# david-knigge/enf-pde

Measured on AMD Instinct MI355X. Metric: query-points/sec (ENF fit+decode) at 64 latents x 64^2 grid, higher is better.
Workload: dtype bf16

## Files before the change

enf-pde_amd/_lib.py:

```python
import ctypes
import os

_HERE = os.path.dirname(os.path.abspath(__file__))
LIB_PATH = os.environ.get("ENF_HIP_LIB") or os.path.join(_HERE, "libenf_hip.so")
TEST_LIB_PATH = os.environ.get("ENF_HIP_TEST_LIB") or os.path.join(_HERE, "libenf_hip_test.so")

ENF_NUM_TENSORS = 46
PREC = {"f32": 0, "fp32": 0, "float32": 0, "bf16": 1, "bfloat16": 1}
INVARIANT_IDS = {"rel_pos_periodic": 0, "latitude_periodic": 1, "polar_periodic": 2, "ponita": 3,
                 "abs_pos": 4, "rel_pos": 5, "norm_rel_pos": 6, "ball": 7, "ball_lat": 8, "ponita_full": 9}

EXPORTS = ["enf_abi_version", "enf_strerror", "enf_invariant_dim", "enf_invariant_pose_dim", "enf_check_desc",
           "enf_packed_weight_bytes", "enf_pack_weights", "enf_workspace_bytes", "enf_forward",
           "enf_backward_latents", "enf_backward_latents_ex", "enf_forward_stages", "enf_lt_layout", "enf_lt_layout_ext", "enf_pack_pair", "enf_pair_forward",
           "enf_pair_backward", "enf_pair_backward_ex", "enf_pair_scratch_bytes", "enf_pair_variant", "enf_pair_partition", "enf_backward_weights", "enf_backward_weights_scratch_bytes",
           "enf_backward_all", "enf_backward_all_scratch_bytes", "enf_fit_step", "enf_fit_inputs",
           "enf_mse_value_grad",
           "enf_ode_conv_forward", "enf_ode_conv_backward_basis", "enf_ode_conv_backward_weight", "enf_ode_conv_backward_weight_scratch_bytes", "enf_ode_poly_num_features", "enf_ode_poly_forward",
           "enf_ode_poly_backward", "enf_ode_vec_readout_forward", "enf_ode_vec_readout_backward", "enf_ode_block_supported", "enf_ode_block_scratch_bytes", "enf_ode_block_forward", "enf_ode_block_backward",
           "enf_ode_basis_supported", "enf_ode_basis_scratch_bytes", "enf_ode_basis_forward",
           "enf_ode_basis_backward", "enf_relu_mask_bytes", "enf_meta_sgd_update"]
ENF_NUM_PAIR_TENSORS = 12
(ENF_S_EQ, ENF_S_EV, ENF_S_G1, ENF_S_NH, ENF_S_DA1, ENF_S_DA2, ENF_S_DA3, ENF_S_HEAD0) = range(8)


def num_store(H):
    return 7 + 4 * H


class EnfDesc(ctypes.Structure):
    _fields_ = [(n, ctypes.c_int32) for n in
                ("B", "N", "Z", "H", "D", "C", "O", "dx", "invariant_id", "use_window", "precision")] + \
               [("h_true", ctypes.c_int32), ("d_true", ctypes.c_int32),
                ("pair_fwd_variant", ctypes.c_int32), ("pair_bwd_variant", ctypes.c_int32), ("mask_mode", ctypes.c_int32),
                ("mask_signals", ctypes.c_int32), ("embedding", ctypes.c_int32), ("relu_masks", ctypes.c_void_p)]


VARIANT = {"auto": 0, "latent_split": 1, "z_fold": 2, "z_fold_zsplit": 3}
MASK_MODE = {"off": 0, "write": 1, "read": 2}
EMB = {"rff": 0, "ffn": 1}


class EnfSgdSegment(ctypes.Structure):
    _fields_ = [("x", ctypes.c_void_p), ("g", ctypes.c_void_p), ("lr", ctypes.c_void_p), ("out", ctypes.c_void_p),
                ("n", ctypes.c_int64), ("width", ctypes.c_int32), ("g_stride", ctypes.c_int32), ("lr_len", ctypes.c_int32),
                ("reserved", ctypes.c_int32)]


ENF_SGD_MAX_SEGMENTS = 4


class EnfFitComponent(ctypes.Structure):
    _fields_ = [("src", ctypes.c_void_p), ("dst", ctypes.c_void_p), ("width", ctypes.c_int32), ("reserved", ctypes.c_int32)]


class EnfError(RuntimeError):
    pass


_lib = None
_test_lib = None


def load():
    global _lib
    if _lib is not None:
        return _lib
    _lib = _bind(LIB_PATH, test_hooks=False)
    return _lib


def load_test():
    global _test_lib
    if _test_lib is None:
        _test_lib = _bind(TEST_LIB_PATH, test_hooks=True)
    return _test_lib


class using:

    def __init__(self, lib):
        self.lib = lib

    def __enter__(self):
        global _lib
        self.prev, _lib = _lib, self.lib
        return self.lib

    def __exit__(self, *exc):
        global _lib
        _lib = self.prev


def _bind(path, test_hooks):
    if not os.path.exists(path):
        raise EnfError(f"{path} not found: build it with `make -C enf-pde_amd/csrc` "
                       "(or python -c 'import __graft_entry__ as g; g.build()'). There is no fallback path.")
    lib = ctypes.CDLL(path)
    vp, i64, sz, ci = ctypes.c_void_p, ctypes.c_int64, ctypes.c_size_t, ctypes.c_int
    dp = ctypes.POINTER(EnfDesc)
    lib.enf_abi_version.restype = ci
    lib.enf_strerror.restype = ctypes.c_char_p
    lib.enf_strerror.argtypes = [ci]
    lib.enf_invariant_dim.argtypes = [ci, ci]
    lib.enf_invariant_pose_dim.argtypes = [ci, ci]
    lib.enf_check_desc.argtypes = [dp]
    lib.enf_packed_weight_bytes.restype = sz
    lib.enf_packed_weight_bytes.argtypes = [dp]
    lib.enf_workspace_bytes.restype = sz
    lib.enf_workspace_bytes.argtypes = [dp]
    lib.enf_pack_weights.argtypes = [dp, ctypes.POINTER(vp), vp, vp]
    lib.enf_forward.argtypes = [dp, vp, i64, vp, vp, vp, vp, vp, vp, vp, vp, sz, vp]
    lib.enf_forward_stages.argtypes = [dp, vp, i64, vp, vp, vp, vp, vp, vp, vp, vp, sz, ctypes.c_uint, vp]
    lib.enf_backward_latents.argtypes = [dp, vp, i64, vp, vp, vp, vp, vp, vp, vp, vp, vp, vp, vp, sz, vp]
    lib.enf_backward_latents_ex.argtypes = [dp, vp, i64, vp, vp, vp, vp, vp, vp, vp, vp, vp, vp, vp, sz, ctypes.c_uint, vp]
    ip = ctypes.POINTER(ci)
    lib.enf_lt_layout.argtypes = [dp, ip, ip, ip, ip, ip, ip]
    lib.enf_pack_pair.argtypes = [dp, ctypes.POINTER(vp), vp, vp]
    lib.enf_mse_value_grad.argtypes = [vp, vp, sz, ctypes.c_float, vp, vp, vp]
    lib.enf_meta_sgd_update.argtypes = [ctypes.c_int, ctypes.POINTER(EnfSgdSegment), ctypes.c_float, vp]
    lib.enf_fit_inputs.argtypes = [ctypes.c_int, ctypes.POINTER(EnfFitComponent)] + [ctypes.c_int32] * 7 + [vp] * 7
    lib.enf_ode_conv_forward.argtypes = [ci, ci, ci, ci, vp, vp, i64, i64, vp, vp, vp, vp]
    lib.enf_ode_conv_backward_basis.argtypes = [ci, ci, ci, ci, vp, vp, vp, vp, vp]
    lib.enf_ode_conv_backward_weight_scratch_bytes.restype = sz
    lib.enf_ode_conv_backward_weight_scratch_bytes.argtypes = [ci, ci, ci, ci]
    lib.enf_ode_conv_backward_weight.argtypes = [ci, ci, ci, ci, vp, vp, vp, vp, vp, sz, vp]
    lib.enf_ode_poly_num_features.argtypes = [ci, ci]
    lib.enf_ode_poly_forward.argtypes = [i64, ci, ci, vp, vp, vp]
    lib.enf_ode_poly_backward.argtypes = [i64, ci, ci, vp, vp, vp, vp]
    lib.enf_ode_basis_supported.argtypes = [ci, ci, ci, ci, ci]
    cf = ctypes.c_float
    lib.enf_ode_vec_readout_forward.argtypes = [ci, ci, ci, ci, vp, vp, vp, vp, cf, cf, vp, vp, vp]
    lib.enf_ode_vec_readout_backward.argtypes = [ci, ci, ci, ci, vp, vp, vp, vp, cf, cf, vp, vp, vp, vp, vp, vp, vp, vp]
    lib.enf_ode_block_supported.argtypes = [ci, ci]
    lib.enf_ode_block_scratch_bytes.restype = sz
    lib.enf_ode_block_scratch_bytes.argtypes = [i64, ci, ci]
    lib.enf_ode_block_forward.argtypes = [i64, ci, ci, vp, vp, vp, vp, vp, vp, vp, ctypes.c_float, vp, vp, vp]
    lib.enf_ode_block_backward.argtypes = [i64, ci, ci, vp, vp, vp, vp, vp, vp, vp, ctypes.c_float, vp, vp, vp, sz, vp]
    lib.enf_ode_basis_scratch_bytes.restype = sz
    lib.enf_ode_basis_scratch_bytes.argtypes = [i64, ci, ci, ci, ci]
    lib.enf_ode_basis_forward.argtypes = [i64, ci, ci, ci, ci, vp, vp, vp, vp, vp, vp, vp, sz, vp]
    lib.enf_ode_basis_backward.argtypes = [i64, ci, ci, ci, ci, vp, vp, vp, vp, vp, vp, vp, vp, vp, vp, vp, vp, sz, vp]
    lib.enf_relu_mask_bytes.restype = sz
    lib.enf_relu_mask_bytes.argtypes = [dp]
    lib.enf_pair_variant.argtypes = [dp, ci]
    lib.enf_pair_partition.argtypes = [dp] + [ctypes.POINTER(ctypes.c_int32)] * 3
    lib.enf_backward_weights_scratch_bytes.restype = sz
    lib.enf_backward_weights_scratch_bytes.argtypes = [dp, ci]
    lib.enf_backward_weights.argtypes = [dp, vp, i64, vp, vp, vp, vp, vp, vp, ctypes.POINTER(vp), vp, vp, sz, vp]
    lib.enf_fit_step.argtypes = [dp, vp, i64, vp, vp, vp, vp, vp, ctypes.c_float, vp, vp, vp, vp, vp, sz, vp]
    lib.enf_backward_all_scratch_bytes.restype = sz
    lib.enf_backward_all_scratch_bytes.argtypes = [dp, ci]
    lib.enf_backward_all.argtypes = [dp, vp, i64, vp, vp, vp, ctypes.POINTER(vp), vp, vp, vp, vp, vp, vp, vp, ctypes.POINTER(vp), vp,
                                     vp, sz, vp, sz, ctypes.c_uint, vp]
    lib.enf_pair_scratch_bytes.restype = sz
    lib.enf_pair_scratch_bytes.argtypes = [dp]
    lib.enf_pair_forward.argtypes = [dp, vp, i64, vp, vp, vp, vp, vp, sz, vp]
    lib.enf_pair_backward.argtypes = [dp, vp, i64, vp, vp, vp, vp, vp, vp, ctypes.POINTER(vp), vp]
    lib.enf_pair_backward_ex.argtypes = [dp, vp, i64, vp, vp, vp, vp, vp, vp, ctypes.POINTER(vp), vp, vp]
    if test_hooks:
        for name in ("enf_debug_gemm", "enf_debug_pack", "enf_test_read_wave_sums"):
            getattr(lib, name).restype = ci
        lib.enf_debug_gemm.argtypes = [vp, vp, vp, ci, ci, ci, vp]
        lib.enf_debug_pack.argtypes = [vp, vp, ci, ci, ci, vp]
        lib.enf_test_read_wave_sums.argtypes = [vp]
    if lib.enf_abi_version() != 2:
        raise EnfError(f"{path}: ABI version mismatch")
    return lib


def check(rc):
    if rc == 0:
        return
    msg = load().enf_strerror(rc).decode()
    if rc == -2:
        raise ValueError(msg)
    if rc == -6:
        raise AssertionError(msg)
    if rc == -3:
        raise NotImplementedError(msg)
    raise EnfError(f"libenf_hip error {rc}: {msg}")


def launch(dev, fn, *args):
    import torch
    idx = dev.index if dev.index is not None else torch.cuda.current_device()
    if idx == torch.cuda.current_device():
        return check(fn(*args))
    with torch.cuda.device(idx):
        return check(fn(*args))


def make_desc(B, N, Z, H, D, C, O, dx, invariant_id, use_window, precision, d_true=0, h_true=0, variants=(0, 0),
              masks=None, embedding=0):
    d = EnfDesc()
    d.B, d.N, d.Z, d.H, d.D, d.C, d.O, d.dx = int(B), int(N), int(Z), int(H), int(D), int(C), int(O), int(dx)
    d.invariant_id, d.use_window, d.precision = int(invariant_id), int(bool(use_window)), int(precision)
    d.d_true, d.h_true = int(d_true), int(h_true)
    d.pair_fwd_variant, d.pair_bwd_variant = int(variants[0]), int(variants[1])
    d.embedding = int(embedding)
    if masks is not None:
        buf, mode, signals = masks
        d.relu_masks, d.mask_mode, d.mask_signals = buf.data_ptr(), MASK_MODE[mode], int(signals)
    return d
```

enf-pde_amd/csrc/enf_api.hip:

```cpp
#include <hip/hip_runtime.h>
#include <mutex>
#include <unordered_map>
#include "enf_launch.h"

extern "C" int enf_abi_version(void) { return ENF_ABI_VERSION; }

extern "C" const char* enf_strerror(int code) {
  switch (code) {
    case ENF_OK: return "ok";
    case ENF_EINVAL: return "invalid argument (null pointer or non-positive size)";
    case ENF_EINVARIANT: return "Unknown invariant type";
    case ENF_EUNSUPPORTED: return "shape not in the compiled kernel set (num_hidden 64 or 128 after padding; num_heads 1, 2, or 4 at num_hidden 64; "
                                  "num_out <= 32; ball / ball_lat at num_hidden 64 only)";
    case ENF_EWORKSPACE: return "workspace too small";
    case ENF_ELAUNCH: return "HIP launch failed";
    case ENF_EDIM: return "coordinate / pose width inconsistent with the invariant";
    default: return "unknown error";
  }
}

extern "C" int enf_invariant_dim(int inv, int dx) {
  const int i = enf_inv_dim(inv, dx);
  return i < 0 ? ENF_EINVARIANT : i;
}
extern "C" int enf_invariant_pose_dim(int inv, int dx) {
  const int i = enf_inv_pose_dim(inv, dx);
  return i < 0 ? ENF_EINVARIANT : i;
}

extern "C" int enf_check_desc(const EnfDesc* d) {
  if (!d) return ENF_EINVAL;
  if (d->B <= 0 || d->N <= 0 || d->Z <= 0 || d->C <= 0 || d->O <= 0 || d->H <= 0 || d->D <= 0) return ENF_EINVAL;
  if (d->invariant_id < 0 || d->invariant_id >= ENF_INV_COUNT) return ENF_EINVARIANT;
  if (d->dx < 1 || d->dx > 3) return ENF_EDIM;
  const bool two_d = d->invariant_id == ENF_INV_REL_POS_PERIODIC || d->invariant_id == ENF_INV_PONITA ||
                     d->invariant_id == ENF_INV_LATITUDE_PERIODIC || d->invariant_id == ENF_INV_POLAR_PERIODIC;
  if (two_d && d->dx != 2) return ENF_EDIM;
  if (d->invariant_id == ENF_INV_PONITA_FULL && d->dx != 3) return ENF_EDIM;
  if (enf_inv_has_phase(d->invariant_id) && d->D != 64) return ENF_EUNSUPPORTED;
  if (enf_inv_has_phase(d->invariant_id) && d->dx != 3) return ENF_EDIM;
  if (!(d->D == 64 || d->D == 128)) return ENF_EUNSUPPORTED;
  if (d->d_true < 0 || d->d_true > d->D || (d->d_true & 1)) return ENF_EINVAL;
  if (!(d->H == 1 || d->H == 2 || (d->H == 4 && d->D == 64))) return ENF_EUNSUPPORTED;
  if (d->h_true < 0 || d->h_true > d->H) return ENF_EINVAL;
  if (d->O > 32) return ENF_EUNSUPPORTED;
  if (d->precision != ENF_PREC_F32 && d->precision != ENF_PREC_BF16) return ENF_EINVAL;
  if (d->pair_fwd_variant < ENF_VARIANT_AUTO || d->pair_fwd_variant > ENF_VARIANT_ZFOLD_ZSPLIT) return ENF_EINVAL;
  if (d->pair_bwd_variant < ENF_VARIANT_AUTO || d->pair_bwd_variant > ENF_VARIANT_ZFOLD) return ENF_EINVAL;
  if (d->mask_mode < ENF_MASK_OFF || d->mask_mode > ENF_MASK_READ || d->mask_signals < 0) return ENF_EINVAL;
  if (d->mask_mode != ENF_MASK_OFF && !d->relu_masks) return ENF_EINVAL;
  if (d->embedding != ENF_EMB_RFF && d->embedding != ENF_EMB_FFN) return ENF_EINVAL;
  if (d->embedding == ENF_EMB_FFN && enf_inv_has_phase(d->invariant_id)) return ENF_EUNSUPPORTED;
  return ENF_OK;
}

extern "C" size_t enf_packed_weight_bytes(const EnfDesc* d) {
  if (enf_check_desc(d) != ENF_OK) return 0;
  return enf_layout(enf_dims(d)).total;
}

extern "C" size_t enf_workspace_bytes(const EnfDesc* d) {
  if (enf_check_desc(d) != ENF_OK) return 0;
  return enf_workspace(enf_dims(d)).total;
}

struct SidePending { hipEvent_t join = nullptr; bool pending = false; };
struct SideStream {
  hipStream_t s = nullptr;
  hipEvent_t fork = nullptr;
  std::mutex mu;
  std::unordered_map<const void*, SidePending> ws;
  SidePending* entry(const void* workspace) {
    auto it = ws.find(workspace);
    if (it != ws.end()) return &it->second;
    if (ws.size() >= 64)
      for (auto j = ws.begin(); j != ws.end();) {
        if (!j->second.pending) { (void)hipEventDestroy(j->second.join); j = ws.erase(j); } else ++j;
      }
    SidePending e;
    if (hipEventCreateWithFlags(&e.join, hipEventDisableTiming) != hipSuccess) return nullptr;
    return &ws.emplace(workspace, e).first->second;
  }
};
static constexpr int ENF_MAX_DEVICES = 64;
static SideStream* side_stream() {
  static std::mutex table_mu;
  static SideStream* table[ENF_MAX_DEVICES] = {};
  static bool tried[ENF_MAX_DEVICES] = {};
  int dev = 0;
  if (hipGetDevice(&dev) != hipSuccess || dev < 0 || dev >= ENF_MAX_DEVICES) return nullptr;
  std::lock_guard<std::mutex> lk(table_mu);
  if (!tried[dev]) {
    tried[dev] = true;
    SideStream* t = new SideStream();
    if (hipStreamCreateWithFlags(&t->s, hipStreamNonBlocking) == hipSuccess &&
        hipEventCreateWithFlags(&t->fork, hipEventDisableTiming) == hipSuccess)
      table[dev] = t;
    else
      delete t;
  }
  return table[dev];
}

int enf_side_join_pending(hipStream_t st, const void* workspace) {
  SideStream* side = side_stream();
  if (!side) return 0;
  std::lock_guard<std::mutex> lk(side->mu);
  auto it = side->ws.find(workspace);
  if (it != side->ws.end() && it->second.pending) {
    if (hipStreamWaitEvent(st, it->second.join, 0) != hipSuccess) return ENF_ELAUNCH;
    it->second.pending = false;
  }
  return 0;
}

static int side_prepare_bwd(SideStream* side, const EnfCall& c, bool zero_dlt) {
  if (!side) return 0;
  std::lock_guard<std::mutex> lk(side->mu);
  SidePending* e = side->entry(c.ws);
  if (!e) return 0;
  if (hipEventRecord(side->fork, c.st) != hipSuccess || hipStreamWaitEvent(side->s, side->fork, 0) != hipSuccess) return ENF_ELAUNCH;
  if (int rc = enf_launch_wz(c.m, c.L, c.blob, c.F(c.W.lt), nullptr, c.F(c.W.wzb), nullptr, c.ws + c.W.wzt, side->s)) return rc;
  if (zero_dlt && hipMemsetAsync(c.F(c.W.dlt), 0, enf_lt_bytes(c.m), side->s) != hipSuccess) return ENF_ELAUNCH;
  if (hipEventRecord(e->join, side->s) != hipSuccess) return ENF_ELAUNCH;
  e->pending = true;
  return 1;
}

extern "C" int enf_forward_stages(const EnfDesc* d, const float* x, int64_t x_bstride, const float* p, const float* a,
                                  const float* sigma, const void* packed, float* out, float* ybar, float* lse,
                                  void* workspace, size_t workspace_bytes, unsigned stages, void* stream) {
  EnfCall c;
  int rc = enf_call(c, d, x && p && a && out, sigma, packed, workspace, workspace_bytes, stream);
  if (rc) return rc;
  const EnfDims& m = c.m;
  const EnfWorkspace& W = c.W;
  float* yb = ybar ? ybar : c.F(W.ybar);
  const bool zf = enf_use_zfold(m);
  float* ls = lse ? lse : c.F(W.lse);
  const bool yhalf = (stages & ENF_STAGE_YBAR_HALF) && m.bf16 && !ybar && (stages & ENF_STAGE_PAIR) && (stages & ENF_STAGE_TAIL) &&
                     !(stages & ENF_STAGE_TAIL_SAVE) && enf_zfold_split(m) <= 1;
  if ((rc = enf_side_join_pending(c.st, workspace))) return rc;
  if ((stages & ENF_STAGE_PROLOGUE) && (rc = enf_launch_prologue(m, c.L, c.blob, p, a, sigma, c.F(W.lt), c.F(W.an), c.F(W.kv), c.st))) return rc;
  if ((stages & (ENF_STAGE_PAIR | ENF_STAGE_FOLD)) &&
      (rc = enf_launch_pair_fwd(m, c.L, c.blob, x, x_bstride, c.F(W.lt), yb, ls, zf ? c.ws + W.wz : nullptr, zf ? c.F(W.wzb) : nullptr,
                                zf ? c.ws + W.wzu : nullptr, enf_zfold_split(m) > 1 ? c.F(W.ysplit) : nullptr, (stages & ENF_STAGE_FOLD) != 0,
                                ((stages & ENF_STAGE_PAIR) != 0 ? 1 : 0) | (yhalf ? 2 : 0), c.st)))
    return rc;
  if ((stages & ENF_STAGE_PREPARE_BWD) && enf_use_zfold_bwd(m) && (rc = side_prepare_bwd(side_stream(), c, true)) < 0) return rc;
  const bool tsave = (stages & ENF_STAGE_TAIL_SAVE) != 0;
  if ((stages & ENF_STAGE_TAIL) &&
      (rc = enf_launch_tail(m, c.L, c.blob, yb, out, nullptr, nullptr, nullptr, tsave ? c.F(W.tail_act) : nullptr, 0, (tsave ? 1 : 0) | (yhalf ? 2 : 0), c.st)))
    return rc;
  return ENF_OK;
}

extern "C" int enf_forward(const EnfDesc* d, const float* x, int64_t x_bstride, const float* p, const float* a,
                           const float* sigma, const void* packed, float* out, float* ybar, float* lse, void* workspace,
                           size_t workspace_bytes, void* stream) {
  return enf_forward_stages(d, x, x_bstride, p, a, sigma, packed, out, ybar, lse, workspace, workspace_bytes,
                            ENF_STAGE_PROLOGUE | ENF_STAGE_FOLD | ENF_STAGE_PAIR | ENF_STAGE_TAIL, stream);
}

extern "C" int enf_backward_latents(const EnfDesc* d, const float* x, int64_t x_bstride, const float* p, const float* a,
                                    const float* sigma, const void* packed, const float* ybar, const float* lse,
                                    const float* dout, float* dp, float* da, float* dsigma, void* workspace,
                                    size_t workspace_bytes, void* stream) {
  return enf_backward_latents_ex(d, x, x_bstride, p, a, sigma, packed, ybar, lse, dout, dp, da, dsigma, workspace,
                                 workspace_bytes, 0u, stream);
}

static int pair_bwd_on_workspace(const EnfCall& c, const float* x, int64_t x_bstride, const float* lse) {
  const bool zb = enf_use_zfold_bwd(c.m);
  return enf_launch_pair_bwd(c.m, c.L, c.blob, x, x_bstride, c.F(c.W.lt), lse, c.F(c.W.dybar), c.F(c.W.delta), c.F(c.W.dlt), nullptr,
                             zb ? c.ws + c.W.wzt : nullptr, zb ? c.F(c.W.wzb) : nullptr, nullptr, c.st);
}

extern "C" int enf_backward_latents_ex(const EnfDesc* d, const float* x, int64_t x_bstride, const float* p, const float* a,
                                       const float* sigma, const void* packed, const float* ybar, const float* lse,
                                       const float* dout, float* dp, float* da, float* dsigma, void* workspace,
                                       size_t workspace_bytes, unsigned flags, void* stream) {
  EnfCall c;
  int rc = enf_call(c, d, x && p && a && ybar && lse && dout && dp && da && dsigma, sigma, packed, workspace, workspace_bytes, stream);
  if (rc) return rc;
  const EnfDims& m = c.m;
  const EnfWorkspace& W = c.W;
  hipStream_t st = c.st;
  const bool zb = enf_use_zfold_bwd(m);
  if (flags & ENF_BWD_ONLY_PAIR) {
    if ((rc = enf_side_join_pending(st, workspace))) return rc;
    if (hipMemsetAsync(c.F(W.dlt), 0, enf_lt_bytes(m), st) != hipSuccess) return ENF_ELAUNCH;
    return pair_bwd_on_workspace(c, x, x_bstride, lse);
  }
  if (!(flags & ENF_BWD_REUSE_PROLOGUE) && (rc = enf_launch_prologue(m, c.L, c.blob, p, a, sigma, c.F(W.lt), c.F(W.an), c.F(W.kv), st)))
    return rc;
  SideStream* side = zb ? side_stream() : nullptr;
  bool prepared = false;
  if (zb && side && (flags & ENF_BWD_REUSE_PREPARED) && (flags & ENF_BWD_REUSE_PROLOGUE)) {
    std::lock_guard<std::mutex> lk(side->mu);
    auto it = side->ws.find(workspace);
    prepared = it != side->ws.end() && it->second.pending;
  }
  if (!prepared && (rc = enf_side_join_pending(st, workspace))) return rc;
  if (zb && !prepared) {
    if ((rc = side_prepare_bwd(side, c, false)) < 0) return rc;
    if (!rc && (rc = enf_launch_wz(m, c.L, c.blob, c.F(W.lt), nullptr, c.F(W.wzb), nullptr, c.ws + W.wzt, st))) return rc;
  }
  const bool treuse = (flags & ENF_BWD_REUSE_TAIL) && (flags & ENF_BWD_REUSE_PROLOGUE);
  if ((rc = enf_launch_tail(m, c.L, c.blob, ybar, nullptr, dout, c.F(W.dybar), c.F(W.delta), c.F(W.tail_act), 1, treuse ? 1 : 0, st))) return rc;
  if (!prepared && hipMemsetAsync(c.F(W.dlt), 0, enf_lt_bytes(m), st) != hipSuccess) return ENF_ELAUNCH;
  if ((rc = enf_side_join_pending(st, workspace))) return rc;
  if ((rc = pair_bwd_on_workspace(c, x, x_bstride, lse))) return rc;
  return enf_launch_prologue_bwd(m, c.L, c.blob, p, sigma, c.F(W.an), c.F(W.kv), c.F(W.dlt), dp, da, dsigma, st);
}


extern "C" int enf_fit_step(const EnfDesc* d, const float* x, int64_t x_bstride, const float* p, const float* a, const float* sigma,
                            const void* packed, const float* target, float grad_scale, float* loss, float* dp, float* da,
                            float* dsigma, void* workspace, size_t workspace_bytes, void* stream) {
  EnfCall c;
  int rc = enf_call(c, d, x && p && a && target && loss && dp && da && dsigma, sigma, packed, workspace, workspace_bytes, stream);
  if (rc) return rc;
  const EnfDims& m = c.m;
  const EnfWorkspace& W = c.W;
  hipStream_t st = c.st;
  const bool zf = enf_use_zfold(m), zb = enf_use_zfold_bwd(m);
  if ((rc = enf_side_join_pending(st, workspace))) return rc;
  if ((rc = enf_launch_prologue(m, c.L, c.blob, p, a, sigma, c.F(W.lt), c.F(W.an), c.F(W.kv), st))) return rc;
  if ((rc = enf_launch_pair_fwd(m, c.L, c.blob, x, x_bstride, c.F(W.lt), c.F(W.ybar), c.F(W.lse), zf ? c.ws + W.wz : nullptr,
                                zf ? c.F(W.wzb) : nullptr, zf ? c.ws + W.wzu : nullptr, enf_zfold_split(m) > 1 ? c.F(W.ysplit) : nullptr, 1, 1, st)))
    return rc;
  if ((rc = side_prepare_bwd(zb ? side_stream() : nullptr, c, true)) < 0) return rc;
  if (!rc) {
    if (zb && (rc = enf_launch_wz(m, c.L, c.blob, c.F(W.lt), nullptr, c.F(W.wzb), nullptr, c.ws + W.wzt, st))) return rc;
    if (hipMemsetAsync(c.F(W.dlt), 0, enf_lt_bytes(m), st) != hipSuccess) return ENF_ELAUNCH;
  }
  if ((rc = enf_launch_tail_loss(m, c.L, c.blob, c.F(W.ybar), target, grad_scale, loss, c.F(W.dybar), c.F(W.delta), c.F(W.tail_act), st))) return rc;
  if ((rc = enf_side_join_pending(st, workspace))) return rc;
  if ((rc = pair_bwd_on_workspace(c, x, x_bstride, c.F(W.lse)))) return rc;
  return enf_launch_prologue_bwd(m, c.L, c.blob, p, sigma, c.F(W.an), c.F(W.kv), c.F(W.dlt), dp, da, dsigma, st);
}

extern "C" int enf_lt_layout(const EnfDesc* d, int* stride, int* off_u, int* off_v0, int* off_pose, int* off_wcoef, int* off_c) {
  int rc = enf_check_desc(d);
  if (rc) return rc;
  if (stride) *stride = enf_lt_stride(d->H, d->D);
  if (off_u) *off_u = enf_lt_off_u(d->H, d->D);
  if (off_v0) *off_v0 = enf_lt_off_v0(d->H, d->D);
  if (off_pose) *off_pose = enf_lt_off_pose(d->H, d->D);
  if (off_wcoef) *off_wcoef = enf_lt_off_wcoef(d->H, d->D);
  if (off_c) *off_c = enf_lt_off_c(d->H, d->D);
  return ENF_OK;
}

extern "C" int enf_lt_layout_ext(const EnfDesc* d, int* off_ext, int* off_phase_q, int* off_phase_v) {
  int rc = enf_check_desc(d);
  if (rc) return rc;
  if (off_ext) *off_ext = enf_lt_off_ext(d->H, d->D);
  if (off_phase_q) *off_phase_q = enf_lt_off_phq(d->H, d->D);
  if (off_phase_v) *off_phase_v = enf_lt_off_phv(d->H, d->D);
  return ENF_OK;
}

extern "C" int enf_pair_variant(const EnfDesc* d, int backward) {
  const int rc = enf_check_desc(d);
  if (rc) return rc;
  const EnfDims m = enf_dims(d);
  if (backward) return enf_use_zfold_bwd(m) ? ENF_VARIANT_ZFOLD : ENF_VARIANT_LATENT_SPLIT;
  const int sp = enf_zfold_split(m);
  return sp > 1 ? ENF_VARIANT_ZFOLD_ZSPLIT : (sp == 1 ? ENF_VARIANT_ZFOLD : ENF_VARIANT_LATENT_SPLIT);
}

extern "C" int enf_pair_partition(const EnfDesc* d, int32_t* run, int32_t* workgroups, int32_t* parts) {
  const int rc = enf_check_desc(d);
  if (rc) return rc;
  if (!run || !workgroups || !parts) return ENF_EINVAL;
  const EnfDims m = enf_dims(d);
  if (enf_zfold_split(m) < 2) return 0;
  const EnfStreamK k = enf_zfold_streamk(m);
  *run = k.len; *workgroups = k.wgs; *parts = k.parts;
  return 1;
}

struct PairScratch { size_t wz, wzb, wzu, ysplit, total; };
static PairScratch pair_scratch(const EnfDims& m) {
  PairScratch s{0, 0, 0, 0, 0};
  if (!enf_use_zfold(m)) return s;
  const size_t BZ = (size_t)m.B * m.Z, BN = (size_t)m.B * m.N;
  const int split = enf_zfold_split(m);
  s.wzb = s.wz + enf_align(BZ * m.H * enf_panel_bytes(m.D, m.D, m.bf16));
  s.wzu = s.wzb + enf_align(sizeof(float) * BZ * m.HD);
  s.ysplit = s.wzu + enf_align(BZ * enf_wzu_bytes(m.H, m.D));
  s.total = s.ysplit + (split > 1 ? sizeof(float) * split * (BN * m.HD + BN * m.H * 3) : 0);
  return s;
}

extern "C" size_t enf_pair_scratch_bytes(const EnfDesc* d) {
  if (enf_check_desc(d)) return 0;
  return pair_scratch(enf_dims(d)).total;
}

extern "C" int enf_pair_forward(const EnfDesc* d, const float* x, int64_t x_bstride, const float* lt, const void* packed,
                                float* ybar, float* lse, void* scratch, size_t scratch_bytes, void* stream) {
  int rc = enf_check_desc(d);
  if (rc) return rc;
  if (!x || !lt || !packed || !ybar || !lse) return ENF_EINVAL;
  const EnfDims m = enf_dims(d);
  const PairScratch S = pair_scratch(m);
  const bool zf = S.total != 0;
  if (zf && (!scratch || scratch_bytes < S.total)) return ENF_EWORKSPACE;
  char* sc = (char*)scratch;
  return enf_launch_pair_fwd(m, enf_layout(m), (const char*)packed, x, x_bstride, lt, ybar, lse, zf ? sc + S.wz : nullptr,
                             zf ? reinterpret_cast<float*>(sc + S.wzb) : nullptr, zf ? sc + S.wzu : nullptr,
                             zf && enf_zfold_split(m) > 1 ? reinterpret_cast<float*>(sc + S.ysplit) : nullptr, 1, 1, (hipStream_t)stream);
}

extern "C" size_t enf_relu_mask_bytes(const EnfDesc* d) {
  if (enf_check_desc(d) != ENF_OK) return 0;
  const size_t signals = d->mask_signals > 0 ? d->mask_signals : d->B;
  return signals * d->Z * ((d->N + 15) / 16) * 2 * 64 * sizeof(unsigned);
}

extern "C" int enf_pair_backward(const EnfDesc* d, const float* x, int64_t x_bstride, const float* lt, const void* packed,
                                 const float* lse, const float* dybar, const float* delta, float* dlt, void* const* store,
                                 void* stream) {
  return enf_pair_backward_ex(d, x, x_bstride, lt, packed, lse, dybar, delta, dlt, store, nullptr, stream);
}

extern "C" int enf_pair_backward_ex(const EnfDesc* d, const float* x, int64_t x_bstride, const float* lt, const void* packed,
                                    const float* lse, const float* dybar, const float* delta, float* dlt, void* const* store,
                                    float* dx, void* stream) {
  int rc = enf_check_desc(d);
  if (rc) return rc;
  if (!x || !lt || !packed || !lse || !dybar || !delta || !dlt) return ENF_EINVAL;
  const EnfDims m = enf_dims(d);
  if (store)
    for (int i = 0; i < ENF_NUM_STORE(m.H); ++i)
      if (!store[i]) return ENF_EINVAL;
  hipStream_t st = (hipStream_t)stream;
  if (hipMemsetAsync(dlt, 0, enf_lt_bytes(m), st) != hipSuccess) return ENF_ELAUNCH;
  return enf_launch_pair_bwd(m, enf_layout(m), (const char*)packed, x, x_bstride, lt, lse, dybar, delta, dlt, store, nullptr, nullptr, dx, st);
}

extern "C" size_t enf_backward_weights_scratch_bytes(const EnfDesc* d, int chunk_signals) {
  if (enf_check_desc(d) != ENF_OK || chunk_signals < 1 || chunk_signals > d->B) return 0;
  return enf_wgrad_scratch_bytes(enf_dims(d), chunk_signals);
}

extern "C" int enf_backward_weights(const EnfDesc* d, const float* x, int64_t x_bstride, const float* lt, const void* packed,
                                    const float* lse, const float* dybar, const float* delta, float* dlt,
                                    float* const* dpair, float* dx, void* scratch, size_t scratch_bytes, void* stream) {
  int rc = enf_check_desc(d);
  if (rc) return rc;
  if (d->embedding == ENF_EMB_FFN) return ENF_EUNSUPPORTED;
  if (!x || !lt || !packed || !lse || !dybar || !delta || !dlt || !dpair || !scratch) return ENF_EINVAL;
  for (int i = 0; i < ENF_NUM_PAIR_TENSORS; ++i)
    if (i != ENF_P_COEFQ && i != ENF_P_COEFV && !dpair[i]) return ENF_EINVAL;
  const EnfDims m = enf_dims(d);
  const int cb = enf_wgrad_chunk(m, scratch_bytes, [&](int n) { return enf_wgrad_scratch_bytes(m, n); });
  if (!cb) return ENF_EWORKSPACE;
  return enf_launch_wgrad_chunks(m, enf_layout(m), (const char*)packed, cb, x, x_bstride, lt, lse, dybar, delta, dlt, dx, (char*)scratch,
                                 dpair, (hipStream_t)stream);
}
```

enf-pde_amd/csrc/enf_debug.hip:

```cpp
#include <hip/hip_runtime.h>
#include "enf_launch.h"
#include "enf_device.h"

template <int KBIN, int MTOUT, bool BF16>
__global__ __launch_bounds__(64) void enf_debug_gemm_kernel(const char* panel, const float* X, float* Y) {
  extern __shared__ __attribute__((aligned(16))) char smem[];
  const int lane = threadIdx.x, col = lane & 15, quad = lane >> 4;
  constexpr int BYTES = PanelCfg<KBIN, MTOUT, BF16>::BYTES;
  for (int i = lane; i < BYTES / 16; i += 64)
    reinterpret_cast<f32x4*>(smem)[i] = reinterpret_cast<const f32x4*>(panel)[i];
  __syncthreads();
  f32x4 x[2 * KBIN];
#pragma unroll
  for (int t = 0; t < 2 * KBIN; ++t)
#pragma unroll
    for (int i = 0; i < 4; ++i) x[t][i] = X[(16 * t + 4 * quad + i) * 16 + col];
  Frags<BF16, KBIN> F;
  make_frags<BF16, KBIN>(F, x);
  f32x4 acc[MTOUT];
#pragma unroll
  for (int m = 0; m < MTOUT; ++m) acc[m] = f32x4{0.f, 0.f, 0.f, 0.f};
  gemm_stage<BF16, KBIN, MTOUT>(acc, F, smem, lane);
#pragma unroll
  for (int m = 0; m < MTOUT; ++m)
#pragma unroll
    for (int i = 0; i < 4; ++i) Y[(16 * m + 4 * quad + i) * 16 + col] = acc[m][i];
}

extern "C" int enf_debug_gemm(const void* panel, const float* X, float* Y, int M, int K, int bf16, void* stream) {
  hipStream_t st = (hipStream_t)stream;
  const size_t bytes = (size_t)M * K * (bf16 ? 2 : 4);
#define C(KB, MT)                                                                                                   \
  if (K == 32 * KB && M == 16 * MT) {                                                                               \
    if (bf16) hipLaunchKernelGGL((enf_debug_gemm_kernel<KB, MT, true>), dim3(1), dim3(64), bytes, st, (const char*)panel, X, Y);  \
    else hipLaunchKernelGGL((enf_debug_gemm_kernel<KB, MT, false>), dim3(1), dim3(64), bytes, st, (const char*)panel, X, Y);      \
    return hipGetLastError() == hipSuccess ? 0 : ENF_ELAUNCH;                                                        \
  }
  C(2, 4) C(4, 4) C(1, 4) C(2, 1)
#undef C
  return ENF_EUNSUPPORTED;
}
```

enf-pde_amd/csrc/enf_launch.h:

```cpp
#pragma once
#include <hip/hip_runtime.h>
#include <atomic>
#include "enf_layout.h"

typedef std::atomic<unsigned long long> EnfAttrBits;
inline bool enf_lds_attr(const void* kern, int bytes, EnfAttrBits& done) {
  int dev = 0;
  if (hipGetDevice(&dev) != hipSuccess) return false;
  if (dev >= 0 && dev < 64 && ((done.load(std::memory_order_acquire) >> dev) & 1ull)) return true;
  if (hipFuncSetAttribute(kern, hipFuncAttributeMaxDynamicSharedMemorySize, bytes) != hipSuccess) return false;
  if (dev >= 0 && dev < 64) done.fetch_or(1ull << dev, std::memory_order_release);
  return true;
}

struct EnfCall {
  EnfDims m;
  EnfLayout L;
  EnfWorkspace W;
  hipStream_t st;
  char* ws;
  const char* blob;
  float* F(size_t off) const { return reinterpret_cast<float*>(ws + off); }
};
inline int enf_call(EnfCall& c, const EnfDesc* d, bool pointers_ok, const float* sigma, const void* packed, void* workspace,
                    size_t workspace_bytes, void* stream) {
  const int rc = enf_check_desc(d);
  if (rc) return rc;
  if (!pointers_ok || !packed || !workspace) return ENF_EINVAL;
  if (d->use_window && !sigma) return ENF_EINVAL;
  c.m = enf_dims(d);
  c.L = enf_layout(c.m);
  c.W = enf_workspace(c.m);
  if (workspace_bytes < c.W.total) return ENF_EWORKSPACE;
  c.st = (hipStream_t)stream;
  c.ws = (char*)workspace;
  c.blob = (const char*)packed;
  return ENF_OK;
}

int enf_side_join_pending(hipStream_t st, const void* workspace);

int enf_launch_prologue(const EnfDims& m, const EnfLayout& L, const char* blob, const float* p, const float* a, const float* sigma,
                        float* lt, float* an, float* kv, hipStream_t st);
int enf_launch_prologue_bwd(const EnfDims& m, const EnfLayout& L, const char* blob, const float* p, const float* sigma,
                            const float* an, const float* kv, const float* dlt, float* dp, float* da, float* dsigma, hipStream_t st);
int enf_launch_prologue_bwd_wg(const EnfDims& m, const EnfLayout& L, const char* blob, const float* p, const float* sigma,
                               const float* an, const float* kv, const float* dlt, float* dp, float* da, float* dsigma, float* pg,
                               hipStream_t st);

int enf_launch_wz(const EnfDims& m, const EnfLayout& L, const char* blob, const float* lt, char* wz, float* wzb, char* wzu,
                  char* wzt, hipStream_t st);

int enf_launch_pair_fwd(const EnfDims& m, const EnfLayout& L, const char* blob, const float* x, long long x_bstride, const float* lt,
                        float* ybar, float* lse, char* wz, float* wzb, char* wzu, float* ysplit, int run_fold, int run_pair,
                        hipStream_t st);

int enf_launch_pair_bwd(const EnfDims& m, const EnfLayout& L, const char* blob, const float* x, long long x_bstride, const float* lt,
                        const float* lse, const float* dybar, const float* delta, float* dlt, void* const* store, const char* wzt,
                        const float* wzb, float* dxq, hipStream_t st);

size_t enf_xtd_part_bytes(const EnfDims& m, long long P);
int enf_launch_xtd(const EnfDims& m, void* const* store, long long P, float* const* dpair, float* part, int accumulate,
                   hipStream_t st);

size_t enf_wgrad_scratch_bytes(const EnfDims& m, int cb);
int enf_launch_wgrad_chunks(const EnfDims& m, const EnfLayout& L, const char* blob, int cb, const float* x, long long x_bstride,
                            const float* lt, const float* lse, const float* dybar, const float* delta, float* dlt, float* dx,
                            char* scratch, float* const* dpair, hipStream_t st);
template <class Bytes>
inline int enf_wgrad_chunk(const EnfDims& m, size_t avail, Bytes bytes) {
  const int step = m.mask_mode == ENF_MASK_READ && m.mask_B < m.B ? m.mask_B : 1;
  int cb = m.B;
  while (cb > step && bytes(cb) > avail) cb = (cb - 1) / step * step;
  return cb >= 1 && bytes(cb) <= avail ? cb : 0;
}

int enf_launch_tail(const EnfDims& m, const EnfLayout& L, const char* blob, const float* ybar, float* out, const float* dout,
                    float* dybar, float* delta, float* act, int bwd, int opt, hipStream_t st);
int enf_launch_tail_wg(const EnfDims& m, const EnfLayout& L, const char* blob, const float* ybar, float* out, const float* dout,
                       float* dybar, float* delta, float* act, float* tdel, int bwd, int opt, hipStream_t st);
int enf_launch_tail_loss(const EnfDims& m, const EnfLayout& L, const char* blob, const float* ybar, const float* target, float gscale,
                         float* loss, float* dybar, float* delta, float* act, hipStream_t st);
```

enf-pde_amd/csrc/enf_prologue.hip:

```cpp
#include <hip/hip_runtime.h>
#include <math.h>
#include <type_traits>
#include "enf_launch.h"

typedef float pf4 __attribute__((ext_vector_type(4)));

#ifndef ENF_PROLOGUE_ZT
#define ENF_PROLOGUE_ZT 4
#endif
constexpr int ZT = ENF_PROLOGUE_ZT;
#ifndef ENF_PROLOGUE_UNROLL
#define ENF_PROLOGUE_UNROLL 16
#endif
#define PRO_UNROLL ENF_PROLOGUE_UNROLL

static __device__ __forceinline__ float wave_sum(float v) {
  for (int o = 32; o > 0; o >>= 1) v += __shfl_xor(v, o, 64);
  return v;
}

struct PrologueArgs {
  const float* p; const float* a; const float* sigma;
  const char* blob; EnfLayout L;
  float* lt; float* an; float* kv;
  int BZ, H, D, C, dp, inv;
  int Dt;
};

__global__ __launch_bounds__(256) void enf_prologue_kernel(PrologueArgs A) {
  extern __shared__ __attribute__((aligned(16))) float sm[];
  const int D = A.D, H = A.H, HD = H * D, C = A.C;
  float* s_a = sm;
  float* s_an = s_a + ZT * C;
  float* s_k = s_an + ZT * D;
  const int tid = threadIdx.x, lane = tid & 63, wave = tid >> 6;
  const int row0 = blockIdx.x * ZT;
  auto W = [&](size_t off) { return reinterpret_cast<const float*>(A.blob + off); };
  const int stride = enf_lt_stride(H, D);
  for (int i = tid; i < ZT * C; i += 256) {
    const int zz = i / C, c = i % C, r = row0 + zz;
    s_a[c * ZT + zz] = r < A.BZ ? A.a[(size_t)r * C + c] : 0.f;
  }
  __syncthreads();
  for (int d = tid; d < D; d += 256) {
    float acc[ZT];
    const float bs = W(A.L.stem_b)[d];
#pragma unroll
    for (int zz = 0; zz < ZT; ++zz) acc[zz] = bs;
#pragma unroll PRO_UNROLL
    for (int c = 0; c < C; ++c) {
      const float w = W(A.L.stem_w)[(size_t)c * D + d];
#pragma unroll
      for (int q = 0; q < ZT / 4; ++q) {
        const pf4 x = *reinterpret_cast<const pf4*>(s_a + c * ZT + 4 * q);
#pragma unroll
        for (int zz = 0; zz < 4; ++zz) acc[4 * q + zz] = fmaf(x[zz], w, acc[4 * q + zz]);
      }
    }
#pragma unroll
    for (int zz = 0; zz < ZT; ++zz) s_an[d * ZT + zz] = acc[zz];
  }
  __syncthreads();
  for (int zz = wave; zz < ZT; zz += 4) {
    const int r = row0 + zz;
    float v = 0.f;
    for (int d = lane; d < A.Dt; d += 64) v += s_an[d * ZT + zz];
    const float mu = wave_sum(v) / A.Dt;
    float q = 0.f;
    for (int d = lane; d < A.Dt; d += 64) { const float t = s_an[d * ZT + zz] - mu; q += t * t; }
    const float rstd = rsqrtf(wave_sum(q) / A.Dt + 1e-6f);
    for (int d = lane; d < D; d += 64) {
      const float sv = s_an[d * ZT + zz];
      const float xn = (sv - mu) * rstd;
      if (r < A.BZ) {
        A.an[(size_t)r * (2 * D + 2) + d] = sv;
        A.an[(size_t)r * (2 * D + 2) + D + d] = xn;
      }
      s_an[d * ZT + zz] = xn * W(A.L.lna_g)[d] + W(A.L.lna_b)[d];
    }
    if (lane == 0 && r < A.BZ) { A.an[(size_t)r * (2 * D + 2) + 2 * D] = mu; A.an[(size_t)r * (2 * D + 2) + 2 * D + 1] = rstd; }
  }
  __syncthreads();
  for (int j = tid; j < 2 * HD; j += 256) {
    const bool isv = j >= HD;
    const int jj = isv ? j - HD : j;
    const float* Wm = W(isv ? A.L.wv : A.L.wk);
    float acc[ZT];
    const float bb = W(isv ? A.L.bv : A.L.bk)[jj];
#pragma unroll
    for (int zz = 0; zz < ZT; ++zz) acc[zz] = bb;
#pragma unroll PRO_UNROLL
    for (int d = 0; d < D; ++d) {
      const float w = Wm[(size_t)d * HD + jj];
#pragma unroll
      for (int q = 0; q < ZT / 4; ++q) {
        const pf4 x = *reinterpret_cast<const pf4*>(s_an + d * ZT + 4 * q);
#pragma unroll
        for (int zz = 0; zz < 4; ++zz) acc[4 * q + zz] = fmaf(x[zz], w, acc[4 * q + zz]);
      }
    }
#pragma unroll
    for (int zz = 0; zz < ZT; ++zz) {
      const int r = row0 + zz;
      if (!isv) s_k[jj * ZT + zz] = acc[zz];
      if (r < A.BZ) {
        A.kv[(size_t)r * 2 * HD + j] = acc[zz];
        if (isv) A.lt[(size_t)r * stride + enf_lt_off_v0(H, D) + jj] = acc[zz];
      }
    }
  }
  __syncthreads();
  for (int j = tid; j < HD; j += 256) {
    const int h = j / D, i = j % D;
    const float* mut = W(A.L.mut) + (size_t)h * D * D + i;
    float acc[ZT];
#pragma unroll
    for (int zz = 0; zz < ZT; ++zz) acc[zz] = 0.f;
#pragma unroll PRO_UNROLL
    for (int dd = 0; dd < D; ++dd) {
      const float w = mut[(size_t)dd * D];
      const float* kp = s_k + (h * D + dd) * ZT;
#pragma unroll
      for (int q = 0; q < ZT / 4; ++q) {
        const pf4 x = *reinterpret_cast<const pf4*>(kp + 4 * q);
#pragma unroll
        for (int zz = 0; zz < 4; ++zz) acc[4 * q + zz] = fmaf(x[zz], w, acc[4 * q + zz]);
      }
    }
#pragma unroll
    for (int zz = 0; zz < ZT; ++zz) {
      const int r = row0 + zz;
      if (r < A.BZ) A.lt[(size_t)r * stride + enf_lt_off_u(H, D) + j] = acc[zz];
    }
  }
  for (int t = wave; t < ZT * H; t += 4) {
    const int zz = t / H, h = t % H, r = row0 + zz;
    float sacc = 0.f;
    for (int dd = lane; dd < D; dd += 64) sacc = fmaf(W(A.L.cvec)[h * D + dd], s_k[(h * D + dd) * ZT + zz], sacc);
    sacc = wave_sum(sacc);
    if (lane == 0 && r < A.BZ) A.lt[(size_t)r * stride + enf_lt_off_c(H, D) + h] = sacc;
  }
  if (tid < ZT) {
    const int r = row0 + tid;
    if (r < A.BZ) {
      const float* pp = A.p + (size_t)r * A.dp;
      float q[4] = {0.f, 0.f, 0.f, 0.f};
      float wc;
      const float sg = A.sigma ? A.sigma[r] : 1.f;
      const bool sphere = A.inv == ENF_INV_LATITUDE_PERIODIC || A.inv == ENF_INV_POLAR_PERIODIC || enf_inv_has_phase(A.inv);
      if (A.inv == ENF_INV_PONITA || A.inv == ENF_INV_PONITA_FULL) { q[0] = pp[0]; q[1] = pp[1]; q[2] = cosf(pp[2]); q[3] = sinf(pp[2]); }
      else if (sphere) { q[0] = pp[0]; q[1] = pp[1]; q[2] = sinf(pp[1]); q[3] = cosf(pp[1]); }
      else { for (int i = 0; i < A.dp && i < 3; ++i) q[i] = pp[i]; }
      wc = sphere ? 1.f / (2.f * sg * sg) : 1.f / (sg * sg);
      float* o = A.lt + (size_t)r * stride;
      for (int i = 0; i < 4; ++i) o[enf_lt_off_pose(H, D) + i] = q[i];
      o[enf_lt_off_wcoef(H, D)] = wc;
      if (enf_inv_has_phase(A.inv)) {
        float lat[2] = {0.f, 0.f};
        if (A.inv == ENF_INV_BALL) {
          const float ca = cosf(pp[0]), sa = sinf(pp[0]), cb = cosf(pp[1]), sb = sinf(pp[1]), cg = cosf(pp[2]), sg2 = sinf(pp[2]);
          float* R = o + enf_lt_off_ext(H, D);
          R[0] = ca * cb; R[1] = ca * sb * sg2 - sa * cg; R[2] = ca * sb * cg + sa * sg2;
          R[3] = sa * cb; R[4] = sa * sb * sg2 + ca * cg; R[5] = sa * sb * cg - ca * sg2;
          R[6] = -sb;     R[7] = cb * sg2;                R[8] = cb * cg;
          lat[0] = pp[3];
        } else { lat[0] = pp[1]; lat[1] = pp[3]; }
        const float* cq = W(A.L.cphq), *cv = W(A.L.cphv);
        for (int j = 0; j < D / 2; ++j) {
          o[enf_lt_off_phq(H, D) + j] = lat[0] * cq[j] + lat[1] * cq[D / 2 + j];
          o[enf_lt_off_phv(H, D) + j] = lat[0] * cv[j] + lat[1] * cv[D / 2 + j];
        }
      }
    }
  }
}

int enf_launch_prologue(const EnfDims& m, const EnfLayout& L, const char* blob, const float* p, const float* a,
                        const float* sigma, float* lt, float* an, float* kv, hipStream_t st) {
  PrologueArgs A;
  A.p = p; A.a = a; A.sigma = sigma; A.blob = blob; A.L = L; A.lt = lt; A.an = an; A.kv = kv;
  A.BZ = m.B * m.Z; A.H = m.H; A.D = m.D; A.C = m.C; A.dp = m.dp; A.inv = m.inv; A.Dt = m.Dt;
  const size_t smem = sizeof(float) * (ZT * m.C + ZT * m.D + ZT * m.HD);
  hipLaunchKernelGGL(enf_prologue_kernel, dim3((A.BZ + ZT - 1) / ZT), dim3(256), smem, st, A);
  return hipGetLastError() == hipSuccess ? 0 : ENF_ELAUNCH;
}

struct PrologueBwdArgs {
  const float* p; const float* sigma; const char* blob; EnfLayout L;
  const float* an; const float* kv; const float* dlt;
  float* dp; float* da; float* dsigma;
  int BZ, H, D, C, dp_dim, inv;
  int Dt;
  float* pg;
};

__global__ __launch_bounds__(256) void enf_prologue_bwd_kernel(PrologueBwdArgs A) {
  extern __shared__ __attribute__((aligned(16))) float sm[];
  const int D = A.D, H = A.H, HD = H * D, C = A.C;
  float* s_du = sm;
  float* s_dk = s_du + ZT * HD;
  float* s_dan = s_dk + ZT * 2 * HD;
  float* s_dc = s_dan + ZT * D;
  float* s_part = s_dc + ZT * H;
  const int tid = threadIdx.x, lane = tid & 63, wave = tid >> 6, row0 = blockIdx.x * ZT;
  const int stride = enf_lt_stride(H, D);
  auto W = [&](size_t off) { return reinterpret_cast<const float*>(A.blob + off); };
  for (int t = tid; t < ZT * HD; t += 256) {
    const int zz = t / HD, j = t % HD, r = row0 + zz;
    const float* g = A.dlt + (size_t)(r < A.BZ ? r : 0) * stride;
    s_du[j * ZT + zz] = r < A.BZ ? g[enf_lt_off_u(H, D) + j] : 0.f;
    s_dk[(HD + j) * ZT + zz] = r < A.BZ ? g[enf_lt_off_v0(H, D) + j] : 0.f;
  }
  if (tid < ZT * H) {
    const int zz = tid / H, h = tid % H, r = row0 + zz;
    s_dc[h * ZT + zz] = r < A.BZ ? A.dlt[(size_t)r * stride + enf_lt_off_c(H, D) + h] : 0.f;
  }
  __syncthreads();
  for (int j = tid; j < HD; j += 256) {
    const int h = j / D, dd = j % D;
    const float cv = W(A.L.cvec)[h * D + dd];
    const float* mu = W(A.L.mu) + (size_t)h * D * D + dd;
    float acc[ZT];
#pragma unroll
    for (int zz = 0; zz < ZT; ++zz) acc[zz] = cv * s_dc[h * ZT + zz];
#pragma unroll PRO_UNROLL
    for (int i = 0; i < D; ++i) {
      const float w = mu[(size_t)i * D];
      const float* gp = s_du + (h * D + i) * ZT;
#pragma unroll
      for (int q = 0; q < ZT / 4; ++q) {
        const pf4 x = *reinterpret_cast<const pf4*>(gp + 4 * q);
#pragma unroll
        for (int zz = 0; zz < 4; ++zz) acc[4 * q + zz] = fmaf(x[zz], w, acc[4 * q + zz]);
      }
    }
#pragma unroll
    for (int zz = 0; zz < ZT; ++zz) {
      s_dk[j * ZT + zz] = acc[zz];
      if (A.pg && row0 + zz < A.BZ) {
        float* pr = A.pg + (size_t)(row0 + zz) * (2 * HD + 4 * D);
        pr[j] = acc[zz];
        pr[HD + 4 * D + j] = s_dc[h * ZT + zz] * A.kv[(size_t)(row0 + zz) * 2 * HD + j];
      }
    }
  }
  __syncthreads();
  {
    const int nsplit = 256 / D, d = tid % D, part = tid / D, jper = HD / nsplit;
    float acc[ZT];
#pragma unroll
    for (int zz = 0; zz < ZT; ++zz) acc[zz] = 0.f;
    const float* wkt = W(A.L.wkt) + d;
    const float* wvt = W(A.L.wvt) + d;
#pragma unroll PRO_UNROLL
    for (int j = part * jper; j < (part + 1) * jper; ++j) {
      const float wk = wkt[(size_t)j * D], wv = wvt[(size_t)j * D];
#pragma unroll
      for (int q = 0; q < ZT / 4; ++q) {
        const pf4 kq = *reinterpret_cast<const pf4*>(s_dk + j * ZT + 4 * q), vq = *reinterpret_cast<const pf4*>(s_dk + (HD + j) * ZT + 4 * q);
#pragma unroll
        for (int zz = 0; zz < 4; ++zz) acc[4 * q + zz] = fmaf(wk, kq[zz], fmaf(wv, vq[zz], acc[4 * q + zz]));
      }
    }
#pragma unroll
    for (int zz = 0; zz < ZT; ++zz) s_part[tid * ZT + zz] = acc[zz];
    __syncthreads();
    if (tid < D) {
      const float g = W(A.L.lna_g)[tid];
#pragma unroll
      for (int zz = 0; zz < ZT; ++zz) {
        float v = 0.f;
        for (int q = 0; q < nsplit; ++q) v += s_part[(q * D + tid) * ZT + zz];
        s_dan[tid * ZT + zz] = v * g;
        if (A.pg && row0 + zz < A.BZ) {
          float* pr = A.pg + (size_t)(row0 + zz) * (2 * HD + 4 * D) + HD;
          const float xn = A.an[(size_t)(row0 + zz) * (2 * D + 2) + D + tid];
          pr[tid] = v;
          pr[2 * D + tid] = xn * g + W(A.L.lna_b)[tid];
          pr[3 * D + tid] = v * xn;
        }
      }
    }
  }
  __syncthreads();
  for (int zz = wave; zz < ZT; zz += 4) {
    const int r = row0 + zz;
    const int rr = r < A.BZ ? r : A.BZ - 1;
    const float* anr = A.an + (size_t)rr * (2 * D + 2);
    float v1 = 0.f, v2 = 0.f;
    for (int d = lane; d < D; d += 64) { const float g = s_dan[d * ZT + zz]; v1 += g; v2 += g * anr[D + d]; }
    const float m1 = wave_sum(v1) / A.Dt, m2 = wave_sum(v2) / A.Dt;
    const float rstd = anr[2 * D + 1];
    for (int d = lane; d < D; d += 64) {
      const float ds = rstd * (s_dan[d * ZT + zz] - m1 - anr[D + d] * m2);
      s_dan[d * ZT + zz] = ds;
      if (A.pg && r < A.BZ) A.pg[(size_t)r * (2 * HD + 4 * D) + HD + D + d] = ds;
    }
  }
  __syncthreads();
  for (int t = tid; t < ZT * C; t += 256) {
    const int zz = t / C, c = t % C, r = row0 + zz;
    float sacc = 0.f;
#pragma unroll PRO_UNROLL
    for (int d = 0; d < D; ++d) sacc = fmaf(W(A.L.stem_w)[(size_t)c * D + d], s_dan[d * ZT + zz], sacc);
    if (r < A.BZ) A.da[(size_t)r * C + c] = sacc;
  }
  if (tid < ZT) {
    const int r = row0 + tid;
    if (r < A.BZ) {
      const float* g = A.dlt + (size_t)r * stride + enf_lt_off_pose(H, D);
      const float* pp = A.p + (size_t)r * A.dp_dim;
      float* o = A.dp + (size_t)r * A.dp_dim;
      const bool sph = A.inv == ENF_INV_LATITUDE_PERIODIC || A.inv == ENF_INV_POLAR_PERIODIC || enf_inv_has_phase(A.inv);
      if (A.inv == ENF_INV_PONITA || A.inv == ENF_INV_PONITA_FULL) { o[0] = g[0]; o[1] = g[1]; o[2] = -sinf(pp[2]) * g[2] + cosf(pp[2]) * g[3]; }
      else if (sph) { o[0] = g[0]; o[1] = g[1] + cosf(pp[1]) * g[2] - sinf(pp[1]) * g[3]; }
      else { for (int i = 0; i < A.dp_dim && i < 3; ++i) o[i] = g[i]; }
      if (enf_inv_has_phase(A.inv)) {
        const float* e = A.dlt + (size_t)r * stride + enf_lt_off_ext(H, D);
        if (A.inv == ENF_INV_BALL) {
          const float ca = cosf(pp[0]), sa = sinf(pp[0]), cb = cosf(pp[1]), sb = sinf(pp[1]), cg = cosf(pp[2]), sg2 = sinf(pp[2]);
          o[0] += e[0] * (-sa * cb) + e[1] * (-sa * sb * sg2 - ca * cg) + e[2] * (-sa * sb * cg + ca * sg2) +
                  e[3] * (ca * cb) + e[4] * (ca * sb * sg2 - sa * cg) + e[5] * (ca * sb * cg + sa * sg2);
          o[1] += e[0] * (-ca * sb) + e[1] * (ca * cb * sg2) + e[2] * (ca * cb * cg) + e[3] * (-sa * sb) + e[4] * (sa * cb * sg2) +
                  e[5] * (sa * cb * cg) + e[6] * (-cb) + e[7] * (-sb * sg2) + e[8] * (-sb * cg);
          o[2] = e[1] * (ca * sb * cg + sa * sg2) + e[2] * (-ca * sb * sg2 + sa * cg) + e[4] * (sa * sb * cg - ca * sg2) +
                 e[5] * (-sa * sb * sg2 - ca * cg) + e[7] * (cb * cg) + e[8] * (-cb * sg2);
          o[3] = e[9];
        } else { o[1] += e[9]; o[2] = 0.f; o[3] = e[10]; }
      }
      const float sg = A.sigma ? A.sigma[r] : 1.f;
      const float dwc = A.dlt[(size_t)r * stride + enf_lt_off_wcoef(H, D)];
      A.dsigma[r] = (sph ? -1.f : -2.f) / (sg * sg * sg) * dwc;
    }
  }
}

namespace {
constexpr int LT = 16;
constexpr int PW = 8;

__device__ __forceinline__ void mm_tile(pf4& acc, const float* __restrict__ A, int lda, int i0, int K, const float* sB, int lane) {
  const int i = lane & 15, kk = lane >> 4;
  const float* ap = A + (size_t)kk * lda + i0 + i;
  const float* bp = sB + kk * LT + i;
  int k0 = 0;
  for (; k0 + 32 <= K; k0 += 32) {
    float a[8], b[8];
#pragma unroll
    for (int u = 0; u < 8; ++u) { a[u] = ap[(size_t)(k0 + 4 * u) * lda]; b[u] = bp[(k0 + 4 * u) * LT]; }
    __builtin_amdgcn_sched_barrier(0);
#pragma unroll
    for (int u = 0; u < 8; ++u) acc = __builtin_amdgcn_mfma_f32_16x16x4f32(a[u], b[u], acc, 0, 0, 0);
  }
  for (; k0 < K; k0 += 4) {
    const bool ok = k0 + kk < K;
    const float a = ok ? ap[(size_t)k0 * lda] : 0.f, b = ok ? bp[k0 * LT] : 0.f;
    acc = __builtin_amdgcn_mfma_f32_16x16x4f32(a, b, acc, 0, 0, 0);
  }
}
__device__ __forceinline__ void mm_tile_rows(pf4& acc, const float* __restrict__ M, int ldm, int i0, int imax, int K, const float* sB, int lane) {
  const int i = lane & 15, kk = lane >> 4;
  const bool iok = i0 + i < imax;
  for (int k0 = 0; k0 < K; k0 += 4) {
    const bool ok = iok && k0 + kk < K;
    const float a = ok ? M[(size_t)(i0 + i) * ldm + k0 + kk] : 0.f, b = k0 + kk < K ? sB[(k0 + kk) * LT + i] : 0.f;
    acc = __builtin_amdgcn_mfma_f32_16x16x4f32(a, b, acc, 0, 0, 0);
  }
}
template <int NT>
__device__ __forceinline__ void mm_tiles(pf4 (&acc)[NT], const float* const (&ap)[NT], const float* const (&bp)[NT], int lda, int K) {
  for (int k0 = 0; k0 < K; k0 += 32) {
    float a[NT][8], b[NT][8];
#pragma unroll
    for (int t = 0; t < NT; ++t)
#pragma unroll
      for (int u = 0; u < 8; ++u) { a[t][u] = ap[t][(size_t)(k0 + 4 * u) * lda]; b[t][u] = bp[t][(k0 + 4 * u) * LT]; }
    __builtin_amdgcn_sched_barrier(0);
#pragma unroll
    for (int u = 0; u < 8; ++u) {
#pragma unroll
      for (int t = 0; t < NT; ++t) acc[t] = __builtin_amdgcn_mfma_f32_16x16x4f32(a[t][u], b[t][u], acc[t], 0, 0, 0);
      __builtin_amdgcn_sched_barrier(0);
    }
  }
}
__device__ __forceinline__ float half_sum(float v) {
  for (int o = 16; o > 0; o >>= 1) v += __shfl_xor(v, o, 64);
  return v;
}

struct ProBwdArgs {
  const float* p; const float* sigma; const char* blob; EnfLayout L;
  const float* an; const float* kv; const float* dlt;
  float* dp; float* da; float* dsigma; float* pg;
  int BZ, H, D, C, dp_dim, inv, Dt;
};

__global__ __launch_bounds__(64 * PW) void enf_prologue_bwd_mfma_kernel(ProBwdArgs A) {
  extern __shared__ __attribute__((aligned(16))) float sm[];
  const int D = A.D, H = A.H, HD = H * D, C = A.C, PGW = 2 * HD + 4 * D;
  float* s_du = sm;
  float* s_dk = s_du + HD * LT;
  float* s_dan = s_dk + 2 * HD * LT;
  float* s_dc = s_dan + D * LT;
  const int tid = threadIdx.x, lane = tid & 63, wave = tid >> 6, j = lane & 15, q = lane >> 4, row0 = blockIdx.x * LT;
  const int stride = enf_lt_stride(H, D);
  auto W = [&](size_t off) { return reinterpret_cast<const float*>(A.blob + off); };
  for (int t = tid; t < LT * HD; t += 64 * PW) {
    const int zz = t / HD, f = t % HD, r = row0 + zz;
    const float* g = A.dlt + (size_t)(r < A.BZ ? r : 0) * stride;
    s_du[f * LT + zz] = r < A.BZ ? g[enf_lt_off_u(H, D) + f] : 0.f;
    s_dk[(HD + f) * LT + zz] = r < A.BZ ? g[enf_lt_off_v0(H, D) + f] : 0.f;
  }
  if (tid < LT * H) {
    const int zz = tid / H, h = tid % H, r = row0 + zz;
    s_dc[h * LT + zz] = r < A.BZ ? A.dlt[(size_t)r * stride + enf_lt_off_c(H, D) + h] : 0.f;
  }
  __syncthreads();
  const int r_mine = row0 + j;
  const bool rok = r_mine < A.BZ;
  {
    const int T = HD / 16;
    auto dk_tiles = [&](auto nt_c) {
      constexpr int NT = decltype(nt_c)::value;
      pf4 acc[NT];
      const float* ap[NT];
      const float* bp[NT];
      int f0[NT];
#pragma unroll
      for (int t = 0; t < NT; ++t) {
        f0[t] = 16 * (wave + PW * t);
        const int h = f0[t] / D, d0 = f0[t] % D;
        acc[t] = pf4{0.f, 0.f, 0.f, 0.f};
        ap[t] = W(A.L.mu) + (size_t)h * D * D + (size_t)q * D + d0 + j;
        bp[t] = s_du + (h * D + q) * LT + j;
      }
      mm_tiles<NT>(acc, ap, bp, D, D);
#pragma unroll
      for (int t = 0; t < NT; ++t) {
        const int h = f0[t] / D;
        const float dc = s_dc[h * LT + j];
        const pf4 cv = *reinterpret_cast<const pf4*>(W(A.L.cvec) + f0[t] + 4 * q);
#pragma unroll
        for (int e = 0; e < 4; ++e) { acc[t][e] = fmaf(cv[e], dc, acc[t][e]); s_dk[(f0[t] + 4 * q + e) * LT + j] = acc[t][e]; }
        if (A.pg && rok) {
          float* pr = A.pg + (size_t)r_mine * PGW;
          const pf4 kq = *reinterpret_cast<const pf4*>(A.kv + (size_t)r_mine * 2 * HD + f0[t] + 4 * q);
          *reinterpret_cast<pf4*>(pr + f0[t] + 4 * q) = acc[t];
          *reinterpret_cast<pf4*>(pr + HD + 4 * D + f0[t] + 4 * q) = pf4{dc * kq[0], dc * kq[1], dc * kq[2], dc * kq[3]};
        }
      }
    };
    if (T == 16) dk_tiles(std::integral_constant<int, 2>{});
    else if (T == 8 || wave < T) dk_tiles(std::integral_constant<int, 1>{});
  }
  __syncthreads();
  if (wave < D / 16) {
    const int t = wave, hk = HD / 2;
    pf4 acc[4];
    const float* ap[4];
    const float* bp[4];
#pragma unroll
    for (int v = 0; v < 4; ++v) {
      acc[v] = pf4{0.f, 0.f, 0.f, 0.f};
      ap[v] = W(v < 2 ? A.L.wkt : A.L.wvt) + (size_t)((v & 1) * hk + q) * D + 16 * t + j;
      bp[v] = s_dk + ((v < 2 ? 0 : HD) + (v & 1) * hk + q) * LT + j;
    }
    mm_tiles<4>(acc, ap, bp, D, hk);
    pf4 sum;
#pragma unroll
    for (int e = 0; e < 4; ++e) sum[e] = (acc[0][e] + acc[1][e]) + (acc[2][e] + acc[3][e]);
    const pf4 g = *reinterpret_cast<const pf4*>(W(A.L.lna_g) + 16 * t + 4 * q);
#pragma unroll
    for (int e = 0; e < 4; ++e) s_dan[(16 * t + 4 * q + e) * LT + j] = sum[e] * g[e];
    if (A.pg && rok) {
      float* pr = A.pg + (size_t)r_mine * PGW + HD;
      const pf4 xn = *reinterpret_cast<const pf4*>(A.an + (size_t)r_mine * (2 * D + 2) + D + 16 * t + 4 * q);
      const pf4 b = *reinterpret_cast<const pf4*>(W(A.L.lna_b) + 16 * t + 4 * q);
      *reinterpret_cast<pf4*>(pr + 16 * t + 4 * q) = sum;
      *reinterpret_cast<pf4*>(pr + 2 * D + 16 * t + 4 * q) = pf4{xn[0] * g[0] + b[0], xn[1] * g[1] + b[1], xn[2] * g[2] + b[2], xn[3] * g[3] + b[3]};
      *reinterpret_cast<pf4*>(pr + 3 * D + 16 * t + 4 * q) = pf4{sum[0] * xn[0], sum[1] * xn[1], sum[2] * xn[2], sum[3] * xn[3]};
    }
  }
  __syncthreads();
  {
    const int zz = 2 * wave + (lane >> 5), l32 = lane & 31, r = row0 + zz;
    const int rr = r < A.BZ ? r : A.BZ - 1;
    const float* anr = A.an + (size_t)rr * (2 * D + 2);
    float v1 = 0.f, v2 = 0.f;
    for (int d = l32; d < D; d += 32) { const float g = s_dan[d * LT + zz]; v1 += g; v2 += g * anr[D + d]; }
    const float m1 = half_sum(v1) / A.Dt, m2 = half_sum(v2) / A.Dt;
    const float rstd = anr[2 * D + 1];
    for (int d = l32; d < D; d += 32) {
      const float ds = rstd * (s_dan[d * LT + zz] - m1 - anr[D + d] * m2);
      s_dan[d * LT + zz] = ds;
      if (A.pg && r < A.BZ) A.pg[(size_t)r * PGW + HD + D + d] = ds;
    }
  }
  __syncthreads();
  for (int t = wave; t < (C + 15) / 16; t += PW) {
    pf4 acc = {0.f, 0.f, 0.f, 0.f};
    mm_tile_rows(acc, W(A.L.stem_w), D, 16 * t, C, D, s_dan, lane);
    if (rok) {
#pragma unroll
      for (int e = 0; e < 4; ++e)
        if (16 * t + 4 * q + e < C) A.da[(size_t)r_mine * C + 16 * t + 4 * q + e] = acc[e];
    }
  }
  if (tid < LT) {
    const int r = row0 + tid;
    if (r < A.BZ) {
      const float* g = A.dlt + (size_t)r * stride + enf_lt_off_pose(H, D);
      const float* pp = A.p + (size_t)r * A.dp_dim;
      float* o = A.dp + (size_t)r * A.dp_dim;
      const bool sph = A.inv == ENF_INV_LATITUDE_PERIODIC || A.inv == ENF_INV_POLAR_PERIODIC || enf_inv_has_phase(A.inv);
      if (A.inv == ENF_INV_PONITA || A.inv == ENF_INV_PONITA_FULL) { o[0] = g[0]; o[1] = g[1]; o[2] = -sinf(pp[2]) * g[2] + cosf(pp[2]) * g[3]; }
      else if (sph) { o[0] = g[0]; o[1] = g[1] + cosf(pp[1]) * g[2] - sinf(pp[1]) * g[3]; }
      else { for (int i = 0; i < A.dp_dim && i < 3; ++i) o[i] = g[i]; }
      if (enf_inv_has_phase(A.inv)) {
        const float* e = A.dlt + (size_t)r * stride + enf_lt_off_ext(H, D);
        if (A.inv == ENF_INV_BALL) {
          const float ca = cosf(pp[0]), sa = sinf(pp[0]), cb = cosf(pp[1]), sb = sinf(pp[1]), cg = cosf(pp[2]), sg2 = sinf(pp[2]);
          o[0] += e[0] * (-sa * cb) + e[1] * (-sa * sb * sg2 - ca * cg) + e[2] * (-sa * sb * cg + ca * sg2) +
                  e[3] * (ca * cb) + e[4] * (ca * sb * sg2 - sa * cg) + e[5] * (ca * sb * cg + sa * sg2);
          o[1] += e[0] * (-ca * sb) + e[1] * (ca * cb * sg2) + e[2] * (ca * cb * cg) + e[3] * (-sa * sb) + e[4] * (sa * cb * sg2) +
                  e[5] * (sa * cb * cg) + e[6] * (-cb) + e[7] * (-sb * sg2) + e[8] * (-sb * cg);
          o[2] = e[1] * (ca * sb * cg + sa * sg2) + e[2] * (-ca * sb * sg2 + sa * cg) + e[4] * (sa * sb * cg - ca * sg2) +
                 e[5] * (-sa * sb * sg2 - ca * cg) + e[7] * (cb * cg) + e[8] * (-cb * sg2);
          o[3] = e[9];
        } else { o[1] += e[9]; o[2] = 0.f; o[3] = e[10]; }
      }
      const float sg = A.sigma ? A.sigma[r] : 1.f;
      const float dwc = A.dlt[(size_t)r * stride + enf_lt_off_wcoef(H, D)];
      A.dsigma[r] = (sph ? -1.f : -2.f) / (sg * sg * sg) * dwc;
    }
  }
}
}

static int enf_launch_prologue_bwd_mfma(const EnfDims& m, const EnfLayout& L, const char* blob, const float* p, const float* sigma,
                                        const float* an, const float* kv, const float* dlt, float* dp, float* da, float* dsigma,
                                        float* pg, hipStream_t st) {
  ProBwdArgs A;
  A.p = p; A.sigma = sigma; A.blob = blob; A.L = L; A.an = an; A.kv = kv; A.dlt = dlt;
  A.dp = dp; A.da = da; A.dsigma = dsigma; A.pg = pg;
  A.BZ = m.B * m.Z; A.H = m.H; A.D = m.D; A.C = m.C; A.dp_dim = m.dp; A.inv = m.inv; A.Dt = m.Dt;
  const size_t smem = sizeof(float) * LT * (3 * m.HD + m.D + m.H);
  static EnfAttrBits attr{0};
  if (!enf_lds_attr(reinterpret_cast<const void*>(enf_prologue_bwd_mfma_kernel), 160 * 1024, attr)) return ENF_ELAUNCH;
  hipLaunchKernelGGL(enf_prologue_bwd_mfma_kernel, dim3((A.BZ + LT - 1) / LT), dim3(64 * PW), smem, st, A);
  return hipGetLastError() == hipSuccess ? 0 : ENF_ELAUNCH;
}

int enf_launch_prologue_bwd(const EnfDims& m, const EnfLayout& L, const char* blob, const float* p,
                            const float* sigma, const float* an, const float* kv, const float* dlt, float* dp,
                            float* da, float* dsigma, hipStream_t st) {
  return enf_launch_prologue_bwd_wg(m, L, blob, p, sigma, an, kv, dlt, dp, da, dsigma, nullptr, st);
}
int enf_launch_prologue_bwd_wg(const EnfDims& m, const EnfLayout& L, const char* blob, const float* p,
                               const float* sigma, const float* an, const float* kv, const float* dlt, float* dp,
                               float* da, float* dsigma, float* pg, hipStream_t st) {
  if (m.D % 32 == 0) return enf_launch_prologue_bwd_mfma(m, L, blob, p, sigma, an, kv, dlt, dp, da, dsigma, pg, st);
  PrologueBwdArgs A;
  A.pg = pg;
  A.p = p; A.sigma = sigma; A.blob = blob; A.L = L; A.an = an; A.kv = kv; A.dlt = dlt;
  A.dp = dp; A.da = da; A.dsigma = dsigma;
  A.BZ = m.B * m.Z; A.H = m.H; A.D = m.D; A.C = m.C; A.dp_dim = m.dp; A.inv = m.inv; A.Dt = m.Dt;
  const size_t smem = sizeof(float) * (ZT * 3 * m.HD + ZT * m.D + ZT * m.H + ZT * 256);
  hipLaunchKernelGGL(enf_prologue_bwd_kernel, dim3((A.BZ + ZT - 1) / ZT), dim3(256), smem, st, A);
  return hipGetLastError() == hipSuccess ? 0 : ENF_ELAUNCH;
}
```

enf-pde_amd/csrc/enf_tail.hip:

```cpp
#include <hip/hip_runtime.h>
#include <cstdlib>
#include "enf_launch.h"
#define ENF_PIPE_ONE_RS 1
#include "enf_device.h"

struct TailArgs {
  const float* ybar; const char* blob; EnfLayout L;
  float* out;
  const float* dout;
  float* dybar; float* delta; float* act;
  const float* target; float* loss; float gscale, inv_n;
  float* tdel;
  int ybar_half;
  int NQ, O;
  float inv_hd;
};

template <int NT> DEV void load_rows(f32x4 (&X)[NT], const float* row, int quad) {
#pragma unroll
  for (int t = 0; t < NT; ++t) X[t] = *reinterpret_cast<const f32x4*>(row + 16 * t + 4 * quad);
}
template <int NT> DEV void load_rows_half(f32x4 (&X)[NT], const unsigned short* row, int quad) {
#pragma unroll
  for (int t = 0; t < NT; ++t) {
    const uint2 w = *reinterpret_cast<const uint2*>(row + 16 * t + 4 * quad);
    X[t] = f32x4{__builtin_bit_cast(float, w.x << 16), __builtin_bit_cast(float, w.x & 0xffff0000u),
                 __builtin_bit_cast(float, w.y << 16), __builtin_bit_cast(float, w.y & 0xffff0000u)};
  }
}
template <int NT> DEV void store_rows(const f32x4 (&X)[NT], float* row, int quad) {
#pragma unroll
  for (int t = 0; t < NT; ++t) *reinterpret_cast<f32x4*>(row + 16 * t + 4 * quad) = X[t];
}
template <int NT> DEV void zero_tiles(f32x4 (&X)[NT]) {
#pragma unroll
  for (int t = 0; t < NT; ++t) X[t] = f32x4{0.f, 0.f, 0.f, 0.f};
}

template <int D, int H, bool BF16> struct TailCfg {
  static constexpr int KB = D / 32, KBH = H * D / 32, NT = D / 16, NTH = H * D / 16, HD = H * D;
  static constexpr int ACT = 2 * HD + 2 * D + 2;
  static constexpr int ST_TB = PanelCfg<KBH, NTH, BF16>::STAGE;
  static constexpr int ST_O0 = PanelCfg<KBH, NT, BF16>::STAGE;
  static constexpr int ST_O2 = PanelCfg<KB, NT, BF16>::STAGE;
  static constexpr int ST_O4 = PanelCfg<KB, 2, BF16>::STAGE;
  static constexpr int ST_G4 = PanelCfg<1, NT, BF16>::STAGE;
  static constexpr int ST_G0 = PanelCfg<KB, NTH, BF16>::STAGE;
  static constexpr int SMEM = 2 * STAGE_MAX + 4 * (2 * HD + 2 * D + 32);
  static constexpr int SMEM3 = 3 * STAGE_MAX + 4 * (2 * HD + 2 * D + 32);
};

template <int BYTES> struct La2Cnt { static constexpr int K = BYTES > 0 ? (BYTES / 1024) / NWAVES : 0; };
template <int K> DEV void wait_vm() { asm volatile("s_waitcnt vmcnt(%0)" ::"n"(K) : "memory"); }
template <int BYTES> DEV void la2_issue(const Pipe& P, unsigned off, char* ring, int slot, int lane) {
  stage_issue<BYTES>(P.rs, off, ring + slot * STAGE_MAX, P.wave, lane);
}
template <int KBIN, int MTOUT, bool BF16> struct Pan {
  using C = PanelCfg<KBIN, MTOUT, BF16>;
  static constexpr int SPP = C::SPP, STAGE = C::STAGE;
};
struct NoPan { static constexpr int SPP = 0, STAGE = 0; };

template <int SP, int KBIN, int MTOUT, bool BF16, typename N1, typename N2, int INIT>
DEV void la2_step(f32x4 (&acc)[MTOUT], const Frags<BF16, KBIN>& F, Pipe& P, char* ring, unsigned panel, unsigned n1, unsigned n2,
                  int lane, const float* bias) {
  using C = PanelCfg<KBIN, MTOUT, BF16>;
  constexpr int AHEAD = SP + 2 - C::SPP;
  const int slot2 = (P.cur + 2) % 3;
  constexpr int ISSUED = AHEAD < 0 ? C::STAGE : (AHEAD < N1::SPP ? N1::STAGE : (AHEAD == N1::SPP && N1::SPP <= 1 ? N2::STAGE : 0));
  if constexpr (AHEAD < 0) la2_issue<C::STAGE>(P, panel + (SP + 2) * C::STAGE, ring, slot2, lane);
  else if constexpr (AHEAD < N1::SPP) la2_issue<N1::STAGE>(P, n1 + AHEAD * N1::STAGE, ring, slot2, lane);
  else if constexpr (AHEAD == N1::SPP && N1::SPP <= 1 && N2::STAGE > 0) la2_issue<N2::STAGE>(P, n2, ring, slot2, lane);
  gemm_stage<BF16, KBIN, C::MTS, INIT>(&acc[SP * C::MTS], F, ring + P.cur * STAGE_MAX, lane, bias + 16 * SP * C::MTS);
  wait_vm<La2Cnt<ISSUED>::K>();
  __syncthreads();
  P.cur = (P.cur + 1) % 3;
}
template <int KBIN, int MTOUT, bool BF16, typename N1, typename N2, int INIT = INIT_ACC>
DEV void panel_gemm_la2(f32x4 (&acc)[MTOUT], const Frags<BF16, KBIN>& F, Pipe& P, char* ring, unsigned panel, unsigned n1,
                        unsigned n2, int lane, const float* bias = nullptr) {
  using C = PanelCfg<KBIN, MTOUT, BF16>;
  static_assert(C::SPP <= 8, "unrolled by hand");
#define LA2_STEP(SP_) if constexpr (C::SPP > SP_) la2_step<SP_, KBIN, MTOUT, BF16, N1, N2, INIT>(acc, F, P, ring, panel, n1, n2, lane, bias);
  LA2_STEP(0) LA2_STEP(1) LA2_STEP(2) LA2_STEP(3) LA2_STEP(4) LA2_STEP(5) LA2_STEP(6) LA2_STEP(7)
#undef LA2_STEP
}
template <typename A0, typename B0>
DEV void la2_first(Pipe& P, char* ring, unsigned a, unsigned b, int wave, int lane) {
  P.cur = 0;
  P.wave = __builtin_amdgcn_readfirstlane(wave);
  P.early = false;
  la2_issue<A0::STAGE>(P, a, ring, 0, lane);
  constexpr int S1 = A0::SPP > 1 ? A0::STAGE : B0::STAGE;
  if constexpr (A0::SPP > 1) la2_issue<A0::STAGE>(P, a + A0::STAGE, ring, 1, lane);
  else if constexpr (B0::STAGE > 0) la2_issue<B0::STAGE>(P, b, ring, 1, lane);
  wait_vm<La2Cnt<S1>::K>();
  __syncthreads();
}
template <bool LA2, int KBIN, int MTOUT, bool BF16, typename N1, typename N2, int NEXT_BYTES>
DEV void tail_gemm(f32x4 (&acc)[MTOUT], const Frags<BF16, KBIN>& F, Pipe& P, char* ring, unsigned panel, unsigned n1, unsigned n2,
                   int lane) {
  if constexpr (LA2) panel_gemm_la2<KBIN, MTOUT, BF16, N1, N2>(acc, F, P, ring, panel, n1, n2, lane);
  else panel_gemm<KBIN, MTOUT, BF16, NEXT_BYTES>(acc, F, P, ring, panel, n1, true, lane);
}

template <int D, int H, bool BF16, bool SAVE, bool LA2, typename NX1, typename NX2>
DEV void tail_forward(f32x4 (&o4)[2], const float* yrow, float* act, const EnfLayout& L, const float* cst, Pipe& P,
                      char* ring, unsigned next, unsigned next2, int lane, int quad, float inv_hd, bool save_ok = true, bool y_half = false) {
  using T = TailCfg<D, H, BF16>;
  constexpr int KB = T::KB, KBH = T::KBH, NT = T::NT, NTH = T::NTH, HD = T::HD;
  using PTB = Pan<KBH, NTH, BF16>; using PO0 = Pan<KBH, NT, BF16>; using PO2 = Pan<KB, NT, BF16>; using PO4 = Pan<KB, 2, BF16>;
  constexpr int NEXT_BYTES = NX1::STAGE > 0 ? NX1::STAGE : 1024;
  const float* c_bB = cst, *c_bF1 = cst + HD, *c_bO0 = cst + 2 * HD, *c_bO2 = cst + 2 * HD + D, *c_bO4 = cst + 2 * HD + 2 * D;
  Frags<BF16, KBH> FH;
  f32x4 a[NTH];
  if (y_half) load_rows_half<NTH>(a, reinterpret_cast<const unsigned short*>(yrow), quad);
  else load_rows<NTH>(a, yrow, quad);
  make_frags<BF16, KBH>(FH, a);
#pragma unroll
  for (int t = 0; t < NTH; ++t) a[t] = rowvec(c_bB, t, quad);
  tail_gemm<LA2, KBH, NTH, BF16, PTB, PO0, T::ST_TB>(a, FH, P, ring, (unsigned)L.atb, (unsigned)L.atf1, (unsigned)L.ato0, lane);
  if (SAVE && save_ok) store_rows<NTH>(a, act, quad);
#pragma unroll
  for (int t = 0; t < NTH; ++t)
#pragma unroll
    for (int i = 0; i < 4; ++i) a[t][i] = gelu_f(a[t][i]);
  float mu, rstd;
  ln_stats<NTH>(a, mu, rstd, inv_hd);
  if (SAVE && save_ok && quad == 0) { act[T::ACT - 2] = mu; act[T::ACT - 1] = rstd; }
  ln_apply<NTH>(a, mu, rstd);
  make_frags<BF16, KBH>(FH, a);
#pragma unroll
  for (int t = 0; t < NTH; ++t) a[t] = rowvec(c_bF1, t, quad);
  tail_gemm<LA2, KBH, NTH, BF16, PO0, PO2, T::ST_O0>(a, FH, P, ring, (unsigned)L.atf1, (unsigned)L.ato0, (unsigned)L.ato2, lane);
  if (SAVE && save_ok) store_rows<NTH>(a, act + HD, quad);
#pragma unroll
  for (int t = 0; t < NTH; ++t)
#pragma unroll
    for (int i = 0; i < 4; ++i) a[t][i] = gelu_f(a[t][i]);
  make_frags<BF16, KBH>(FH, a);
  f32x4 c[NT];
#pragma unroll
  for (int t = 0; t < NT; ++t) c[t] = rowvec(c_bO0, t, quad);
  tail_gemm<LA2, KBH, NT, BF16, PO2, PO4, T::ST_O2>(c, FH, P, ring, (unsigned)L.ato0, (unsigned)L.ato2, (unsigned)L.ato4, lane);
  if (SAVE && save_ok) store_rows<NT>(c, act + 2 * HD, quad);
#pragma unroll
  for (int t = 0; t < NT; ++t)
#pragma unroll
    for (int i = 0; i < 4; ++i) c[t][i] = gelu_f(c[t][i]);
  Frags<BF16, KB> FD;
  make_frags<BF16, KB>(FD, c);
#pragma unroll
  for (int t = 0; t < NT; ++t) c[t] = rowvec(c_bO2, t, quad);
  tail_gemm<LA2, KB, NT, BF16, PO4, NX1, T::ST_O4>(c, FD, P, ring, (unsigned)L.ato2, (unsigned)L.ato4, next, lane);
  if (SAVE && save_ok) store_rows<NT>(c, act + 2 * HD + D, quad);
#pragma unroll
  for (int t = 0; t < NT; ++t)
#pragma unroll
    for (int i = 0; i < 4; ++i) c[t][i] = gelu_f(c[t][i]);
  make_frags<BF16, KB>(FD, c);
  o4[0] = rowvec(c_bO4, 0, quad);
  o4[1] = rowvec(c_bO4, 1, quad);
  tail_gemm<LA2, KB, 2, BF16, NX1, NX2, NEXT_BYTES>(o4, FD, P, ring, (unsigned)L.ato4, next, next2, lane);
}

template <int D, int H, bool BF16>
DEV void tail_consts(float* cst, const char* blob, const EnfLayout& L, int tid) {
  constexpr int HD = H * D;
  auto G = [&](size_t off) { return reinterpret_cast<const float*>(blob + off); };
  for (int i = tid; i < HD; i += NTHREADS) { cst[i] = G(L.bB)[i]; cst[HD + i] = G(L.bF1)[i]; }
  for (int i = tid; i < D; i += NTHREADS) { cst[2 * HD + i] = G(L.bO0)[i]; cst[2 * HD + D + i] = G(L.bO2)[i]; }
  for (int i = tid; i < 32; i += NTHREADS) cst[2 * HD + 2 * D + i] = G(L.bO4)[i];
}

template <int D, int H, bool BF16, bool LA2, bool SAVE>
__global__ __launch_bounds__(NTHREADS, 2) void enf_tail_fwd_kernel(TailArgs A) {
  using T = TailCfg<D, H, BF16>;
  extern __shared__ __attribute__((aligned(16))) char smem[];
  char* ring = smem;
  float* cst = reinterpret_cast<float*>(smem + (LA2 ? 3 : 2) * STAGE_MAX);
  const int tid = threadIdx.x, lane = tid & 63, wave = tid >> 6, col = lane & 15, quad = lane >> 4;
  const int q0 = blockIdx.x * (16 * NWAVES) + wave * 16;
  const int qi = min(q0 + col, A.NQ - 1);
  tail_consts<D, H, BF16>(cst, A.blob, A.L, tid);
  Pipe P;
  P.rs = make_blob_rsrc(A.blob, (unsigned)A.L.total);
  P.rs2 = P.rs;
  if constexpr (LA2) {
    __syncthreads();
    la2_first<Pan<T::KBH, T::NTH, BF16>, Pan<T::KBH, T::NTH, BF16>>(P, ring, (unsigned)A.L.atb, (unsigned)A.L.atf1, wave, lane);
  } else first_stage<T::ST_TB>(P, ring, (unsigned)A.L.atb, wave, lane);
  f32x4 o4[2];
  const bool yh = !SAVE && A.ybar_half;
  const float* yrow = yh ? reinterpret_cast<const float*>(reinterpret_cast<const unsigned short*>(A.ybar) + (size_t)qi * T::HD)
                         : A.ybar + (size_t)qi * T::HD;
  tail_forward<D, H, BF16, SAVE, LA2, NoPan, NoPan>(o4, yrow, SAVE ? A.act + (size_t)qi * T::ACT : nullptr, A.L,
                                                    cst, P, ring, NO_STAGE, NO_STAGE, lane, quad, A.inv_hd, true, yh);
  if (q0 + col < A.NQ) {
#pragma unroll
    for (int t = 0; t < 2; ++t)
#pragma unroll
      for (int i = 0; i < 4; ++i) {
        const int o = 16 * t + 4 * quad + i;
        if (o < A.O) A.out[(size_t)(q0 + col) * A.O + o] = o4[t][i];
      }
  }
}

template <int D, int H, bool BF16, bool LA2, bool RECOMP, bool WG = false, bool LOSS = false>
__global__ __launch_bounds__(NTHREADS, 2) void enf_tail_bwd_kernel(TailArgs A) {
  static_assert(!LOSS || RECOMP, "the fused loss needs the forward chain's outputs");
  using T = TailCfg<D, H, BF16>;
  constexpr int KB = T::KB, KBH = T::KBH, NT = T::NT, NTH = T::NTH, HD = T::HD;
  using PG4 = Pan<1, NT, BF16>; using PG2 = Pan<KB, NT, BF16>; using PG0 = Pan<KB, NTH, BF16>; using PGH = Pan<KBH, NTH, BF16>;
  extern __shared__ __attribute__((aligned(16))) char smem[];
  char* ring = smem;
  float* cst = reinterpret_cast<float*>(smem + (LA2 ? 3 : 2) * STAGE_MAX);
  const int tid = threadIdx.x, lane = tid & 63, wave = tid >> 6, col = lane & 15, quad = lane >> 4;
  const int q0 = blockIdx.x * (16 * NWAVES) + wave * 16;
  const bool qvalid = q0 + col < A.NQ;
  const int qi = min(q0 + col, A.NQ - 1);
  float* act = A.act + (size_t)qi * T::ACT;
  float* tdel = WG ? A.tdel + (size_t)qi * (2 * HD + 2 * D) : nullptr;
  const float* yrow = A.ybar + (size_t)qi * HD;
  tail_consts<D, H, BF16>(cst, A.blob, A.L, tid);
  Pipe P;
  P.rs = make_blob_rsrc(A.blob, (unsigned)A.L.total);
  P.rs2 = P.rs;
  f32x4 o4[2] = {f32x4{0.f, 0.f, 0.f, 0.f}, f32x4{0.f, 0.f, 0.f, 0.f}};
  if constexpr (RECOMP) {
    if constexpr (LA2) {
      __syncthreads();
      la2_first<PGH, PGH>(P, ring, (unsigned)A.L.atb, (unsigned)A.L.atf1, wave, lane);
    } else first_stage<T::ST_TB>(P, ring, (unsigned)A.L.atb, wave, lane);
    tail_forward<D, H, BF16, true, LA2, PG4, PG2>(o4, yrow, act, A.L, cst, P, ring, (unsigned)A.L.gto4, (unsigned)A.L.gto2, lane, quad,
                                                  A.inv_hd, !WG || qvalid);
  } else {
    if constexpr (LA2) {
      __syncthreads();
      la2_first<PG4, PG2>(P, ring, (unsigned)A.L.gto4, (unsigned)A.L.gto2, wave, lane);
    } else first_stage<T::ST_G4>(P, ring, (unsigned)A.L.gto4, wave, lane);
  }

  f32x4 g0[2];
  if constexpr (LOSS) {
    float se = 0.f;
    const float gs = 2.0f * A.inv_n * A.gscale;
#pragma unroll
    for (int t = 0; t < 2; ++t)
#pragma unroll
      for (int i = 0; i < 4; ++i) {
        const int o = 16 * t + 4 * quad + i;
        const float dd = (o < A.O && qvalid) ? o4[t][i] - A.target[(size_t)qi * A.O + o] : 0.f;
        se = fmaf(dd, dd, se);
        g0[t][i] = dd * gs;
      }
#pragma unroll
    for (int o = 32; o > 0; o >>= 1) se += __shfl_xor(se, o, 64);
    if (lane == 0) atomicAdd(A.loss, se * A.inv_n);
  } else {
#pragma unroll
  for (int t = 0; t < 2; ++t)
#pragma unroll
    for (int i = 0; i < 4; ++i) {
      const int o = 16 * t + 4 * quad + i;
      g0[t][i] = (o < A.O && qvalid) ? A.dout[(size_t)qi * A.O + o] : 0.f;
    }
  }
  Frags<BF16, 1> F1;
  make_frags<BF16, 1>(F1, g0);
  f32x4 c[NT];
  zero_tiles<NT>(c);
  tail_gemm<LA2, 1, NT, BF16, PG2, PG0, T::ST_O2>(c, F1, P, ring, (unsigned)A.L.gto4, (unsigned)A.L.gto2, (unsigned)A.L.gto0, lane);
  {
    f32x4 pre[NT];
    load_rows<NT>(pre, act + 2 * HD + D, quad);
#pragma unroll
    for (int t = 0; t < NT; ++t)
#pragma unroll
      for (int i = 0; i < 4; ++i) c[t][i] *= gelu_grad_f(pre[t][i]);
    if constexpr (WG) {
      if (qvalid) store_rows<NT>(c, tdel + 2 * HD + D, quad);
#pragma unroll
      for (int t = 0; t < NT; ++t)
#pragma unroll
        for (int i = 0; i < 4; ++i) pre[t][i] = gelu_f(pre[t][i]);
      if (qvalid) store_rows<NT>(pre, act + 2 * HD + D, quad);
    }
  }
  Frags<BF16, KB> FD;
  make_frags<BF16, KB>(FD, c);
  zero_tiles<NT>(c);
  tail_gemm<LA2, KB, NT, BF16, PG0, PGH, T::ST_G0>(c, FD, P, ring, (unsigned)A.L.gto2, (unsigned)A.L.gto0, (unsigned)A.L.gtf1, lane);
  {
    f32x4 pre[NT];
    load_rows<NT>(pre, act + 2 * HD, quad);
#pragma unroll
    for (int t = 0; t < NT; ++t)
#pragma unroll
      for (int i = 0; i < 4; ++i) c[t][i] *= gelu_grad_f(pre[t][i]);
    if constexpr (WG) {
      if (qvalid) store_rows<NT>(c, tdel + 2 * HD, quad);
#pragma unroll
      for (int t = 0; t < NT; ++t)
#pragma unroll
        for (int i = 0; i < 4; ++i) pre[t][i] = gelu_f(pre[t][i]);
      if (qvalid) store_rows<NT>(pre, act + 2 * HD, quad);
    }
  }
  make_frags<BF16, KB>(FD, c);
  f32x4 a[NTH];
  zero_tiles<NTH>(a);
  tail_gemm<LA2, KB, NTH, BF16, PGH, PGH, T::ST_TB>(a, FD, P, ring, (unsigned)A.L.gto0, (unsigned)A.L.gtf1, (unsigned)A.L.gtb, lane);
  {
    f32x4 pre[NTH];
    load_rows<NTH>(pre, act + HD, quad);
#pragma unroll
    for (int t = 0; t < NTH; ++t)
#pragma unroll
      for (int i = 0; i < 4; ++i) a[t][i] *= gelu_grad_f(pre[t][i]);
    if constexpr (WG) {
      if (qvalid) store_rows<NTH>(a, tdel + HD, quad);
#pragma unroll
      for (int t = 0; t < NTH; ++t)
#pragma unroll
        for (int i = 0; i < 4; ++i) pre[t][i] = gelu_f(pre[t][i]);
      if (qvalid) store_rows<NTH>(pre, act + HD, quad);
    }
  }
  Frags<BF16, KBH> FH;
  make_frags<BF16, KBH>(FH, a);
  zero_tiles<NTH>(a);
  tail_gemm<LA2, KBH, NTH, BF16, PGH, NoPan, T::ST_TB>(a, FH, P, ring, (unsigned)A.L.gtf1, (unsigned)A.L.gtb, NO_STAGE, lane);
  {
    f32x4 pre[NTH];
    load_rows<NTH>(pre, act, quad);
    const float mu = act[T::ACT - 2], rstd = act[T::ACT - 1];
    float s1 = 0.f, s2 = 0.f;
#pragma unroll
    for (int t = 0; t < NTH; ++t)
#pragma unroll
      for (int i = 0; i < 4; ++i) {
        const float nh = (gelu_f(pre[t][i]) - mu) * rstd;
        s1 += a[t][i]; s2 = fmaf(a[t][i], nh, s2);
      }
    const float m1 = xquad_sum(s1) * A.inv_hd, m2 = xquad_sum(s2) * A.inv_hd;
#pragma unroll
    for (int t = 0; t < NTH; ++t)
#pragma unroll
      for (int i = 0; i < 4; ++i) {
        const float nh = (gelu_f(pre[t][i]) - mu) * rstd;
        a[t][i] = rstd * (a[t][i] - m1 - nh * m2) * gelu_grad_f(pre[t][i]);
        if constexpr (WG) pre[t][i] = nh;
      }
    if constexpr (WG) {
      if (qvalid) store_rows<NTH>(a, tdel, quad);
      if (qvalid) store_rows<NTH>(pre, act, quad);
    }
  }
  make_frags<BF16, KBH>(FH, a);
  zero_tiles<NTH>(a);
  tail_gemm<LA2, KBH, NTH, BF16, NoPan, NoPan, 1024>(a, FH, P, ring, (unsigned)A.L.gtb, NO_STAGE, NO_STAGE, lane);
  f32x4 y[NTH];
  load_rows<NTH>(y, yrow, quad);
#pragma unroll
  for (int h = 0; h < H; ++h) {
    float s = 0.f;
#pragma unroll
    for (int t = 0; t < NT; ++t)
#pragma unroll
      for (int i = 0; i < 4; ++i) s = fmaf(a[h * NT + t][i], y[h * NT + t][i], s);
    s = xquad_sum(s);
    if (quad == 0 && qvalid) A.delta[(size_t)qi * H + h] = s;
  }
  if (qvalid) store_rows<NTH>(a, A.dybar + (size_t)qi * HD, quad);
}

template <int D, int H, bool BF16>
static int launch_tail(const TailArgs& A, bool bwd, bool opt, hipStream_t st) {
  const bool wg = bwd && A.tdel != nullptr;
  const bool fused_loss = bwd && A.target != nullptr;
  using T = TailCfg<D, H, BF16>;
  dim3 grid((A.NQ + 16 * NWAVES - 1) / (16 * NWAVES));
  const bool la2 = grid.x <= 256;
  static EnfAttrBits attr_done[4][2][2];
  auto go = [&](void (*kern_ptr)(TailArgs)) -> int {
    const int smem = la2 ? T::SMEM3 : T::SMEM;
    if (!enf_lds_attr(reinterpret_cast<const void*>(kern_ptr), smem, attr_done[fused_loss ? 3 : (wg ? 2 : bwd)][la2][opt])) return ENF_ELAUNCH;
    hipLaunchKernelGGL(kern_ptr, grid, dim3(NTHREADS), smem, st, A);
    return hipGetLastError() == hipSuccess ? 0 : ENF_ELAUNCH;
  };
  if (fused_loss) {
    if (wg || opt) return ENF_EINVAL;
    return la2 ? go(enf_tail_bwd_kernel<D, H, BF16, true, true, false, true>) : go(enf_tail_bwd_kernel<D, H, BF16, false, true, false, true>);
  }
  if (wg) {
    if (la2) return opt ? go(enf_tail_bwd_kernel<D, H, BF16, true, false, true>) : go(enf_tail_bwd_kernel<D, H, BF16, true, true, true>);
    return opt ? go(enf_tail_bwd_kernel<D, H, BF16, false, false, true>) : go(enf_tail_bwd_kernel<D, H, BF16, false, true, true>);
  }
  if (bwd) {
    if (la2) return opt ? go(enf_tail_bwd_kernel<D, H, BF16, true, false>) : go(enf_tail_bwd_kernel<D, H, BF16, true, true>);
    return opt ? go(enf_tail_bwd_kernel<D, H, BF16, false, false>) : go(enf_tail_bwd_kernel<D, H, BF16, false, true>);
  }
  if (la2) return opt ? go(enf_tail_fwd_kernel<D, H, BF16, true, true>) : go(enf_tail_fwd_kernel<D, H, BF16, true, false>);
  return opt ? go(enf_tail_fwd_kernel<D, H, BF16, false, true>) : go(enf_tail_fwd_kernel<D, H, BF16, false, false>);
}

int enf_launch_tail(const EnfDims& m, const EnfLayout& L, const char* blob, const float* ybar, float* out,
                    const float* dout, float* dybar, float* delta, float* act, int bwd, int opt, hipStream_t st) {
  return enf_launch_tail_wg(m, L, blob, ybar, out, dout, dybar, delta, act, nullptr, bwd, opt, st);
}
int enf_launch_tail_wg(const EnfDims& m, const EnfLayout& L, const char* blob, const float* ybar, float* out,
                       const float* dout, float* dybar, float* delta, float* act, float* tdel, int bwd, int opt, hipStream_t st) {
  if (m.OB != 1) return ENF_EUNSUPPORTED;
  TailArgs A;
  A.target = nullptr; A.loss = nullptr; A.gscale = 0.f; A.inv_n = 0.f;
  A.tdel = tdel;
  A.ybar_half = (!bwd && (opt & 2) && m.bf16) ? 1 : 0;
  opt &= 1;
  A.ybar = ybar; A.blob = blob; A.L = L; A.out = out; A.dout = dout; A.dybar = dybar; A.delta = delta; A.act = act;
  A.NQ = m.B * m.N; A.O = m.O; A.inv_hd = 1.0f / (float)(m.Ht * m.Dt);
#define ENF_CASE(DD, HH)                                                                   \
  if (m.D == DD && m.H == HH) return m.bf16 ? launch_tail<DD, HH, true>(A, bwd != 0, opt != 0, st) : launch_tail<DD, HH, false>(A, bwd != 0, opt != 0, st);
  ENF_CASE(128, 2)
  ENF_CASE(64, 2)
  ENF_CASE(128, 1)
  ENF_CASE(64, 1)
  ENF_CASE(64, 4)
#undef ENF_CASE
  return ENF_EUNSUPPORTED;
}

int enf_launch_tail_loss(const EnfDims& m, const EnfLayout& L, const char* blob, const float* ybar, const float* target,
                         float gscale, float* loss, float* dybar, float* delta, float* act, hipStream_t st) {
  if (m.OB != 1) return ENF_EUNSUPPORTED;
  TailArgs A;
  A.ybar = ybar; A.blob = blob; A.L = L; A.out = nullptr; A.dout = nullptr; A.dybar = dybar; A.delta = delta; A.act = act; A.tdel = nullptr;
  A.ybar_half = 0;
  A.target = target; A.loss = loss; A.gscale = gscale; A.inv_n = 1.0f / ((float)m.B * (float)m.N * (float)m.O);
  A.NQ = m.B * m.N; A.O = m.O; A.inv_hd = 1.0f / (float)(m.Ht * m.Dt);
#define ENF_CASE(DD, HH)                                                                   \
  if (m.D == DD && m.H == HH) return m.bf16 ? launch_tail<DD, HH, true>(A, true, false, st) : launch_tail<DD, HH, false>(A, true, false, st);
  ENF_CASE(128, 2)
  ENF_CASE(64, 2)
  ENF_CASE(128, 1)
  ENF_CASE(64, 1)
  ENF_CASE(64, 4)
#undef ENF_CASE
  return ENF_EUNSUPPORTED;
}
```

enf-pde_amd/enf/models/__init__.py:

```python
import ctypes
import math

import torch

from .. import steerable_attention
from ..steerable_attention.invariant import BaseInvariant
from ... import _lib
from . import _pad

__all__ = ["EquivariantCrossAttentionNeF", "TENSOR_PATHS", "FFN_TENSOR_PATHS", "tensor_paths"]

_BLK = "cross_attention_blocks_0"
TENSOR_PATHS = [
    ("latent_stem", "kernel"), ("latent_stem", "bias"),
    (_BLK, "layer_norm_attn", "scale"), (_BLK, "layer_norm_attn", "bias"),
    (_BLK, "attn", "invariant_embedding_query", "encoding", "coefficients"),
    (_BLK, "attn", "invariant_embedding_query", "layers_0", "linear", "kernel"),
    (_BLK, "attn", "invariant_embedding_query", "layers_0", "linear", "bias"),
    (_BLK, "attn", "invariant_embedding_query", "linear_final", "kernel"),
    (_BLK, "attn", "invariant_embedding_query", "linear_final", "bias"),
    (_BLK, "attn", "invariant_embedding_value", "encoding", "coefficients"),
    (_BLK, "attn", "invariant_embedding_value", "layers_0", "linear", "kernel"),
    (_BLK, "attn", "invariant_embedding_value", "layers_0", "linear", "bias"),
    (_BLK, "attn", "invariant_embedding_value", "linear_final", "kernel"),
    (_BLK, "attn", "invariant_embedding_value", "linear_final", "bias"),
    (_BLK, "attn", "inv_emb_to_q", "kernel"), (_BLK, "attn", "inv_emb_to_q", "bias"),
    (_BLK, "attn", "a_to_k", "kernel"), (_BLK, "attn", "a_to_k", "bias"),
    (_BLK, "attn", "a_to_v", "kernel"), (_BLK, "attn", "a_to_v", "bias"),
    (_BLK, "attn", "inv_emb_to_v", "Dense_0", "kernel"), (_BLK, "attn", "inv_emb_to_v", "Dense_0", "bias"),
    (_BLK, "attn", "inv_emb_to_v", "LayerNorm_0", "scale"), (_BLK, "attn", "inv_emb_to_v", "LayerNorm_0", "bias"),
    (_BLK, "attn", "inv_emb_to_v", "Dense_1", "kernel"), (_BLK, "attn", "inv_emb_to_v", "Dense_1", "bias"),
    (_BLK, "attn", "inv_emb_cond_mixer", "Dense_0", "kernel"), (_BLK, "attn", "inv_emb_cond_mixer", "Dense_0", "bias"),
    (_BLK, "attn", "inv_emb_cond_mixer", "LayerNorm_0", "scale"), (_BLK, "attn", "inv_emb_cond_mixer", "LayerNorm_0", "bias"),
    (_BLK, "attn", "inv_emb_cond_mixer", "Dense_1", "kernel"), (_BLK, "attn", "inv_emb_cond_mixer", "Dense_1", "bias"),
    (_BLK, "attn", "out_proj", "kernel"), (_BLK, "attn", "out_proj", "bias"),
    (_BLK, "pointwise_ffn", "Dense_0", "kernel"), (_BLK, "pointwise_ffn", "Dense_0", "bias"),
    (_BLK, "pointwise_ffn", "LayerNorm_0", "scale"), (_BLK, "pointwise_ffn", "LayerNorm_0", "bias"),
    (_BLK, "pointwise_ffn", "Dense_1", "kernel"), (_BLK, "pointwise_ffn", "Dense_1", "bias"),
    ("out_proj", "layers_0", "kernel"), ("out_proj", "layers_0", "bias"),
    ("out_proj", "layers_2", "kernel"), ("out_proj", "layers_2", "bias"),
    ("out_proj", "layers_4", "kernel"), ("out_proj", "layers_4", "bias"),
]
assert len(TENSOR_PATHS) == _lib.ENF_NUM_TENSORS
BLOCK_PATHS = [t[1:] for t in TENSOR_PATHS if t[0] == _BLK]


def _ffn_paths(branch):
    e = (_BLK, "attn", f"invariant_embedding_{branch}")
    return [e + ("Dense_0", "kernel"), None, e + ("Dense_0", "bias"), e + ("Dense_1", "kernel"), e + ("Dense_1", "bias")]


FFN_TENSOR_PATHS = TENSOR_PATHS[:4] + _ffn_paths("query") + _ffn_paths("value") + TENSOR_PATHS[14:]
assert len(FFN_TENSOR_PATHS) == _lib.ENF_NUM_TENSORS


def tensor_paths(num_layers=0):
    return TENSOR_PATHS + [(f"self_attention_blocks_{i}",) + t for i in range(num_layers) for t in BLOCK_PATHS]


def _get(tree, path):
    for k in path:
        tree = tree[k]
    return tree


def _set(tree, path, value):
    for k in path[:-1]:
        tree = tree.setdefault(k, {})
    tree[path[-1]] = value


def _ptr(t):
    return ctypes.c_void_p(t.data_ptr()) if t is not None else ctypes.c_void_p(0)


FUSED_FIT_STEP = __import__("os").environ.get("ENF_FIT_STEP") != "0"


class _EnfFunction(torch.autograd.Function):

    @staticmethod
    def forward(ctx, x, p, a, sigma, model, packed):
        lib = _lib.load()
        B, Z = p.shape[0], p.shape[1]
        N = x.shape[1]
        desc = model._desc(B, N, Z, masks=model._masks)
        xb, xstride = model._x_arg(x)
        p_, a_ = p.contiguous(), a.contiguous()
        s_ = sigma.contiguous() if sigma is not None else None
        dev = p.device
        out = torch.empty((B, N, model.num_out), device=dev, dtype=torch.float32)
        HD = model._Hp * model._Dp
        no_grad = not any(ctx.needs_input_grad[:4])
        ybar = None if no_grad else torch.empty((B, N, HD), device=dev, dtype=torch.float32)
        lse = None if no_grad else torch.empty((B, N, model._Hp), device=dev, dtype=torch.float32)
        ws = model._workspace(desc, dev)
        st = ctypes.c_void_p(torch.cuda.current_stream(dev).cuda_stream)
        ctx.tail_saved = any(ctx.needs_input_grad[1:4])
        lt_key = (ws.data_ptr(), packed.data_ptr(), B, Z) + tuple((t.data_ptr(), t._version) for t in (p_, a_) + ((s_,) if s_ is not None else ()))
        held = model._lt_held.get(ws.data_ptr())
        reuse_lt = held is not None and held[0] == lt_key and held[1] == model._ws_tags.get(ws.data_ptr())
        stages = (14 if reuse_lt else 15) | (16 if ctx.tail_saved else 0) | (64 if no_grad else 0)
        _lib.launch(dev, lib.enf_forward_stages, ctypes.byref(desc), _ptr(xb), xstride, _ptr(p_), _ptr(a_), _ptr(s_), _ptr(packed),
                                          _ptr(out), _ptr(ybar), _ptr(lse), _ptr(ws), ws.numel(), stages, st)
        ctx.ws_tag = model._ws_touch(ws)
        model._lt_held[ws.data_ptr()] = (lt_key, ctx.ws_tag[1], (p_, a_, s_, packed))
        ctx.model = model
        ctx.has_sigma = sigma is not None
        ctx.xstride = xstride
        if not no_grad:
            ctx.save_for_backward(xb, p_, a_, s_ if s_ is not None else p_.new_empty(0), packed, ybar, lse)
        return out

    @staticmethod
    @torch.autograd.function.once_differentiable
    def backward(ctx, dout):
        lib = _lib.load()
        model = ctx.model
        xb, p_, a_, s_, packed, ybar, lse = ctx.saved_tensors
        sigma = s_ if ctx.has_sigma else None
        B, Z = p_.shape[0], p_.shape[1]
        N = ybar.shape[1]
        desc = model._desc(B, N, Z)
        dev = p_.device
        dout = dout.contiguous().float()
        dp = torch.empty_like(p_)
        da = torch.empty_like(a_)
        dsig = torch.empty((B, Z, 1), device=dev, dtype=torch.float32)
        ws = model._workspace(desc, dev)
        st = ctypes.c_void_p(torch.cuda.current_stream(dev).cuda_stream)
        reuse = 1 if model._ws_tag(ws) == ctx.ws_tag else 0
        if reuse and ctx.tail_saved:
            reuse |= 2
        _lib.launch(dev, lib.enf_backward_latents_ex, ctypes.byref(desc), _ptr(xb), ctx.xstride, _ptr(p_), _ptr(a_), _ptr(sigma),
                                               _ptr(packed), _ptr(ybar), _ptr(lse), _ptr(dout), _ptr(dp), _ptr(da),
                                               _ptr(dsig), _ptr(ws), ws.numel(), reuse, st)
        model._ws_touch(ws)
        return None, dp, da, (dsig if ctx.has_sigma else None), None, None


class EquivariantCrossAttentionNeF:

    default_pair_variants = ("auto", "auto")

    def __init__(self, num_hidden, num_heads, num_layers, num_out, latent_dim, cross_attn_invariant,
                 self_attn_invariant=None, embedding_type="rff", embedding_freq_multiplier=(0.05, 0.1),
                 condition_value_transform=True, use_gaussian_window=True, precision="bf16"):
        if not isinstance(cross_attn_invariant, BaseInvariant):
            raise TypeError("cross_attn_invariant must come from enf.steerable_attention.invariant.get_ca_invariant")
        if embedding_type not in ("rff", "ffn"):
            if embedding_type == "polynomial":
                raise NotImplementedError(f"embedding type '{embedding_type}' is outside the accelerated path "
                                          "(no shipped config selects it; SURVEY.md 2, row 2)")
            raise ValueError(f"Unknown embedding type: {embedding_type}.")
        if embedding_type == "ffn":
            if int(num_layers) > 0:
                raise NotImplementedError("embedding type 'ffn' is built for num_layers = 0 only (no latent self-attention)")
            if cross_attn_invariant.name in ("ball", "ball_lat"):
                raise NotImplementedError(f"embedding type 'ffn' is not built for the '{cross_attn_invariant.name}' invariant")
        if not condition_value_transform:
            raise NotImplementedError("condition_value_transform=False is not on the accelerated path")
        if embedding_type == "rff":
            assert not num_hidden % 2, "For the Fourier Features hidden_dim should be even to calculate them correctly."
        elif num_hidden % 2:
            raise NotImplementedError(f"embedding type 'ffn' is built for an even num_hidden, not {num_hidden}")
        if precision not in _lib.PREC:
            raise ValueError(f"unknown precision {precision!r}")
        self.num_hidden, self.num_heads, self.num_layers = int(num_hidden), int(num_heads), int(num_layers)
        self._Dp = _pad.padded_width(self.num_hidden)
        self._Hp = _pad.padded_heads(self.num_heads)
        if self._Hp == 4 and self._Dp != 64:
            raise NotImplementedError("3 or 4 heads are built for num_hidden <= 64 only")
        self.num_out, self.latent_dim = int(num_out), int(latent_dim)
        self.cross_attn_invariant = cross_attn_invariant
        self.self_attn_invariant = self_attn_invariant if self_attn_invariant is not None else cross_attn_invariant
        if self.num_layers > 0:
            if self.self_attn_invariant.name not in _lib.INVARIANT_IDS:
                raise NotImplementedError(f"self-attention with the '{self.self_attn_invariant.name}' invariant is not built")
        self.embedding_type = embedding_type
        self.embedding_freq_multiplier = tuple(embedding_freq_multiplier)
        self.condition_value_transform = condition_value_transform
        self.use_gaussian_window = bool(use_gaussian_window)
        self.precision = precision
        self._pack_cache = {}
        self._ws_cache = {}
        self._ws_gen = 0
        self._ws_tags = {}
        self._lt_held = {}
        self.pair_variants = None
        self._masks = None

    def with_precision(self, precision):
        import copy
        if precision not in _lib.PREC:
            raise ValueError(f"unknown precision {precision!r}")
        m = copy.copy(self)
        m.precision = precision
        m._pack_cache, m._ws_cache, m._ws_gen, m._ws_tags, m._masks, m._lt_held = {}, {}, 0, {}, None, {}
        return m

    def _desc(self, B, N, Z, masks=None):
        inv = self.cross_attn_invariant
        return _lib.make_desc(B, N, Z, self._Hp, self._Dp, self.latent_dim, self.num_out,
                              inv.num_x_pos_dims, inv.kernel_id, self.use_gaussian_window, _lib.PREC[self.precision],
                              d_true=self.num_hidden if self._Dp != self.num_hidden else 0,
                              h_true=self.num_heads if self._Hp != self.num_heads else 0,
                              variants=tuple(_lib.VARIANT[v] for v in (self.pair_variants or self.default_pair_variants)),
                              masks=masks, embedding=_lib.EMB[self.embedding_type])

    def _workspace(self, desc, device):
        lib = _lib.load()
        nbytes = lib.enf_workspace_bytes(ctypes.byref(desc))
        if nbytes == 0:
            _lib.check(lib.enf_check_desc(ctypes.byref(desc)))
        key = (str(device), torch.cuda.current_stream(device).cuda_stream)
        ws = self._ws_cache.get(key)
        if ws is None or ws.numel() < nbytes:
            ws = torch.empty(int(nbytes), device=device, dtype=torch.uint8)
            self._ws_cache[key] = ws
        return ws

    def _ws_touch(self, ws):
        self._ws_gen += 1
        self._ws_tags[ws.data_ptr()] = self._ws_gen
        return (ws.data_ptr(), self._ws_gen)

    def _ws_tag(self, ws):
        return (ws.data_ptr(), self._ws_tags.get(ws.data_ptr()))

    @staticmethod
    def _x_arg(x):
        if x.dim() != 3:
            raise ValueError("x must be (batch, num_coords, coord_dim)")
        if x.stride(0) == 0:
            return x[0].contiguous(), 0
        xc = x.contiguous()
        return xc, xc.shape[1] * xc.shape[2]

    def init(self, key, x=None, p=None, a=None, gaussian_window_size=None, device=None):
        if device is None:
            device = p.device if p is not None else torch.device("cuda")
        g = key if isinstance(key, torch.Generator) else torch.Generator().manual_seed(int(key))
        D, H, C, O = self.num_hidden, self.num_heads, self.latent_dim, self.num_out
        I = self.cross_attn_invariant.dim
        HD = H * D

        def normal(shape, std):
            return torch.randn(shape, generator=g) * std

        def lecun(n_in, n_out):
            t = torch.empty(n_in, n_out)
            torch.nn.init.trunc_normal_(t, mean=0.0, std=1.0, a=-2.0, b=2.0, generator=g)
            return {"kernel": t * (math.sqrt(1.0 / n_in) / 0.87962566103423978), "bias": torch.zeros(n_out)}

        def ln(n):
            return {"scale": torch.ones(n), "bias": torch.zeros(n)}

        def ffn(n_in, n_hid, n_out):
            return {"Dense_0": lecun(n_in, n_hid), "LayerNorm_0": ln(n_hid), "Dense_1": lecun(n_hid, n_out)}

        def rff(std):
            lim = math.sqrt(3 * 2.0 / D)
            return {"encoding": {"coefficients": normal((I, D // 2), std)},
                    "layers_0": {"linear": {"kernel": normal((D, D), math.sqrt(2.0 / D)), "bias": normal((D,), 1e-6)}},
                    "linear_final": {"kernel": (torch.rand((D, D), generator=g) * 2 - 1) * lim, "bias": normal((D,), 1e-6)}}

        def ffn_emb():
            return {"Dense_0": lecun(I, D), "Dense_1": lecun(D, D)}

        fq, fv = self.embedding_freq_multiplier
        emb_q, emb_v = (ffn_emb(), ffn_emb()) if self.embedding_type == "ffn" else (rff(fq), rff(fv))
        attn = {"invariant_embedding_query": emb_q, "invariant_embedding_value": emb_v,
                "inv_emb_to_q": lecun(D, HD), "a_to_k": lecun(D, HD), "a_to_v": lecun(D, HD),
                "inv_emb_to_v": ffn(D, D, 2 * HD), "inv_emb_cond_mixer": ffn(D, D, D), "out_proj": lecun(HD, HD)}
        P = {"latent_stem": lecun(C, D),
             _BLK: {"layer_norm_attn": ln(D), "attn": attn, "pointwise_ffn": ffn(HD, HD, HD)},
             "out_proj": {"layers_0": lecun(HD, D), "layers_2": lecun(D, D), "layers_4": lecun(D, O)}}
        Is = self.self_attn_invariant.dim
        for i in range(self.num_layers):
            def rff_s(std):
                r = rff(std)
                r["encoding"]["coefficients"] = normal((Is, D // 2), std)
                return r
            P[f"self_attention_blocks_{i}"] = {
                "layer_norm_attn": ln(D),
                "attn": {"invariant_embedding_query": rff_s(fq), "invariant_embedding_value": rff_s(fv),
                         "inv_emb_to_q": lecun(D, HD), "a_to_k": lecun(D, HD), "a_to_v": lecun(D, HD),
                         "inv_emb_to_v": ffn(D, D, 2 * HD), "inv_emb_cond_mixer": ffn(D, D, D), "out_proj": lecun(HD, D)},
                "pointwise_ffn": ffn(D, D, D)}

        def to_dev(t):
            return {k: to_dev(v) for k, v in t.items()} if isinstance(t, dict) else t.to(device=device, dtype=torch.float32)
        return {"params": to_dev(P)}

    def tensor_paths(self):
        return FFN_TENSOR_PATHS if self.embedding_type == "ffn" else tensor_paths(self.num_layers)

    def param_tensors(self, params):
        P = params["params"] if "params" in params else params
        paths = self.tensor_paths()
        dev = _get(P, paths[0]).device
        return [torch.empty(0, device=dev) if path is None else _get(P, path) for path in paths]

    def invalidate_caches(self):
        self._pack_cache.clear()
        self._lt_held.clear()
        self._pair_key = None
        self._pair_blob = None
        self._train_blob = None

    def load_params(self, tree, device="cuda"):
        self.invalidate_caches()
        P = tree["params"] if "params" in tree else tree
        out = {}
        for path in self.tensor_paths():
            if path is not None:
                _set(out, path, torch.as_tensor(_get(P, path)).to(device=device, dtype=torch.float32).contiguous())
        return {"params": out}

    def pack(self, params):
        lib = _lib.load()
        ts = self.param_tensors(params)[:_lib.ENF_NUM_TENSORS]
        dev = ts[0].device
        if dev.type != "cuda":
            raise _lib.EnfError("parameters must live on the GPU: the decoder has no CPU path")
        key = (self.precision, tuple((t.data_ptr(), t._version) if t is not None else None for t in ts))
        hit = self._pack_cache.get("k")
        if hit is not None and hit[0] == key:
            return hit[1]
        desc = self._desc(1, 1, 1)
        _lib.check(lib.enf_check_desc(ctypes.byref(desc)))
        ts = [t.detach().to(torch.float32).contiguous() if t is not None else None for t in ts]
        self._check_shapes(ts)
        if self._Dp != self.num_hidden or self._Hp != self.num_heads:
            ts = [t.contiguous() if t is not None else None
                  for t in _pad.pad_tensors(ts, self.num_hidden, self._Dp, self.num_heads, self._Hp, ffn=self.embedding_type == "ffn")]
        nbytes = lib.enf_packed_weight_bytes(ctypes.byref(desc))
        blob = torch.empty(int(nbytes), device=dev, dtype=torch.uint8)
        arr = (ctypes.c_void_p * len(ts))(*[t.data_ptr() if t is not None else None for t in ts])
        st = ctypes.c_void_p(torch.cuda.current_stream(dev).cuda_stream)
        _lib.launch(dev, lib.enf_pack_weights, ctypes.byref(desc), arr, _ptr(blob), st)
        self._pack_cache["k"] = (key, blob, ts)
        return blob

    def _check_shapes(self, ts):
        shp_done = []
        for t, shp, path in zip(ts, self._expected_shapes(), self.tensor_paths()):
            if shp is None:
                if t is not None and t.numel():
                    raise ValueError(f"the ffn embedding has no tensor in ENF_W_* slot {len(shp_done)}")
                shp_done.append(None)
                continue
            shp_done.append(shp)
            if t is None:
                raise ValueError(f"parameter {'/'.join(path)} is missing")
            if tuple(t.shape) != shp:
                raise ValueError(f"parameter {'/'.join(path)} has shape {tuple(t.shape)}, expected {shp}")

    def _expected_shapes(self):
        D, H, C, O, I = self.num_hidden, self.num_heads, self.latent_dim, self.num_out, self.cross_attn_invariant.dim
        HD = H * D
        rff = [(I, D), None, (D,), (D, D), (D,)] if self.embedding_type == "ffn" else [(I, D // 2), (D, D), (D,), (D, D), (D,)]
        return ([(C, D), (D,), (D,), (D,)] + rff + rff + [(D, HD), (HD,)] * 3 +
                [(D, D), (D,), (D,), (D,), (D, 2 * HD), (2 * HD,)] + [(D, D), (D,), (D,), (D,), (D, D), (D,)] +
                [(HD, HD), (HD,)] + [(HD, HD), (HD,), (HD,), (HD,), (HD, HD), (HD,)] +
                [(HD, D), (D,), (D, D), (D,), (D, O), (O,)])

    def apply(self, params, x, p, a, gaussian_window_size=None):
        inv = self.cross_attn_invariant
        if not (x.is_cuda and p.is_cuda and a.is_cuda):
            raise _lib.EnfError("EquivariantCrossAttentionNeF.apply needs CUDA/HIP tensors: there is no CPU path")
        if x.shape[-1] != inv.num_x_pos_dims:
            raise AssertionError(f"x has coordinate width {x.shape[-1]}, invariant '{inv.name}' expects {inv.num_x_pos_dims}")
        if p.shape[-1] != inv.num_z_pos_dims + inv.num_z_ori_dims:
            raise AssertionError(f"p has width {p.shape[-1]}, expected {inv.num_z_pos_dims + inv.num_z_ori_dims}")
        if a.shape[-1] != self.latent_dim:
            raise AssertionError(f"a has width {a.shape[-1]}, expected latent_dim={self.latent_dim}")
        if x.shape[0] != p.shape[0] or a.shape[:2] != p.shape[:2]:
            raise AssertionError("batch / latent dimensions of x, p, a disagree")
        sigma = gaussian_window_size if self.use_gaussian_window else None
        if self.use_gaussian_window and sigma is None:
            raise AssertionError("gaussian_window_size is required when use_gaussian_window=True")
        if sigma is not None and not torch.is_tensor(sigma):
            sigma = torch.full((p.shape[0], p.shape[1], 1), float(sigma), device=p.device)
        x, p, a = x.float(), p.float(), a.float()
        if sigma is not None:
            sigma = sigma.float().reshape(p.shape[0], p.shape[1], 1)
        ts = self.param_tensors(params)
        if self.num_layers > 0:
            from . import _train
            self._check_shapes(ts)
            return _train.apply_layers(self, ts, x, p, a, sigma)
        if torch.is_grad_enabled() and (x.requires_grad or any(t is not None and t.requires_grad for t in ts)):
            from . import _train
            self._check_shapes(ts)
            return _train.apply_train(self, ts, x, p, a, sigma)
        packed = self.pack(params)
        return _EnfFunction.apply(x, p, a, sigma, self, packed)

    __call__ = apply

    def relu_mask_buffer(self, B, N, Z, device):
        desc = self._desc(B, N, Z)
        return torch.empty(int(_lib.load().enf_relu_mask_bytes(ctypes.byref(desc))) // 4, device=device, dtype=torch.int32)

    def relu_masks(self, buf, mode, signals):
        import contextlib
        if mode not in ("write", "read"):
            raise ValueError("mode must be 'write' or 'read'")

        @contextlib.contextmanager
        def cm():
            prev, self._masks = self._masks, (buf, mode, int(signals))
            try:
                yield buf
            finally:
                self._masks = prev
        return cm()

    @torch.no_grad()
    def mse_value_and_latent_grads(self, params, x, p, a, gaussian_window_size, target, grad_scale=1.0, loss_out=None):
        lib = _lib.load()
        sigma = gaussian_window_size if self.use_gaussian_window else None
        if self.num_layers > 0:
            with torch.enable_grad():
                leaves = [t.detach().float().requires_grad_(True) for t in (p, a)] + \
                         ([sigma.detach().float().requires_grad_(True)] if sigma is not None else [])
                out = self.apply(params, x, leaves[0], leaves[1], leaves[2] if sigma is not None else None)
                loss = ((out - target) ** 2).mean()
                g = torch.autograd.grad(loss * grad_scale, leaves, allow_unused=True)
            g = [torch.zeros_like(t) if gi is None else gi for t, gi in zip(leaves, g)]
            if loss_out is not None:
                loss_out.add_(loss.detach().reshape(1))
            return loss.detach().reshape(1), g[0], g[1], (g[2] if sigma is not None else None)
        packed = self.pack(params)
        x, p_, a_ = x.float(), p.float().contiguous(), a.float().contiguous()
        s_ = sigma.float().reshape(p_.shape[0], p_.shape[1], 1).contiguous() if sigma is not None else None
        B, Z, N, dev = p_.shape[0], p_.shape[1], x.shape[1], p_.device
        desc = self._desc(B, N, Z, masks=self._masks)
        xb, xstride = self._x_arg(x)
        ws = self._workspace(desc, dev)
        st = ctypes.c_void_p(torch.cuda.current_stream(dev).cuda_stream)
        tgt = target.float().contiguous()
        if tuple(tgt.shape) != (B, N, self.num_out):
            raise AssertionError(f"target has shape {tuple(tgt.shape)}, expected {(B, N, self.num_out)}")
        loss = loss_out if loss_out is not None else torch.zeros(1, device=dev, dtype=torch.float32)
        dp, da = torch.empty_like(p_), torch.empty_like(a_)
        dsig = torch.empty((B, Z, 1), device=dev, dtype=torch.float32)
        if not FUSED_FIT_STEP:
            HD = self._Hp * self._Dp
            out = torch.empty((B, N, self.num_out), device=dev, dtype=torch.float32)
            ybar = torch.empty((B, N, HD), device=dev, dtype=torch.float32)
            lse = torch.empty((B, N, self._Hp), device=dev, dtype=torch.float32)
            _lib.launch(dev, lib.enf_forward_stages, ctypes.byref(desc), _ptr(xb), xstride, _ptr(p_), _ptr(a_), _ptr(s_), _ptr(packed),
                        _ptr(out), _ptr(ybar), _ptr(lse), _ptr(ws), ws.numel(), 15 | 16 | 32, st)
            dout = torch.empty_like(out)
            _lib.launch(dev, lib.enf_mse_value_grad, _ptr(out), _ptr(tgt), out.numel(), float(grad_scale), _ptr(dout), _ptr(loss), st)
            _lib.launch(dev, lib.enf_backward_latents_ex, ctypes.byref(desc), _ptr(xb), xstride, _ptr(p_), _ptr(a_), _ptr(s_),
                        _ptr(packed), _ptr(ybar), _ptr(lse), _ptr(dout), _ptr(dp), _ptr(da), _ptr(dsig), _ptr(ws), ws.numel(), 1 | 2 | 4, st)
            self._ws_touch(ws)
            return loss, dp, da, (dsig if sigma is not None else None)
        _lib.launch(dev, lib.enf_fit_step, ctypes.byref(desc), _ptr(xb), xstride, _ptr(p_), _ptr(a_), _ptr(s_), _ptr(packed), _ptr(tgt),
                    float(grad_scale), _ptr(loss), _ptr(dp), _ptr(da), _ptr(dsig), _ptr(ws), ws.numel(), st)
        self._ws_touch(ws)
        return loss, dp, da, (dsig if sigma is not None else None)
```

enf-pde_amd/fitting/inner_loop.py:

```python
import ctypes

import torch

from .. import _lib


def default_meta_sgd_lrs(latent_dim, lr_p=1.0, lr_a=5.0, lr_window=0.0, with_ori=False, device="cuda"):
    lrs = {"p_pos": torch.full((1,), lr_p, device=device), "a": torch.full((latent_dim,), lr_a, device=device),
           "gaussian_window": torch.full((1,), lr_window, device=device)}
    if with_ori:
        lrs["p_ori"] = torch.full((1,), lr_p, device=device)
    return lrs


def make_masks(num_coords, num_sampled, num_inner_steps, generator=None, device="cuda"):
    cols = [torch.randperm(num_coords, generator=generator)[:num_sampled] for _ in range(num_inner_steps + 1)]
    return torch.stack(cols, dim=1).to(device)


FUSED_FIT_INPUTS = __import__("os").environ.get("ENF_FIT_INPUTS") != "0"


def _fit_inputs(latents0, coords, img, masks):
    ts = list(latents0.values()) + [coords, img]
    if not (img.is_cuda and masks.is_cuda and masks.dtype == torch.int64 and masks.dim() == 2 and masks.is_contiguous() and coords.dim() == 2
            and img.dim() == 3 and 1 <= len(latents0) <= _lib.ENF_SGD_MAX_SEGMENTS and masks.shape[0] > 0
            and all(t.dtype == torch.float32 and t.is_contiguous() and t.device == img.device for t in ts)
            and all(v.dim() == 3 and v.shape[0] == 1 for v in latents0.values())
            and len({v.shape[1] for v in latents0.values()}) == 1):
        return None
    B, N, O = img.shape
    Ns, S1 = masks.shape
    Z = next(iter(latents0.values())).shape[1]
    dev = img.device
    lat = {k: torch.empty((B, Z, v.shape[2]), device=dev, dtype=torch.float32) for k, v in latents0.items()}
    xs = torch.empty((S1, Ns, coords.shape[1]), device=dev, dtype=torch.float32)
    ys = torch.empty((S1, B, Ns, O), device=dev, dtype=torch.float32)
    losses = torch.empty(S1, device=dev, dtype=torch.float32)
    comps = (_lib.EnfFitComponent * _lib.ENF_SGD_MAX_SEGMENTS)()
    keep = []
    for i, (k, v) in enumerate(latents0.items()):
        src = v.detach()
        keep.append(src)
        comps[i] = _lib.EnfFitComponent(src.data_ptr(), lat[k].data_ptr(), v.shape[2], 0)
    st = ctypes.c_void_p(torch.cuda.current_stream(dev).cuda_stream)
    _lib.launch(dev, _lib.load().enf_fit_inputs, len(latents0), comps, B, Z, N, Ns, S1, coords.shape[1], O, coords.data_ptr(), img.data_ptr(),
                masks.data_ptr(), xs.data_ptr(), ys.data_ptr(), losses.data_ptr(), st)
    return lat, xs, ys, losses


def _pose(lat, num_ori_dims):
    return torch.cat((lat["p_pos"], lat["p_ori"]), dim=-1) if num_ori_dims > 0 else lat["p_pos"]


def meta_sgd_update(lat, grads, lrs, scale):
    lib = _lib.load()
    new = dict(lat)
    segs = (_lib.EnfSgdSegment * _lib.ENF_SGD_MAX_SEGMENTS)()
    keep = []
    for i, (k, g) in enumerate(grads.items()):
        x = lat[k].float().contiguous()
        w = x.shape[-1]
        if g.dtype != torch.float32 or g.shape != x.shape or g.stride(-1) != 1 or \
                any(g.stride(d) != g.stride(d + 1) * g.shape[d + 1] for d in range(g.dim() - 2)):
            g = g.float().contiguous()
        lr = lrs[k].detach().float().contiguous()
        out = torch.empty_like(x)
        keep += [x, g, lr]
        segs[i] = _lib.EnfSgdSegment(x.data_ptr(), g.data_ptr(), lr.data_ptr(), out.data_ptr(), x.numel(), w,
                                     g.stride(-2) if g.dim() > 1 else w, lr.numel(), 0)
        new[k] = out
    st = ctypes.c_void_p(torch.cuda.current_stream(out.device).cuda_stream)
    _lib.launch(out.device, lib.enf_meta_sgd_update, len(grads), segs, float(scale), st)
    return new


def inner_loop(nef, nef_params, latents0, lrs, coords, img, masks, optimize_gaussian_window=False,
               noise_pos=0.0, generator=None):
    B = img.shape[0]
    S = masks.shape[1] - 1
    n_ori = nef.cross_attn_invariant.num_z_ori_dims
    fused = _fit_inputs(latents0, coords, img, masks) if FUSED_FIT_INPUTS else None
    if fused is not None:
        lat, xs_all, ys_all, losses = fused
    else:
        lat = {k: v.detach().repeat_interleave(B, dim=0) for k, v in latents0.items()}
        masks_t = masks.t().contiguous()
        xs_all = coords[masks_t]
        ys_all = img[:, masks_t].transpose(0, 1).float().contiguous()
        losses = torch.zeros(S + 1, device=img.device, dtype=torch.float32)
    if noise_pos:
        lat["p_pos"] = lat["p_pos"] + torch.randn(lat["p_pos"].shape, generator=generator,
                                                  device="cpu").to(lat["p_pos"].device) * noise_pos
    n_pos = lat["p_pos"].shape[-1]
    for s in range(S):
        xs = xs_all[s][None].expand(B, -1, -1)
        _, dp, da, dsig = nef.mse_value_and_latent_grads(nef_params, xs, _pose(lat, n_ori), lat["a"],
                                                         lat.get("gaussian_window"), ys_all[s], loss_out=losses[s:s + 1])
        grads = {"p_pos": dp[..., :n_pos], "a": da}
        if n_ori > 0:
            grads["p_ori"] = dp[..., n_pos:]
        if optimize_gaussian_window and dsig is not None:
            grads["gaussian_window"] = dsig
        lat = meta_sgd_update(lat, grads, lrs, B)
    with torch.no_grad():
        xs = xs_all[S][None].expand(B, -1, -1)
        out = nef.apply(nef_params, xs, _pose(lat, n_ori), lat["a"], lat.get("gaussian_window")).float().contiguous()
        st = ctypes.c_void_p(torch.cuda.current_stream(out.device).cuda_stream)
        if out.shape != ys_all[S].shape:
            raise AssertionError(f"targets have shape {tuple(ys_all[S].shape)}, expected {tuple(out.shape)}")
        _lib.launch(out.device, _lib.load().enf_mse_value_grad, out.data_ptr(), ys_all[S].data_ptr(), out.numel(), 1.0, None,
                    losses[S:].data_ptr(), st)
    return losses[S], lat


@torch.no_grad()
def decode(nef, nef_params, coords, p, a, window, chunk=None):
    B = p.shape[0]
    x = coords[None].expand(B, -1, -1) if coords.dim() == 2 else coords
    if chunk is None:
        return nef.apply(nef_params, x, p, a, window)
    outs = [nef.apply(nef_params, x[:, i:i + chunk], p, a, window) for i in range(0, x.shape[1], chunk)]
    return torch.cat(outs, dim=1)
```

include/enf_hip.h:

```cpp
#ifndef ENF_HIP_H
#define ENF_HIP_H

#include <stddef.h>
#include <stdint.h>

#ifdef __cplusplus
extern "C" {
#endif

#define ENF_ABI_VERSION 2

enum {
  ENF_INV_REL_POS_PERIODIC = 0,
  ENF_INV_LATITUDE_PERIODIC = 1,
  ENF_INV_POLAR_PERIODIC = 2,
  ENF_INV_PONITA = 3,
  ENF_INV_ABS_POS = 4,
  ENF_INV_REL_POS = 5,
  ENF_INV_NORM_REL_POS = 6,
  ENF_INV_BALL = 7,
  ENF_INV_BALL_LAT = 8,
  ENF_INV_PONITA_FULL = 9,
  ENF_INV_COUNT = 10
};

enum {
  ENF_PREC_F32 = 0,
  ENF_PREC_BF16 = 1
};

enum {
  ENF_VARIANT_AUTO = 0,
  ENF_VARIANT_LATENT_SPLIT = 1,
  ENF_VARIANT_ZFOLD = 2,
  ENF_VARIANT_ZFOLD_ZSPLIT = 3
};

enum {
  ENF_EMB_RFF = 0,
  ENF_EMB_FFN = 1
};

#define ENF_MASK_OFF 0
#define ENF_MASK_WRITE 1
#define ENF_MASK_READ 2

enum {
  ENF_OK = 0,
  ENF_EINVAL = -1,
  ENF_EINVARIANT = -2,
  ENF_EUNSUPPORTED = -3,
  ENF_EWORKSPACE = -4,
  ENF_ELAUNCH = -5,
  ENF_EDIM = -6
};

typedef struct EnfDesc {
  int32_t B, N, Z;
  int32_t H, D, C, O;
  int32_t dx;
  int32_t invariant_id;
  int32_t use_window;
  int32_t precision;
  int32_t h_true;
  int32_t d_true;
  int32_t pair_fwd_variant;
  int32_t pair_bwd_variant;
  int32_t mask_mode;
  int32_t mask_signals;
  int32_t embedding;
  void* relu_masks;
} EnfDesc;

enum {
  ENF_W_STEM_W = 0, ENF_W_STEM_B,
  ENF_W_LNA_G, ENF_W_LNA_B,
  ENF_W_RQ_COEF, ENF_W_RQ_W1, ENF_W_RQ_B1, ENF_W_RQ_W2, ENF_W_RQ_B2,
  ENF_W_RV_COEF, ENF_W_RV_W1, ENF_W_RV_B1, ENF_W_RV_W2, ENF_W_RV_B2,
  ENF_W_Q_W, ENF_W_Q_B,
  ENF_W_K_W, ENF_W_K_B,
  ENF_W_V_W, ENF_W_V_B,
  ENF_W_F1_W0, ENF_W_F1_B0, ENF_W_F1_G, ENF_W_F1_BE, ENF_W_F1_W1, ENF_W_F1_B1,
  ENF_W_MX_W0, ENF_W_MX_B0, ENF_W_MX_G, ENF_W_MX_BE, ENF_W_MX_W1, ENF_W_MX_B1,
  ENF_W_AO_W, ENF_W_AO_B,
  ENF_W_FF_W0, ENF_W_FF_B0, ENF_W_FF_G, ENF_W_FF_BE, ENF_W_FF_W1, ENF_W_FF_B1,
  ENF_W_O0_W, ENF_W_O0_B, ENF_W_O2_W, ENF_W_O2_B, ENF_W_O4_W, ENF_W_O4_B,
  ENF_NUM_TENSORS
};

int enf_abi_version(void);
const char* enf_strerror(int code);

int enf_invariant_dim(int invariant_id, int dx);
int enf_invariant_pose_dim(int invariant_id, int dx);

int enf_check_desc(const EnfDesc* d);

size_t enf_packed_weight_bytes(const EnfDesc* d);
int enf_pack_weights(const EnfDesc* d, const float* const* tensors, void* packed, void* stream);

size_t enf_workspace_bytes(const EnfDesc* d);

int enf_forward(const EnfDesc* d, const float* x, int64_t x_bstride, const float* p, const float* a,
                const float* sigma, const void* packed, float* out, float* ybar, float* lse,
                void* workspace, size_t workspace_bytes, void* stream);

#define ENF_STAGE_PROLOGUE 1u
#define ENF_STAGE_PAIR 2u
#define ENF_STAGE_TAIL 4u
#define ENF_STAGE_FOLD 8u
#define ENF_STAGE_TAIL_SAVE 16u
#define ENF_STAGE_PREPARE_BWD 32u
#define ENF_STAGE_YBAR_HALF 64u
int enf_forward_stages(const EnfDesc* d, const float* x, int64_t x_bstride, const float* p, const float* a,
                       const float* sigma, const void* packed, float* out, float* ybar, float* lse,
                       void* workspace, size_t workspace_bytes, unsigned stages, void* stream);

int enf_backward_latents(const EnfDesc* d, const float* x, int64_t x_bstride, const float* p,
                         const float* a, const float* sigma, const void* packed, const float* ybar,
                         const float* lse, const float* dout, float* dp, float* da, float* dsigma,
                         void* workspace, size_t workspace_bytes, void* stream);
#define ENF_BWD_REUSE_PROLOGUE 1u
#define ENF_BWD_REUSE_TAIL 2u
#define ENF_BWD_REUSE_PREPARED 4u
#define ENF_BWD_ONLY_PAIR 8u
int enf_backward_latents_ex(const EnfDesc* d, const float* x, int64_t x_bstride, const float* p,
                         const float* a, const float* sigma, const void* packed, const float* ybar,
                         const float* lse, const float* dout, float* dp, float* da, float* dsigma,
                         void* workspace, size_t workspace_bytes, unsigned flags, void* stream);

enum {
  ENF_P_AQ1 = 0, ENF_P_BQ1,
  ENF_P_AV1, ENF_P_BV1,
  ENF_P_AF, ENF_P_BF,
  ENF_P_AGB, ENF_P_BGB,
  ENF_P_AM, ENF_P_BM,
  ENF_P_COEFQ, ENF_P_COEFV,
  ENF_NUM_PAIR_TENSORS
};
enum { ENF_S_EQ = 0, ENF_S_EV, ENF_S_G1, ENF_S_NH, ENF_S_DA1, ENF_S_DA2, ENF_S_DA3, ENF_S_HEAD0  };
#define ENF_NUM_STORE(H) (7 + 4 * (H))

int enf_lt_layout(const EnfDesc* d, int* stride, int* off_u, int* off_v0, int* off_pose, int* off_wcoef, int* off_c);
int enf_lt_layout_ext(const EnfDesc* d, int* off_ext, int* off_phase_q, int* off_phase_v);
int enf_pack_pair(const EnfDesc* d, const float* const* pair_tensors, void* packed, void* stream);
size_t enf_pair_scratch_bytes(const EnfDesc* d);
int enf_pair_forward(const EnfDesc* d, const float* x, int64_t x_bstride, const float* lt, const void* packed,
                     float* ybar, float* lse, void* scratch, size_t scratch_bytes, void* stream);
int enf_pair_backward(const EnfDesc* d, const float* x, int64_t x_bstride, const float* lt, const void* packed,
                      const float* lse, const float* dybar, const float* delta, float* dlt, void* const* store,
                      void* stream);
int enf_pair_backward_ex(const EnfDesc* d, const float* x, int64_t x_bstride, const float* lt, const void* packed,
                         const float* lse, const float* dybar, const float* delta, float* dlt, void* const* store,
                         float* dx, void* stream);

size_t enf_relu_mask_bytes(const EnfDesc* d);

int enf_fit_step(const EnfDesc* d, const float* x, int64_t x_bstride, const float* p, const float* a, const float* sigma,
                 const void* packed, const float* target, float grad_scale, float* loss, float* dp, float* da, float* dsigma,
                 void* workspace, size_t workspace_bytes, void* stream);

int enf_mse_value_grad(const float* out, const float* target, size_t n, float grad_scale, float* dout, float* loss,
                       void* stream);

#define ENF_SGD_MAX_SEGMENTS 4
typedef struct EnfSgdSegment {
  const float* x;
  const float* g;
  const float* lr;
  float* out;
  int64_t n;
  int32_t width, g_stride, lr_len, reserved;
} EnfSgdSegment;
int enf_meta_sgd_update(int nseg, const EnfSgdSegment* segs, float scale, void* stream);

typedef struct EnfFitComponent {
  const float* src;
  float* dst;
  int32_t width, reserved;
} EnfFitComponent;
int enf_fit_inputs(int ncomp, const EnfFitComponent* comps, int32_t B, int32_t Z, int32_t N, int32_t Ns, int32_t S1, int32_t dx, int32_t O,
                   const float* coords, const float* img, const int64_t* masks, float* xs, float* ys, float* losses, void* stream);

int enf_ode_conv_forward(int B, int Z, int J, int C, const float* a, const float* kb, int64_t kb_stride_r,
                         int64_t kb_stride_s, const float* W, const float* bias, float* out, void* stream);
int enf_ode_conv_backward_basis(int B, int Z, int J, int C, const float* a, const float* g, const float* W, float* dkb,
                                void* stream);
size_t enf_ode_conv_backward_weight_scratch_bytes(int B, int Z, int J, int C);
int enf_ode_conv_backward_weight(int B, int Z, int J, int C, const float* a, const float* kb, const float* g, float* dW,
                                 void* scratch, size_t scratch_bytes, void* stream);
int enf_ode_poly_num_features(int I, int degree);
int enf_ode_poly_forward(int64_t P, int I, int degree, const float* x, float* feat, void* stream);
int enf_ode_poly_backward(int64_t P, int I, int degree, const float* x, const float* dfeat, float* dx, void* stream);
int enf_ode_vec_readout_forward(int B, int Z, int I, int D, const float* inv, const float* aw, const float* u, const float* w,
                                float cr, float cs, const float* Wi, float* out, void* stream);
int enf_ode_vec_readout_backward(int B, int Z, int I, int D, const float* inv, const float* aw, const float* u, const float* w,
                                 float cr, float cs, const float* Wi, const float* g, float* dinv, float* daw, float* du,
                                 float* dw, float* dWi_part, void* stream);
int enf_ode_block_supported(int H, int M);
size_t enf_ode_block_scratch_bytes(int64_t R, int H, int M);
int enf_ode_block_forward(int64_t R, int H, int M, const float* x, const float* gamma, const float* beta, const float* W1,
                          const float* b1, const float* W2, const float* b2, float eps, float* out, float* pre, void* stream);
int enf_ode_block_backward(int64_t R, int H, int M, const float* x, const float* gamma, const float* beta, const float* W1,
                           const float* W2, const float* pre, const float* g, float eps, float* dx, float* dparams,
                           void* scratch, size_t scratch_bytes, void* stream);
int enf_ode_basis_supported(int I, int degree, int H1, int J, int backward);
size_t enf_ode_basis_scratch_bytes(int64_t P, int I, int H1, int J, int backward);
int enf_ode_basis_forward(int64_t P, int I, int degree, int H1, int J, const float* inv, const float* W1, const float* b1,
                          const float* W3, const float* b3, float* kb, void* scratch, size_t scratch_bytes, void* stream);
int enf_ode_basis_backward(int64_t P, int I, int degree, int H1, int J, const float* inv, const float* W1, const float* b1,
                           const float* W3, const float* b3, const float* dkb, float* dinv, float* dW1, float* db1,
                           float* dW3, float* db3, void* scratch, size_t scratch_bytes, void* stream);

size_t enf_backward_all_scratch_bytes(const EnfDesc* d, int chunk_signals);
int enf_backward_all(const EnfDesc* d, const float* x, int64_t x_bstride, const float* p, const float* a, const float* sigma,
                     const float* const* tensors, const void* packed, const float* ybar, const float* lse, const float* dout,
                     float* dp, float* da, float* dsigma, float* const* dW, float* dx, void* workspace, size_t workspace_bytes,
                     void* scratch, size_t scratch_bytes, unsigned flags, void* stream);

size_t enf_backward_weights_scratch_bytes(const EnfDesc* d, int chunk_signals);
int enf_backward_weights(const EnfDesc* d, const float* x, int64_t x_bstride, const float* lt, const void* packed,
                         const float* lse, const float* dybar, const float* delta, float* dlt, float* const* dpair,
                         float* dx, void* scratch, size_t scratch_bytes, void* stream);

int enf_pair_variant(const EnfDesc* d, int backward);
int enf_pair_partition(const EnfDesc* d, int32_t* run, int32_t* workgroups, int32_t* parts);

#ifdef __cplusplus
}
#endif
#endif
```

Baseline: 26.71 million.

## Run whole inner fit loop in native code with fused boundary kernel

Adds an enf_fit_loop entry point that drives every inner-loop step from C++. Latents are ping-ponged between two buffers, and a new boundary kernel fuses the previous step's prologue-backward, the meta-SGD update and the next step's prologue. The final step gets a forward-plus-loss tail kernel that can read a half-precision ybar. The goal is to remove per-step Python and ctypes dispatch and several separate kernel launches. In exchange it adds much new code and is only taken when the model has no extra layers and no position noise is applied.

```diff
diff --git a/enf-pde_amd/_lib.py b/enf-pde_amd/_lib.py
--- a/enf-pde_amd/_lib.py
+++ b/enf-pde_amd/_lib.py
@@ -14,7 +14,7 @@
            "enf_packed_weight_bytes", "enf_pack_weights", "enf_workspace_bytes", "enf_forward",
            "enf_backward_latents", "enf_backward_latents_ex", "enf_forward_stages", "enf_lt_layout", "enf_lt_layout_ext", "enf_pack_pair", "enf_pair_forward",
            "enf_pair_backward", "enf_pair_backward_ex", "enf_pair_scratch_bytes", "enf_pair_variant", "enf_pair_partition", "enf_backward_weights", "enf_backward_weights_scratch_bytes",
-           "enf_backward_all", "enf_backward_all_scratch_bytes", "enf_fit_step", "enf_fit_inputs",
+           "enf_backward_all", "enf_backward_all_scratch_bytes", "enf_fit_step", "enf_fit_inputs", "enf_fit_loop", "enf_fit_loop_workspace_bytes",
            "enf_mse_value_grad",
            "enf_ode_conv_forward", "enf_ode_conv_backward_basis", "enf_ode_conv_backward_weight", "enf_ode_conv_backward_weight_scratch_bytes", "enf_ode_poly_num_features", "enf_ode_poly_forward",
            "enf_ode_poly_backward", "enf_ode_vec_readout_forward", "enf_ode_vec_readout_backward", "enf_ode_block_supported", "enf_ode_block_scratch_bytes", "enf_ode_block_forward", "enf_ode_block_backward",
@@ -52,6 +52,12 @@
 
 class EnfFitComponent(ctypes.Structure):
     _fields_ = [("src", ctypes.c_void_p), ("dst", ctypes.c_void_p), ("width", ctypes.c_int32), ("reserved", ctypes.c_int32)]
+
+
+class EnfFitLatents(ctypes.Structure):
+    _fields_ = [("p", ctypes.c_void_p * 2), ("a", ctypes.c_void_p * 2), ("sigma", ctypes.c_void_p * 2),
+                ("lr_pos", ctypes.c_void_p), ("lr_ori", ctypes.c_void_p), ("lr_a", ctypes.c_void_p), ("lr_sigma", ctypes.c_void_p),
+                ("n_pos", ctypes.c_int32), ("lr_pos_len", ctypes.c_int32), ("lr_ori_len", ctypes.c_int32), ("lr_a_len", ctypes.c_int32)]
 
 
 class EnfError(RuntimeError):
@@ -149,6 +155,9 @@
     lib.enf_backward_weights_scratch_bytes.argtypes = [dp, ci]
     lib.enf_backward_weights.argtypes = [dp, vp, i64, vp, vp, vp, vp, vp, vp, ctypes.POINTER(vp), vp, vp, sz, vp]
     lib.enf_fit_step.argtypes = [dp, vp, i64, vp, vp, vp, vp, vp, ctypes.c_float, vp, vp, vp, vp, vp, sz, vp]
+    lib.enf_fit_loop_workspace_bytes.restype = sz
+    lib.enf_fit_loop_workspace_bytes.argtypes = [dp]
+    lib.enf_fit_loop.argtypes = [dp, ctypes.POINTER(EnfFitLatents), vp, vp, vp, ctypes.c_float, ci, vp, ctypes.c_uint, vp, sz, vp]
     lib.enf_backward_all_scratch_bytes.restype = sz
     lib.enf_backward_all_scratch_bytes.argtypes = [dp, ci]
     lib.enf_backward_all.argtypes = [dp, vp, i64, vp, vp, vp, ctypes.POINTER(vp), vp, vp, vp, vp, vp, vp, vp, ctypes.POINTER(vp), vp,
@@ -164,6 +173,8 @@
         lib.enf_debug_gemm.argtypes = [vp, vp, vp, ci, ci, ci, vp]
         lib.enf_debug_pack.argtypes = [vp, vp, ci, ci, ci, vp]
         lib.enf_test_read_wave_sums.argtypes = [vp]
+        lib.enf_test_boundary.restype = ci
+        lib.enf_test_boundary.argtypes = [dp, vp, ctypes.POINTER(EnfFitLatents), ci, ci, ctypes.c_float] + [vp] * 8
     if lib.enf_abi_version() != 2:
         raise EnfError(f"{path}: ABI version mismatch")
     return lib
diff --git a/enf-pde_amd/csrc/enf_api.hip b/enf-pde_amd/csrc/enf_api.hip
--- a/enf-pde_amd/csrc/enf_api.hip
+++ b/enf-pde_amd/csrc/enf_api.hip
@@ -241,6 +241,77 @@
   return enf_launch_prologue_bwd(m, c.L, c.blob, p, sigma, c.F(W.an), c.F(W.kv), c.F(W.dlt), dp, da, dsigma, st);
 }
 
+struct FitLoopScratch { size_t dp, da, dsigma, total; };
+static FitLoopScratch fit_loop_scratch(const EnfDims& m) {
+  FitLoopScratch s;
+  const size_t BZ = (size_t)m.B * m.Z;
+  s.dp = enf_workspace(m).total;
+  s.da = s.dp + enf_align(sizeof(float) * BZ * m.dp);
+  s.dsigma = s.da + enf_align(sizeof(float) * BZ * m.C);
+  s.total = s.dsigma + enf_align(sizeof(float) * BZ);
+  return s;
+}
+
+extern "C" size_t enf_fit_loop_workspace_bytes(const EnfDesc* d) {
+  if (enf_check_desc(d) != ENF_OK) return 0;
+  return fit_loop_scratch(enf_dims(d)).total;
+}
+
+extern "C" int enf_fit_loop(const EnfDesc* d, const EnfFitLatents* lat, const float* xs, const float* ys, const void* packed,
+                            float grad_scale, int steps, float* losses, unsigned flags, void* workspace, size_t workspace_bytes,
+                            void* stream) {
+  EnfCall c;
+  const bool ptrs = lat && xs && ys && losses && lat->p[0] && lat->p[1] && lat->a[0] && lat->a[1] && lat->lr_pos && lat->lr_a;
+  int rc = enf_call(c, d, ptrs, lat ? lat->sigma[0] : nullptr, packed, workspace, workspace_bytes, stream);
+  if (rc) return rc;
+  const EnfDims& m = c.m;
+  const EnfWorkspace& W = c.W;
+  hipStream_t st = c.st;
+  if (steps < 0 || flags != 0) return ENF_EINVAL;
+  if (lat->n_pos < 1 || lat->n_pos > m.dp || (lat->n_pos < m.dp && !lat->lr_ori)) return ENF_EDIM;
+  if ((lat->lr_pos_len != 1 && lat->lr_pos_len != lat->n_pos) || (lat->lr_a_len != 1 && lat->lr_a_len != m.C) ||
+      (lat->n_pos < m.dp && lat->lr_ori_len != 1 && lat->lr_ori_len != m.dp - lat->n_pos))
+    return ENF_EDIM;
+  if (lat->lr_sigma && (!lat->sigma[0] || !lat->sigma[1])) return ENF_EINVAL;
+  const FitLoopScratch S = fit_loop_scratch(m);
+  if (workspace_bytes < S.total) return ENF_EWORKSPACE;
+  const bool zf = enf_use_zfold(m), zb = enf_use_zfold_bwd(m);
+  const size_t nx = (size_t)m.N * m.dx, ny = (size_t)m.B * m.N * m.O;
+  if ((rc = enf_side_join_pending(st, workspace))) return rc;
+  EnfBoundary b{};
+  b.lr_pos = lat->lr_pos; b.lr_ori = lat->lr_ori; b.lr_a = lat->lr_a; b.lr_sigma = lat->lr_sigma;
+  b.n_pos = lat->n_pos; b.lr_pos_len = lat->lr_pos_len; b.lr_ori_len = lat->lr_ori_len; b.lr_a_len = lat->lr_a_len;
+  b.dp = c.F(S.dp); b.da = c.F(S.da); b.dsigma = c.F(S.dsigma);
+  b.scale = grad_scale;
+  const float* sigma = lat->sigma[0];
+  for (int s = 0; s <= steps; ++s) {
+    const int cur = s & 1, prev = cur ^ 1;
+    b.first = s == 0;
+    b.p = lat->p[b.first ? 0 : prev]; b.a = lat->a[b.first ? 0 : prev]; b.sigma = b.first ? lat->sigma[0] : sigma;
+    b.p_next = lat->p[cur]; b.a_next = lat->a[cur]; b.sigma_next = lat->sigma[cur];
+    if ((rc = enf_launch_boundary(m, c.L, c.blob, b, c.F(W.lt), c.F(W.an), c.F(W.kv), c.F(W.dlt), st))) return rc;
+    if (!b.first && lat->lr_sigma) sigma = lat->sigma[cur];
+    const float* x = xs + (size_t)s * nx;
+    if (s == steps) break;
+    if ((rc = enf_launch_pair_fwd(m, c.L, c.blob, x, 0, c.F(W.lt), c.F(W.ybar), c.F(W.lse), zf ? c.ws + W.wz : nullptr,
+                                  zf ? c.F(W.wzb) : nullptr, zf ? c.ws + W.wzu : nullptr, enf_zfold_split(m) > 1 ? c.F(W.ysplit) : nullptr, 1, 1, st)))
+      return rc;
+    if ((rc = side_prepare_bwd(zb ? side_stream() : nullptr, c, false)) < 0) return rc;
+    if (!rc && zb && (rc = enf_launch_wz(m, c.L, c.blob, c.F(W.lt), nullptr, c.F(W.wzb), nullptr, c.ws + W.wzt, st))) return rc;
+    if ((rc = enf_launch_tail_loss(m, c.L, c.blob, c.F(W.ybar), ys + (size_t)s * ny, 1.0f, losses + s, c.F(W.dybar), c.F(W.delta),
+                                   c.F(W.tail_act), st)))
+      return rc;
+    if ((rc = enf_side_join_pending(st, workspace))) return rc;
+    if ((rc = pair_bwd_on_workspace(c, x, 0, c.F(W.lse)))) return rc;
+  }
+  const bool yhalf = m.bf16 && enf_zfold_split(m) <= 1;
+  if ((rc = enf_launch_pair_fwd(m, c.L, c.blob, xs + (size_t)steps * nx, 0, c.F(W.lt), c.F(W.ybar), c.F(W.lse), zf ? c.ws + W.wz : nullptr,
+                                zf ? c.F(W.wzb) : nullptr, zf ? c.ws + W.wzu : nullptr, enf_zfold_split(m) > 1 ? c.F(W.ysplit) : nullptr, 1,
+                                1 | (yhalf ? 2 : 0), st)))
+    return rc;
+  return enf_launch_tail_fwd_loss(m, c.L, c.blob, c.F(W.ybar), yhalf ? 1 : 0, ys + (size_t)steps * ny, losses + steps, st);
+}
+
 extern "C" int enf_lt_layout(const EnfDesc* d, int* stride, int* off_u, int* off_v0, int* off_pose, int* off_wcoef, int* off_c) {
   int rc = enf_check_desc(d);
   if (rc) return rc;
diff --git a/enf-pde_amd/csrc/enf_debug.hip b/enf-pde_amd/csrc/enf_debug.hip
--- a/enf-pde_amd/csrc/enf_debug.hip
+++ b/enf-pde_amd/csrc/enf_debug.hip
@@ -40,3 +40,40 @@
 #undef C
   return ENF_EUNSUPPORTED;
 }
+
+extern "C" int enf_test_boundary(const EnfDesc* d, const void* packed, const EnfFitLatents* lat, int first, int fused, float scale, float* lt,
+                                 float* an, float* kv, float* dlt, float* dp, float* da, float* dsigma, void* stream) {
+  const int rc0 = enf_check_desc(d);
+  if (rc0) return rc0;
+  const EnfDims m = enf_dims(d);
+  const EnfLayout L = enf_layout(m);
+  hipStream_t st = (hipStream_t)stream;
+  const char* blob = (const char*)packed;
+  float* sig1 = lat->lr_sigma ? lat->sigma[1] : lat->sigma[0];
+  if (fused) {
+    EnfBoundary b{};
+    b.p = lat->p[0]; b.a = lat->a[0]; b.sigma = lat->sigma[0];
+    b.p_next = lat->p[1]; b.a_next = lat->a[1]; b.sigma_next = lat->sigma[1];
+    b.lr_pos = lat->lr_pos; b.lr_ori = lat->lr_ori; b.lr_a = lat->lr_a; b.lr_sigma = lat->lr_sigma;
+    b.n_pos = lat->n_pos; b.lr_pos_len = lat->lr_pos_len; b.lr_ori_len = lat->lr_ori_len; b.lr_a_len = lat->lr_a_len;
+    b.dp = dp; b.da = da; b.dsigma = dsigma; b.first = first; b.scale = scale;
+    return enf_launch_boundary(m, L, blob, b, lt, an, kv, dlt, st);
+  }
+  int rc;
+  if (first) {
+    if ((rc = enf_launch_prologue(m, L, blob, lat->p[0], lat->a[0], lat->sigma[0], lt, an, kv, st))) return rc;
+  } else {
+    if ((rc = enf_launch_prologue_bwd(m, L, blob, lat->p[0], lat->sigma[0], an, kv, dlt, dp, da, dsigma, st))) return rc;
+    const int64_t BZ = (int64_t)m.B * m.Z;
+    const int n_ori = m.dp - lat->n_pos;
+    EnfSgdSegment seg[ENF_SGD_MAX_SEGMENTS];
+    int n = 0;
+    if (n_ori != 0) return ENF_EUNSUPPORTED;
+    seg[n++] = EnfSgdSegment{lat->p[0], dp, lat->lr_pos, lat->p[1], BZ * m.dp, m.dp, m.dp, lat->lr_pos_len, 0};
+    seg[n++] = EnfSgdSegment{lat->a[0], da, lat->lr_a, lat->a[1], BZ * m.C, m.C, m.C, lat->lr_a_len, 0};
+    if (lat->lr_sigma) seg[n++] = EnfSgdSegment{lat->sigma[0], dsigma, lat->lr_sigma, lat->sigma[1], BZ, 1, 1, 1, 0};
+    if ((rc = enf_meta_sgd_update(n, seg, scale, stream))) return rc;
+    if ((rc = enf_launch_prologue(m, L, blob, lat->p[1], lat->a[1], sig1, lt, an, kv, st))) return rc;
+  }
+  return hipMemsetAsync(dlt, 0, enf_lt_bytes(m), st) == hipSuccess ? 0 : ENF_ELAUNCH;
+}
diff --git a/enf-pde_amd/csrc/enf_launch.h b/enf-pde_amd/csrc/enf_launch.h
--- a/enf-pde_amd/csrc/enf_launch.h
+++ b/enf-pde_amd/csrc/enf_launch.h
@@ -48,6 +48,17 @@
                                const float* an, const float* kv, const float* dlt, float* dp, float* da, float* dsigma, float* pg,
                                hipStream_t st);
 
+struct EnfBoundary {
+  const float* p; const float* a; const float* sigma;
+  float* p_next; float* a_next; float* sigma_next;
+  const float* lr_pos; const float* lr_ori; const float* lr_a; const float* lr_sigma;
+  float* dp; float* da; float* dsigma;
+  int n_pos, lr_pos_len, lr_ori_len, lr_a_len, first;
+  float scale;
+};
+int enf_launch_boundary(const EnfDims& m, const EnfLayout& L, const char* blob, const EnfBoundary& b, float* lt, float* an, float* kv,
+                        float* dlt, hipStream_t st);
+
 int enf_launch_wz(const EnfDims& m, const EnfLayout& L, const char* blob, const float* lt, char* wz, float* wzb, char* wzu,
                   char* wzt, hipStream_t st);
 
@@ -81,3 +92,5 @@
                        float* dybar, float* delta, float* act, float* tdel, int bwd, int opt, hipStream_t st);
 int enf_launch_tail_loss(const EnfDims& m, const EnfLayout& L, const char* blob, const float* ybar, const float* target, float gscale,
                          float* loss, float* dybar, float* delta, float* act, hipStream_t st);
+int enf_launch_tail_fwd_loss(const EnfDims& m, const EnfLayout& L, const char* blob, const float* ybar, int ybar_half, const float* target,
+                             float* loss, hipStream_t st);
diff --git a/enf-pde_amd/csrc/enf_prologue.hip b/enf-pde_amd/csrc/enf_prologue.hip
--- a/enf-pde_amd/csrc/enf_prologue.hip
+++ b/enf-pde_amd/csrc/enf_prologue.hip
@@ -27,82 +27,83 @@
   int Dt;
 };
 
-__global__ __launch_bounds__(256) void enf_prologue_kernel(PrologueArgs A) {
-  extern __shared__ __attribute__((aligned(16))) float sm[];
+template <int ZT_, int NTH, class Args>
+static __device__ __forceinline__ void prologue_fwd_body(const Args& A, const float* p, const float* a, const float* sigma, int dpw,
+                                                         float* sm, int row0) {
   const int D = A.D, H = A.H, HD = H * D, C = A.C;
   float* s_a = sm;
-  float* s_an = s_a + ZT * C;
-  float* s_k = s_an + ZT * D;
+  float* s_an = s_a + ZT_ * C;
+  float* s_k = s_an + ZT_ * D;
   const int tid = threadIdx.x, lane = tid & 63, wave = tid >> 6;
-  const int row0 = blockIdx.x * ZT;
+  
   auto W = [&](size_t off) { return reinterpret_cast<const float*>(A.blob + off); };
   const int stride = enf_lt_stride(H, D);
-  for (int i = tid; i < ZT * C; i += 256) {
+  for (int i = tid; i < ZT_ * C; i += NTH) {
     const int zz = i / C, c = i % C, r = row0 + zz;
-    s_a[c * ZT + zz] = r < A.BZ ? A.a[(size_t)r * C + c] : 0.f;
-  }
-  __syncthreads();
-  for (int d = tid; d < D; d += 256) {
-    float acc[ZT];
+    s_a[c * ZT_ + zz] = r < A.BZ ? a[(size_t)r * C + c] : 0.f;
+  }
+  __syncthreads();
+  for (int d = tid; d < D; d += NTH) {
+    float acc[ZT_];
     const float bs = W(A.L.stem_b)[d];
 #pragma unroll
-    for (int zz = 0; zz < ZT; ++zz) acc[zz] = bs;
+    for (int zz = 0; zz < ZT_; ++zz) acc[zz] = bs;
 #pragma unroll PRO_UNROLL
     for (int c = 0; c < C; ++c) {
       const float w = W(A.L.stem_w)[(size_t)c * D + d];
 #pragma unroll
-      for (int q = 0; q < ZT / 4; ++q) {
-        const pf4 x = *reinterpret_cast<const pf4*>(s_a + c * ZT + 4 * q);
+      for (int q = 0; q < ZT_ / 4; ++q) {
+        const pf4 x = *reinterpret_cast<const pf4*>(s_a + c * ZT_ + 4 * q);
 #pragma unroll
         for (int zz = 0; zz < 4; ++zz) acc[4 * q + zz] = fmaf(x[zz], w, acc[4 * q + zz]);
       }
     }
 #pragma unroll
-    for (int zz = 0; zz < ZT; ++zz) s_an[d * ZT + zz] = acc[zz];
-  }
-  __syncthreads();
-  for (int zz = wave; zz < ZT; zz += 4) {
+    for (int zz = 0; zz < ZT_; ++zz) s_an[d * ZT_ + zz] = acc[zz];
+  }
+  __syncthreads();
+  for (int zz = wave; zz < ZT_; zz += NTH / 64) {
     const int r = row0 + zz;
     float v = 0.f;
-    for (int d = lane; d < A.Dt; d += 64) v += s_an[d * ZT + zz];
+    for (int d = lane; d < A.Dt; d += 64) v += s_an[d * ZT_ + zz];
     const float mu = wave_sum(v) / A.Dt;
     float q = 0.f;
-    for (int d = lane; d < A.Dt; d += 64) { const float t = s_an[d * ZT + zz] - mu; q += t * t; }
+    for (int d = lane; d < A.Dt; d += 64) { const float t = s_an[d * ZT_ + zz] - mu; q += t * t; }
     const float rstd = rsqrtf(wave_sum(q) / A.Dt + 1e-6f);
     for (int d = lane; d < D; d += 64) {
-      const float sv = s_an[d * ZT + zz];
+      const float sv = s_an[d * ZT_ + zz];
       const float xn = (sv - mu) * rstd;
       if (r < A.BZ) {
         A.an[(size_t)r * (2 * D + 2) + d] = sv;
         A.an[(size_t)r * (2 * D + 2) + D + d] = xn;
       }
-      s_an[d * ZT + zz] = xn * W(A.L.lna_g)[d] + W(A.L.lna_b)[d];
+      s_an[d * ZT_ + zz] = xn * W(A.L.lna_g)[d] + W(A.L.lna_b)[d];
     }
     if (lane == 0 && r < A.BZ) { A.an[(size_t)r * (2 * D + 2) + 2 * D] = mu; A.an[(size_t)r * (2 * D + 2) + 2 * D + 1] = rstd; }
   }
   __syncthreads();
-  for (int j = tid; j < 2 * HD; j += 256) {
+  for (int j = tid; j < 2 * HD; j += NTH) {
     const bool isv = j >= HD;
     const int jj = isv ? j - HD : j;
     const float* Wm = W(isv ? A.L.wv : A.L.wk);
-    float acc[ZT];
+    float acc[ZT_];
     const float bb = W(isv ? A.L.bv : A.L.bk)[jj];
 #pragma unroll
-    for (int zz = 0; zz < ZT; ++zz) acc[zz] = bb;
+    for (int zz = 0; zz < ZT_; ++zz) acc[zz] = bb;
 #pragma unroll PRO_UNROLL
     for (int d = 0; d < D; ++d) {
       const float w = Wm[(size_t)d * HD + jj];
 #pragma unroll
-      for (int q = 0; q < ZT / 4; ++q) {
-        const pf4 x = *reinterpret_cast<const pf4*>(s_an + d * ZT + 4 * q);
+      for (int q = 0; q < ZT_ / 4; ++q) {
+        const pf4 x = *reinterpret_cast<const pf4*>(s_an + d * ZT_ + 4 * q);
 #pragma unroll
         for (int zz = 0; zz < 4; ++zz) acc[4 * q + zz] = fmaf(x[zz], w, acc[4 * q + zz]);
       }
     }
 #pragma unroll
-    for (int zz = 0; zz < ZT; ++zz) {
+    for (int zz = 0; zz < ZT_; ++zz) {
       const int r = row0 + zz;
-      if (!isv) s_k[jj * ZT + zz] = acc[zz];
+      if (!isv) s_k[jj * ZT_ + zz] = acc[zz];
       if (r < A.BZ) {
         A.kv[(size_t)r * 2 * HD + j] = acc[zz];
         if (isv) A.lt[(size_t)r * stride + enf_lt_off_v0(H, D) + jj] = acc[zz];
@@ -110,47 +111,47 @@
     }
   }
   __syncthreads();
-  for (int j = tid; j < HD; j += 256) {
+  for (int j = tid; j < HD; j += NTH) {
     const int h = j / D, i = j % D;
     const float* mut = W(A.L.mut) + (size_t)h * D * D + i;
-    float acc[ZT];
-#pragma unroll
-    for (int zz = 0; zz < ZT; ++zz) acc[zz] = 0.f;
+    float acc[ZT_];
+#pragma unroll
+    for (int zz = 0; zz < ZT_; ++zz) acc[zz] = 0.f;
 #pragma unroll PRO_UNROLL
     for (int dd = 0; dd < D; ++dd) {
       const float w = mut[(size_t)dd * D];
-      const float* kp = s_k + (h * D + dd) * ZT;
-#pragma unroll
-      for (int q = 0; q < ZT / 4; ++q) {
+      const float* kp = s_k + (h * D + dd) * ZT_;
+#pragma unroll
+      for (int q = 0; q < ZT_ / 4; ++q) {
         const pf4 x = *reinterpret_cast<const pf4*>(kp + 4 * q);
 #pragma unroll
         for (int zz = 0; zz < 4; ++zz) acc[4 * q + zz] = fmaf(x[zz], w, acc[4 * q + zz]);
       }
     }
 #pragma unroll
-    for (int zz = 0; zz < ZT; ++zz) {
+    for (int zz = 0; zz < ZT_; ++zz) {
       const int r = row0 + zz;
       if (r < A.BZ) A.lt[(size_t)r * stride + enf_lt_off_u(H, D) + j] = acc[zz];
     }
   }
-  for (int t = wave; t < ZT * H; t += 4) {
+  for (int t = wave; t < ZT_ * H; t += NTH / 64) {
     const int zz = t / H, h = t % H, r = row0 + zz;
     float sacc = 0.f;
-    for (int dd = lane; dd < D; dd += 64) sacc = fmaf(W(A.L.cvec)[h * D + dd], s_k[(h * D + dd) * ZT + zz], sacc);
+    for (int dd = lane; dd < D; dd += 64) sacc = fmaf(W(A.L.cvec)[h * D + dd], s_k[(h * D + dd) * ZT_ + zz], sacc);
     sacc = wave_sum(sacc);
     if (lane == 0 && r < A.BZ) A.lt[(size_t)r * stride + enf_lt_off_c(H, D) + h] = sacc;
   }
-  if (tid < ZT) {
+  if (tid < ZT_) {
     const int r = row0 + tid;
     if (r < A.BZ) {
-      const float* pp = A.p + (size_t)r * A.dp;
+      const float* pp = p + (size_t)r * dpw;
       float q[4] = {0.f, 0.f, 0.f, 0.f};
       float wc;
-      const float sg = A.sigma ? A.sigma[r] : 1.f;
+      const float sg = sigma ? sigma[r] : 1.f;
       const bool sphere = A.inv == ENF_INV_LATITUDE_PERIODIC || A.inv == ENF_INV_POLAR_PERIODIC || enf_inv_has_phase(A.inv);
       if (A.inv == ENF_INV_PONITA || A.inv == ENF_INV_PONITA_FULL) { q[0] = pp[0]; q[1] = pp[1]; q[2] = cosf(pp[2]); q[3] = sinf(pp[2]); }
       else if (sphere) { q[0] = pp[0]; q[1] = pp[1]; q[2] = sinf(pp[1]); q[3] = cosf(pp[1]); }
-      else { for (int i = 0; i < A.dp && i < 3; ++i) q[i] = pp[i]; }
+      else { for (int i = 0; i < dpw && i < 3; ++i) q[i] = pp[i]; }
       wc = sphere ? 1.f / (2.f * sg * sg) : 1.f / (sg * sg);
       float* o = A.lt + (size_t)r * stride;
       for (int i = 0; i < 4; ++i) o[enf_lt_off_pose(H, D) + i] = q[i];
@@ -173,6 +174,11 @@
       }
     }
   }
+}
+
+__global__ __launch_bounds__(256) void enf_prologue_kernel(PrologueArgs A) {
+  extern __shared__ __attribute__((aligned(16))) float sm[];
+  prologue_fwd_body<ZT, 256>(A, A.p, A.a, A.sigma, A.dp, sm, blockIdx.x * ZT);
 }
 
 int enf_launch_prologue(const EnfDims& m, const EnfLayout& L, const char* blob, const float* p, const float* a,
@@ -396,14 +402,15 @@
   int BZ, H, D, C, dp_dim, inv, Dt;
 };
 
-__global__ __launch_bounds__(64 * PW) void enf_prologue_bwd_mfma_kernel(ProBwdArgs A) {
-  extern __shared__ __attribute__((aligned(16))) float sm[];
+template <class Args>
+static __device__ __forceinline__ void prologue_bwd_mfma_body(const Args& A, const float* p, const float* sigma, float* dp, float* da,
+                                                              float* dsigma, float* pg, int dpw, float* sm, int row0) {
   const int D = A.D, H = A.H, HD = H * D, C = A.C, PGW = 2 * HD + 4 * D;
   float* s_du = sm;
   float* s_dk = s_du + HD * LT;
   float* s_dan = s_dk + 2 * HD * LT;
   float* s_dc = s_dan + D * LT;
-  const int tid = threadIdx.x, lane = tid & 63, wave = tid >> 6, j = lane & 15, q = lane >> 4, row0 = blockIdx.x * LT;
+  const int tid = threadIdx.x, lane = tid & 63, wave = tid >> 6, j = lane & 15, q = lane >> 4;
   const int stride = enf_lt_stride(H, D);
   auto W = [&](size_t off) { return reinterpret_cast<const float*>(A.blob + off); };
   for (int t = tid; t < LT * HD; t += 64 * PW) {
@@ -443,8 +450,8 @@
         const pf4 cv = *reinterpret_cast<const pf4*>(W(A.L.cvec) + f0[t] + 4 * q);
 #pragma unroll
         for (int e = 0; e < 4; ++e) { acc[t][e] = fmaf(cv[e], dc, acc[t][e]); s_dk[(f0[t] + 4 * q + e) * LT + j] = acc[t][e]; }
-        if (A.pg && rok) {
-          float* pr = A.pg + (size_t)r_mine * PGW;
+        if (pg && rok) {
+          float* pr = pg + (size_t)r_mine * PGW;
           const pf4 kq = *reinterpret_cast<const pf4*>(A.kv + (size_t)r_mine * 2 * HD + f0[t] + 4 * q);
           *reinterpret_cast<pf4*>(pr + f0[t] + 4 * q) = acc[t];
           *reinterpret_cast<pf4*>(pr + HD + 4 * D + f0[t] + 4 * q) = pf4{dc * kq[0], dc * kq[1], dc * kq[2], dc * kq[3]};
@@ -473,8 +480,8 @@
     const pf4 g = *reinterpret_cast<const pf4*>(W(A.L.lna_g) + 16 * t + 4 * q);
 #pragma unroll
     for (int e = 0; e < 4; ++e) s_dan[(16 * t + 4 * q + e) * LT + j] = sum[e] * g[e];
-    if (A.pg && rok) {
-      float* pr = A.pg + (size_t)r_mine * PGW + HD;
+    if (pg && rok) {
+      float* pr = pg + (size_t)r_mine * PGW + HD;
       const pf4 xn = *reinterpret_cast<const pf4*>(A.an + (size_t)r_mine * (2 * D + 2) + D + 16 * t + 4 * q);
       const pf4 b = *reinterpret_cast<const pf4*>(W(A.L.lna_b) + 16 * t + 4 * q);
       *reinterpret_cast<pf4*>(pr + 16 * t + 4 * q) = sum;
@@ -494,7 +501,7 @@
     for (int d = l32; d < D; d += 32) {
       const float ds = rstd * (s_dan[d * LT + zz] - m1 - anr[D + d] * m2);
       s_dan[d * LT + zz] = ds;
-      if (A.pg && r < A.BZ) A.pg[(size_t)r * PGW + HD + D + d] = ds;
+      if (pg && r < A.BZ) pg[(size_t)r * PGW + HD + D + d] = ds;
     }
   }
   __syncthreads();
@@ -504,19 +511,19 @@
     if (rok) {
 #pragma unroll
       for (int e = 0; e < 4; ++e)
-        if (16 * t + 4 * q + e < C) A.da[(size_t)r_mine * C + 16 * t + 4 * q + e] = acc[e];
+        if (16 * t + 4 * q + e < C) da[(size_t)r_mine * C + 16 * t + 4 * q + e] = acc[e];
     }
   }
   if (tid < LT) {
     const int r = row0 + tid;
     if (r < A.BZ) {
       const float* g = A.dlt + (size_t)r * stride + enf_lt_off_pose(H, D);
-      const float* pp = A.p + (size_t)r * A.dp_dim;
-      float* o = A.dp + (size_t)r * A.dp_dim;
+      const float* pp = p + (size_t)r * dpw;
+      float* o = dp + (size_t)r * dpw;
       const bool sph = A.inv == ENF_INV_LATITUDE_PERIODIC || A.inv == ENF_INV_POLAR_PERIODIC || enf_inv_has_phase(A.inv);
       if (A.inv == ENF_INV_PONITA || A.inv == ENF_INV_PONITA_FULL) { o[0] = g[0]; o[1] = g[1]; o[2] = -sinf(pp[2]) * g[2] + cosf(pp[2]) * g[3]; }
       else if (sph) { o[0] = g[0]; o[1] = g[1] + cosf(pp[1]) * g[2] - sinf(pp[1]) * g[3]; }
-      else { for (int i = 0; i < A.dp_dim && i < 3; ++i) o[i] = g[i]; }
+      else { for (int i = 0; i < dpw && i < 3; ++i) o[i] = g[i]; }
       if (enf_inv_has_phase(A.inv)) {
         const float* e = A.dlt + (size_t)r * stride + enf_lt_off_ext(H, D);
         if (A.inv == ENF_INV_BALL) {
@@ -530,12 +537,75 @@
           o[3] = e[9];
         } else { o[1] += e[9]; o[2] = 0.f; o[3] = e[10]; }
       }
-      const float sg = A.sigma ? A.sigma[r] : 1.f;
+      const float sg = sigma ? sigma[r] : 1.f;
       const float dwc = A.dlt[(size_t)r * stride + enf_lt_off_wcoef(H, D)];
-      A.dsigma[r] = (sph ? -1.f : -2.f) / (sg * sg * sg) * dwc;
-    }
-  }
-}
+      dsigma[r] = (sph ? -1.f : -2.f) / (sg * sg * sg) * dwc;
+    }
+  }
+}
+
+__global__ __launch_bounds__(64 * PW) void enf_prologue_bwd_mfma_kernel(ProBwdArgs A) {
+  extern __shared__ __attribute__((aligned(16))) float sm[];
+  prologue_bwd_mfma_body(A, A.p, A.sigma, A.dp, A.da, A.dsigma, A.pg, A.dp_dim, sm, blockIdx.x * LT);
+}
+
+struct BoundaryArgs {
+  const char* blob; EnfLayout L;
+  float* lt; float* an; float* kv; float* dlt;
+  int BZ, H, D, C, inv, Dt, dpw;
+  EnfBoundary b;
+};
+
+__global__ __launch_bounds__(64 * PW) void enf_boundary_kernel(BoundaryArgs A) {
+  extern __shared__ __attribute__((aligned(16))) float sm[];
+  const int tid = threadIdx.x, row0 = blockIdx.x * LT, C = A.C, dpw = A.dpw;
+  const int rows = min(LT, A.BZ - row0);
+  const EnfBoundary& b = A.b;
+  const float *p = b.p, *a = b.a, *sigma = b.sigma;
+  if (!b.first) {
+    prologue_bwd_mfma_body(A, b.p, b.sigma, b.dp, b.da, b.dsigma, static_cast<float*>(nullptr), dpw, sm, row0);
+    __syncthreads();
+    for (int t = tid; t < rows * C; t += 64 * PW) {
+      const size_t i = (size_t)row0 * C + t;
+      const int c = t % C;
+      const float g = b.da[i] * b.scale;
+      b.a_next[i] = b.a[i] - b.lr_a[b.lr_a_len == 1 ? 0 : c] * g;
+    }
+    for (int t = tid; t < rows * dpw; t += 64 * PW) {
+      const size_t i = (size_t)row0 * dpw + t;
+      const int c = t % dpw;
+      const float lr = c < b.n_pos ? b.lr_pos[b.lr_pos_len == 1 ? 0 : c] : b.lr_ori[b.lr_ori_len == 1 ? 0 : c - b.n_pos];
+      const float g = b.dp[i] * b.scale;
+      b.p_next[i] = b.p[i] - lr * g;
+    }
+    if (b.lr_sigma && tid < rows) {
+      const float g = b.dsigma[row0 + tid] * b.scale;
+      b.sigma_next[row0 + tid] = b.sigma[row0 + tid] - b.lr_sigma[0] * g;
+    }
+    p = b.p_next; a = b.a_next;
+    if (b.lr_sigma) sigma = b.sigma_next;
+  }
+  {
+    pf4* z = reinterpret_cast<pf4*>(A.dlt + (size_t)row0 * enf_lt_stride(A.H, A.D));
+    for (int t = tid; t < rows * (enf_lt_stride(A.H, A.D) / 4); t += 64 * PW) z[t] = pf4{0.f, 0.f, 0.f, 0.f};
+  }
+  __syncthreads();
+  prologue_fwd_body<LT, 64 * PW>(A, p, a, sigma, dpw, sm, row0);
+}
+}
+
+int enf_launch_boundary(const EnfDims& m, const EnfLayout& L, const char* blob, const EnfBoundary& b, float* lt, float* an, float* kv,
+                        float* dlt, hipStream_t st) {
+  BoundaryArgs A;
+  A.blob = blob; A.L = L; A.lt = lt; A.an = an; A.kv = kv; A.dlt = dlt;
+  A.BZ = m.B * m.Z; A.H = m.H; A.D = m.D; A.C = m.C; A.inv = m.inv; A.Dt = m.Dt; A.dpw = m.dp;
+  A.b = b;
+  const int bwd = 3 * m.HD + m.D + m.H, fwd = m.C + m.D + m.HD;
+  const size_t smem = sizeof(float) * LT * (bwd > fwd ? bwd : fwd);
+  static EnfAttrBits attr{0};
+  if (!enf_lds_attr(reinterpret_cast<const void*>(enf_boundary_kernel), 160 * 1024, attr)) return ENF_ELAUNCH;
+  hipLaunchKernelGGL(enf_boundary_kernel, dim3((A.BZ + LT - 1) / LT), dim3(64 * PW), smem, st, A);
+  return hipGetLastError() == hipSuccess ? 0 : ENF_ELAUNCH;
 }
 
 static int enf_launch_prologue_bwd_mfma(const EnfDims& m, const EnfLayout& L, const char* blob, const float* p, const float* sigma,
diff --git a/enf-pde_amd/csrc/enf_tail.hip b/enf-pde_amd/csrc/enf_tail.hip
--- a/enf-pde_amd/csrc/enf_tail.hip
+++ b/enf-pde_amd/csrc/enf_tail.hip
@@ -173,7 +173,7 @@
   for (int i = tid; i < 32; i += NTHREADS) cst[2 * HD + 2 * D + i] = G(L.bO4)[i];
 }
 
-template <int D, int H, bool BF16, bool LA2, bool SAVE>
+template <int D, int H, bool BF16, bool LA2, bool SAVE, bool LOSS = false>
 __global__ __launch_bounds__(NTHREADS, 2) void enf_tail_fwd_kernel(TailArgs A) {
   using T = TailCfg<D, H, BF16>;
   extern __shared__ __attribute__((aligned(16))) char smem[];
@@ -196,7 +196,21 @@
                          : A.ybar + (size_t)qi * T::HD;
   tail_forward<D, H, BF16, SAVE, LA2, NoPan, NoPan>(o4, yrow, SAVE ? A.act + (size_t)qi * T::ACT : nullptr, A.L,
                                                     cst, P, ring, NO_STAGE, NO_STAGE, lane, quad, A.inv_hd, true, yh);
-  if (q0 + col < A.NQ) {
+  if constexpr (LOSS) {
+    const bool qvalid = q0 + col < A.NQ;
+    float se = 0.f;
+#pragma unroll
+    for (int t = 0; t < 2; ++t)
+#pragma unroll
+      for (int i = 0; i < 4; ++i) {
+        const int o = 16 * t + 4 * quad + i;
+        const float dd = (o < A.O && qvalid) ? o4[t][i] - A.target[(size_t)qi * A.O + o] : 0.f;
+        se = fmaf(dd, dd, se);
+      }
+#pragma unroll
+    for (int o = 32; o > 0; o >>= 1) se += __shfl_xor(se, o, 64);
+    if (lane == 0) atomicAdd(A.loss, se * A.inv_n);
+  } else if (q0 + col < A.NQ) {
 #pragma unroll
     for (int t = 0; t < 2; ++t)
 #pragma unroll
@@ -380,16 +394,21 @@
 static int launch_tail(const TailArgs& A, bool bwd, bool opt, hipStream_t st) {
   const bool wg = bwd && A.tdel != nullptr;
   const bool fused_loss = bwd && A.target != nullptr;
+  const bool fwd_loss = !bwd && A.target != nullptr;
   using T = TailCfg<D, H, BF16>;
   dim3 grid((A.NQ + 16 * NWAVES - 1) / (16 * NWAVES));
   const bool la2 = grid.x <= 256;
-  static EnfAttrBits attr_done[4][2][2];
+  static EnfAttrBits attr_done[5][2][2];
   auto go = [&](void (*kern_ptr)(TailArgs)) -> int {
     const int smem = la2 ? T::SMEM3 : T::SMEM;
-    if (!enf_lds_attr(reinterpret_cast<const void*>(kern_ptr), smem, attr_done[fused_loss ? 3 : (wg ? 2 : bwd)][la2][opt])) return ENF_ELAUNCH;
+    if (!enf_lds_attr(reinterpret_cast<const void*>(kern_ptr), smem, attr_done[fwd_loss ? 4 : fused_loss ? 3 : (wg ? 2 : bwd)][la2][opt])) return ENF_ELAUNCH;
     hipLaunchKernelGGL(kern_ptr, grid, dim3(NTHREADS), smem, st, A);
     return hipGetLastError() == hipSuccess ? 0 : ENF_ELAUNCH;
   };
+  if (fwd_loss) {
+    if (opt) return ENF_EINVAL;
+    return la2 ? go(enf_tail_fwd_kernel<D, H, BF16, true, false, true>) : go(enf_tail_fwd_kernel<D, H, BF16, false, false, true>);
+  }
   if (fused_loss) {
     if (wg || opt) return ENF_EINVAL;
     return la2 ? go(enf_tail_bwd_kernel<D, H, BF16, true, true, false, true>) : go(enf_tail_bwd_kernel<D, H, BF16, false, true, false, true>);
@@ -449,3 +468,23 @@
 #undef ENF_CASE
   return ENF_EUNSUPPORTED;
 }
+
+
+int enf_launch_tail_fwd_loss(const EnfDims& m, const EnfLayout& L, const char* blob, const float* ybar, int ybar_half, const float* target,
+                             float* loss, hipStream_t st) {
+  if (m.OB != 1) return ENF_EUNSUPPORTED;
+  TailArgs A;
+  A.ybar = ybar; A.blob = blob; A.L = L; A.out = nullptr; A.dout = nullptr; A.dybar = nullptr; A.delta = nullptr; A.act = nullptr; A.tdel = nullptr;
+  A.ybar_half = (ybar_half && m.bf16) ? 1 : 0;
+  A.target = target; A.loss = loss; A.gscale = 0.f; A.inv_n = 1.0f / ((float)m.B * (float)m.N * (float)m.O);
+  A.NQ = m.B * m.N; A.O = m.O; A.inv_hd = 1.0f / (float)(m.Ht * m.Dt);
+#define ENF_CASE(DD, HH)                                                                   \
+  if (m.D == DD && m.H == HH) return m.bf16 ? launch_tail<DD, HH, true>(A, false, false, st) : launch_tail<DD, HH, false>(A, false, false, st);
+  ENF_CASE(128, 2)
+  ENF_CASE(64, 2)
+  ENF_CASE(128, 1)
+  ENF_CASE(64, 1)
+  ENF_CASE(64, 4)
+#undef ENF_CASE
+  return ENF_EUNSUPPORTED;
+}
diff --git a/enf-pde_amd/enf/models/__init__.py b/enf-pde_amd/enf/models/__init__.py
--- a/enf-pde_amd/enf/models/__init__.py
+++ b/enf-pde_amd/enf/models/__init__.py
@@ -208,9 +208,9 @@
                               variants=tuple(_lib.VARIANT[v] for v in (self.pair_variants or self.default_pair_variants)),
                               masks=masks, embedding=_lib.EMB[self.embedding_type])
 
-    def _workspace(self, desc, device):
+    def _workspace(self, desc, device, nbytes_fn=None):
         lib = _lib.load()
-        nbytes = lib.enf_workspace_bytes(ctypes.byref(desc))
+        nbytes = (nbytes_fn or lib.enf_workspace_bytes)(ctypes.byref(desc))
         if nbytes == 0:
             _lib.check(lib.enf_check_desc(ctypes.byref(desc)))
         key = (str(device), torch.cuda.current_stream(device).cuda_stream)
@@ -417,6 +417,63 @@
             finally:
                 self._masks = prev
         return cm()
+
+    @torch.no_grad()
+    def fit_loop(self, params, lat, xs_all, ys_all, lrs, losses, grad_scale, optimize_gaussian_window):
+        inv = self.cross_attn_invariant
+        n_pos, n_ori = inv.num_z_pos_dims, inv.num_z_ori_dims
+        S = xs_all.shape[0] - 1
+        keys = {"p_pos", "a"} | ({"p_ori"} if n_ori > 0 else set())
+        win = lat.get("gaussian_window") if self.use_gaussian_window else None
+        move_win = bool(optimize_gaussian_window) and win is not None
+        need = keys | ({"gaussian_window"} if move_win else set())
+        if self.num_layers > 0 or not FUSED_FIT_STEP or S < 0 or not keys <= set(lat) or not need <= set(lrs) or \
+                (self.use_gaussian_window and win is None):
+            return None
+        B, Z = lat["a"].shape[:2]
+        N = xs_all.shape[1]
+        lr = {k: lrs[k].detach() for k in need}
+        if lat["p_pos"].shape[-1] != n_pos or (n_ori > 0 and lat["p_ori"].shape[-1] != n_ori) or lat["a"].shape[-1] != self.latent_dim or \
+                xs_all.shape[-1] != inv.num_x_pos_dims or tuple(ys_all.shape) != (S + 1, B, N, self.num_out) or \
+                (win is not None and tuple(win.shape) != (B, Z, 1)) or \
+                any(v.dtype != torch.float32 or not v.is_contiguous() or v.device != xs_all.device or v.numel() not in (1, lat[k].shape[-1])
+                    for k, v in lr.items()):
+            return None
+        lib = _lib.load()
+        dev = xs_all.device
+        packed = self.pack(params)
+        desc = self._desc(B, N, Z, masks=self._masks)
+        ws = self._workspace(desc, dev, lib.enf_fit_loop_workspace_bytes)
+        p0 = torch.cat((lat["p_pos"], lat["p_ori"]), dim=-1) if n_ori > 0 else lat["p_pos"]
+        sets = {"p": (p0, torch.empty_like(p0)), "a": (lat["a"], torch.empty_like(lat["a"])),
+                "s": (win, torch.empty_like(win) if move_win else None)}
+        L = _lib.EnfFitLatents()
+        for i in range(2):
+            L.p[i], L.a[i] = sets["p"][i].data_ptr(), sets["a"][i].data_ptr()
+            L.sigma[i] = sets["s"][i].data_ptr() if sets["s"][i] is not None else None
+        L.lr_pos, L.lr_a = lr["p_pos"].data_ptr(), lr["a"].data_ptr()
+        L.lr_ori = lr["p_ori"].data_ptr() if n_ori > 0 else None
+        L.lr_sigma = lr["gaussian_window"].data_ptr() if move_win else None
+        L.n_pos, L.lr_pos_len, L.lr_a_len = n_pos, lr["p_pos"].numel(), lr["a"].numel()
+        L.lr_ori_len = lr["p_ori"].numel() if n_ori > 0 else 0
+        st = ctypes.c_void_p(torch.cuda.current_stream(dev).cuda_stream)
+        _lib.launch(dev, lib.enf_fit_loop, ctypes.byref(desc), ctypes.byref(L), _ptr(xs_all), _ptr(ys_all), _ptr(packed), float(grad_scale),
+                    S, _ptr(losses), 0, _ptr(ws), ws.numel(), st)
+        tag = self._ws_touch(ws)
+        fin = S & 1
+        p_, a_ = sets["p"][fin], sets["a"][fin]
+        s_ = sets["s"][fin] if move_win else win
+        out = dict(lat)
+        out["a"] = a_
+        if n_ori > 0:
+            out["p_pos"], out["p_ori"] = p_[..., :n_pos].contiguous(), p_[..., n_pos:].contiguous()
+        else:
+            out["p_pos"] = p_
+        if win is not None:
+            out["gaussian_window"] = s_
+        lt_key = (ws.data_ptr(), packed.data_ptr(), B, Z) + tuple((t.data_ptr(), t._version) for t in (p_, a_) + ((s_,) if s_ is not None else ()))
+        self._lt_held[ws.data_ptr()] = (lt_key, tag[1], (p_, a_, s_, packed))
+        return out
 
     @torch.no_grad()
     def mse_value_and_latent_grads(self, params, x, p, a, gaussian_window_size, target, grad_scale=1.0, loss_out=None):
diff --git a/enf-pde_amd/fitting/inner_loop.py b/enf-pde_amd/fitting/inner_loop.py
--- a/enf-pde_amd/fitting/inner_loop.py
+++ b/enf-pde_amd/fitting/inner_loop.py
@@ -92,6 +92,10 @@
     if noise_pos:
         lat["p_pos"] = lat["p_pos"] + torch.randn(lat["p_pos"].shape, generator=generator,
                                                   device="cpu").to(lat["p_pos"].device) * noise_pos
+    if fused is not None and not noise_pos and hasattr(nef, "fit_loop"):
+        fitted = nef.fit_loop(nef_params, lat, xs_all, ys_all, lrs, losses, B, optimize_gaussian_window)
+        if fitted is not None:
+            return losses[S], fitted
     n_pos = lat["p_pos"].shape[-1]
     for s in range(S):
         xs = xs_all[s][None].expand(B, -1, -1)
diff --git a/include/enf_hip.h b/include/enf_hip.h
--- a/include/enf_hip.h
+++ b/include/enf_hip.h
@@ -181,6 +181,20 @@
 } EnfFitComponent;
 int enf_fit_inputs(int ncomp, const EnfFitComponent* comps, int32_t B, int32_t Z, int32_t N, int32_t Ns, int32_t S1, int32_t dx, int32_t O,
                    const float* coords, const float* img, const int64_t* masks, float* xs, float* ys, float* losses, void* stream);
+
+typedef struct EnfFitLatents {
+  float* p[2];
+  float* a[2];
+  float* sigma[2];
+  const float* lr_pos;
+  const float* lr_ori;
+  const float* lr_a;
+  const float* lr_sigma;
+  int32_t n_pos, lr_pos_len, lr_ori_len, lr_a_len;
+} EnfFitLatents;
+size_t enf_fit_loop_workspace_bytes(const EnfDesc* d);
+int enf_fit_loop(const EnfDesc* d, const EnfFitLatents* lat, const float* xs, const float* ys, const void* packed, float grad_scale,
+                 int steps, float* losses, unsigned flags, void* workspace, size_t workspace_bytes, void* stream);
 
 int enf_ode_conv_forward(int B, int Z, int J, int C, const float* a, const float* kb, int64_t kb_stride_r,
                          int64_t kb_stride_s, const float* W, const float* bias, float* out, void* stream);
```

Result: slower. 25.68 million (-3.8%).
